# TrevorS/voxtral-mini-realtime-rs

Measured on AMD Instinct MI355X. Metric: decode_tok_per_s, higher is better.
Workload: dtype f32

## Files before the change

include/voxtral_hip.h:

```cpp
#ifndef VOXTRAL_HIP_H
#define VOXTRAL_HIP_H

#include <stddef.h>
#include <stdint.h>

#ifdef __cplusplus
extern "C" {
#endif

#define VOX_OK 0
#define VOX_ERR_INVALID 1
#define VOX_ERR_IO 2
#define VOX_ERR_HIP 3
#define VOX_ERR_NOTFOUND 4
#define VOX_ERR_UNSUPPORTED 5

#define VOX_MEM_HOST 0
#define VOX_MEM_DEVICE 1

typedef struct vox_ctx vox_ctx;
typedef struct vox_gguf vox_gguf;
typedef struct vox_q4 vox_q4;
typedef struct vox_model vox_model;
typedef struct vox_cache vox_cache;
// ... 17 lines not shown
int32_t vox_resample_len(size_t n_in, uint32_t sr_in, uint32_t sr_out, size_t* n_out);
int32_t vox_resample(vox_ctx* ctx, const float* in, size_t n_in, uint32_t sr_in, uint32_t sr_out, float* out, size_t cap, size_t* n_out,
                     int32_t mem_kind);
int32_t vox_resample_plan(uint32_t sr_in, uint32_t sr_out, int32_t* fft_in, int32_t* fft_out, int32_t* delay, float* cutoff, float* taps_or_null, size_t cap);
int32_t vox_peak_normalize(float* samples, size_t n, float target_peak);

typedef struct {
    uint32_t sample_rate;
    uint32_t n_left_pad_tokens;
    float    frame_rate;
    uint32_t extra_right_pad_tokens;
} vox_pad_cfg;
int32_t vox_pad_cfg_voxtral(vox_pad_cfg* cfg);
int32_t vox_pad_len(size_t n, const vox_pad_cfg* cfg, size_t* out);
int32_t vox_pad_audio(const float* in, size_t n, const vox_pad_cfg* cfg, float* out);
int32_t vox_num_audio_tokens(size_t n, const vox_pad_cfg* cfg, size_t* out);

typedef struct {
    uint32_t max_mel_frames;
    uint32_t hop_length;
    uint32_t sample_rate;
    uint32_t overlap_frames;
} vox_chunk_cfg;
typedef struct { size_t start_sample, end_sample, index; int32_t is_last; } vox_chunk;
int32_t vox_needs_chunking(size_t n, const vox_chunk_cfg* cfg, int32_t* out);
int32_t vox_chunk_plan(size_t n, const vox_chunk_cfg* cfg, vox_chunk* out, size_t cap, size_t* n_chunks);

int32_t vox_mel_num_frames(size_t n_samples, size_t* out);
int32_t vox_mel_filterbank(float* out_128x201);
int32_t vox_hann_window(int32_t length, float* out);
int32_t vox_mel_compute_log(vox_ctx* ctx, const float* samples, size_t n, float* out_Tx128, int32_t mem_kind);

int32_t vox_time_embedding(float t, int32_t dim, float* out);

int32_t vox_gguf_open(const char* path, vox_gguf** out);
int32_t vox_gguf_open_memory(const void* data, size_t size, vox_gguf** out);
int32_t vox_gguf_open_shards(const void* const* shards, const size_t* sizes, int32_t n, vox_gguf** out);
int32_t vox_gguf_close(vox_gguf* g);
int32_t vox_gguf_version(const vox_gguf* g, uint32_t* out);
int32_t vox_gguf_tensor_count(const vox_gguf* g, uint64_t* out);
int32_t vox_gguf_tensor_name(const vox_gguf* g, uint64_t index, const char** out);
int32_t vox_gguf_tensor_info(const vox_gguf* g, const char* name, uint64_t dims[4], uint32_t* ndims,
                             uint32_t* dtype, uint64_t* nbytes);
int32_t vox_gguf_tensor_data(const vox_gguf* g, const char* name, void* dst, size_t cap);

int32_t vox_q4_tensor_from_bytes(vox_ctx* ctx, const uint8_t* raw, size_t nbytes, int64_t N, int64_t K, vox_q4** out);
int32_t vox_q4_tensor_shape(const vox_q4* q, int64_t* N, int64_t* K);
int32_t vox_q4_tensor_num_blocks(const vox_q4* q, int64_t* out);
int32_t vox_q4_tensor_dequantize(vox_ctx* ctx, const vox_q4* q, float* out_NxK);
int32_t vox_q4_tensor_free(vox_q4* q);
int32_t vox_q4_matmul(vox_ctx* ctx, const vox_q4* w, const float* x, int32_t B, int32_t M, float* out, int32_t mem_kind);
int32_t vox_q4_linear_forward(vox_ctx* ctx, const vox_q4* w, const float* bias_or_null, const float* x,
                              int32_t B, int32_t M, float* out, int32_t mem_kind);

int32_t vox_dense_tensor_from_f32(vox_ctx* ctx, const float* w_NxK, const float* w_other_or_null, int64_t N, int64_t K, vox_q4** out);
int32_t vox_linear_forward_ex(vox_ctx* ctx, const vox_q4* w, const float* bias_or_null, const float* x, int32_t B, int32_t M, float* out, int32_t epilogue, int32_t mem_kind);
int32_t vox_conv_downsample(vox_ctx* ctx, const float* x_CxL, int32_t C, int32_t L, const float* w1, const float* b1, const float* w2, const float* b2, int32_t O, float* out_OxL2);

typedef struct {
    int32_t enc_layers, enc_dim, enc_heads, enc_head_dim, enc_ffn, enc_window;
    int32_t dec_layers, dec_dim, dec_heads, dec_kv_heads, dec_head_dim, dec_ffn, dec_window, vocab;
    int32_t n_mels, reshape_factor, t_cond_dim;
    float rope_theta, norm_eps;
} vox_model_cfg;

int32_t vox_attention(vox_ctx* ctx, const float* q, const float* k, const float* v, int32_t M, int32_t kv_len, int32_t n_heads,
                      int32_t n_kv_heads, int32_t head_dim, int32_t offset, int32_t window, float* out, int32_t mem_kind);

int32_t vox_q4_model_load(vox_ctx* ctx, const char* gguf_path, vox_model** out);
#define VOX_LOAD_LAYOUT_ONLY 1u
int32_t vox_q4_model_load_ex(vox_ctx* ctx, const char* gguf_path, uint32_t flags, vox_model** out);
int32_t vox_q4_model_load_gguf(vox_ctx* ctx, vox_gguf* g, uint32_t flags, vox_model** out);
int32_t vox_f32_model_load(vox_ctx* ctx, const char* safetensors_path, vox_model** out);
int32_t vox_model_free(vox_model* m);
int32_t vox_model_config(const vox_model* m, vox_model_cfg* out);
int32_t vox_model_weight_bytes(const vox_model* m, uint64_t* out);
int32_t vox_model_arena(const vox_model* m, void** dev_ptr, uint64_t* nbytes);
int32_t vox_model_arena_finalize(vox_model* m);
int32_t vox_model_replicate(const vox_model* src, vox_ctx* dst_ctx, vox_model** out);
int32_t vox_model_memory(const vox_model* m, uint64_t out[4]);

int32_t vox_model_set_t_embed(vox_model* m, const float* t_embed_host);
int32_t vox_model_set_decode_engine(vox_model* m, int32_t on, int32_t* active_or_null);
int32_t vox_model_set_batch_engine(vox_model* m, int32_t on, int32_t* active_or_null, uint64_t* launches_or_null);

int32_t vox_encode_audio(vox_model* m, const float* mel_128xT, int32_t T, float* out, int32_t cap_rows,
                         int32_t* S, int32_t mem_kind);
int32_t vox_transcribe_streaming(vox_model* m, const float* mel_128xT, int32_t T, const float* t_embed,
                                 int32_t* out_ids, int32_t cap, int32_t* n_ids, float* logits_or_null,
                                 int32_t mem_kind);
int32_t vox_transcribe_audio(vox_model* m, const float* samples, size_t n, const float* t_embed,
                             int32_t* out_ids, int32_t cap, int32_t* n_ids, int32_t mem_kind);

int32_t vox_transcribe_batch(vox_model* m, int32_t n, const float* const* samples, const size_t* n_samples, const float* t_embed,
                             int32_t* const* out_ids, const int32_t* caps, int32_t* n_ids, int32_t mem_kind);
int32_t vox_transcribe_batch_ex(vox_model* m, int32_t n, const float* const* samples, const size_t* n_samples, const int32_t* norm_group_or_null, const float* t_embed,
                                int32_t* const* out_ids, const int32_t* caps, int32_t* n_ids, int32_t mem_kind);
int32_t vox_model_set_sessions(vox_model* m, int32_t sessions);

int32_t vox_decoder_cache_create(vox_model* m, int32_t max_seq, vox_cache** out);
int32_t vox_cache_free(vox_cache* c);
int32_t vox_cache_seq_len(const vox_cache* c, int32_t* out);
int32_t vox_cache_reset(vox_cache* c);
int32_t vox_cache_update(vox_cache* c, int32_t layer, int32_t pos, const float* k_HxNxhd, const float* v_HxNxhd, int32_t n_rows, int32_t mem_kind);
int32_t vox_cache_truncate(vox_cache* c, int32_t len);
int32_t vox_encoder_cache_create(vox_model* m, int32_t capacity_rows, vox_cache** out);
int32_t vox_encoder_cache_apply_sliding_window(vox_cache* enc_cache, int32_t window);
int32_t vox_cache_abs_pos(const vox_cache* c, int32_t* out);
int32_t vox_encode_audio_with_cache(vox_model* m, const float* mel_128xT, int32_t T, vox_cache* enc_cache, float* out, int32_t cap_rows,
                                    int32_t* S, int32_t mem_kind);
int32_t vox_embed_tokens_from_ids(vox_model* m, const int32_t* ids, int32_t n, float* out_nxD);
int32_t vox_forward_hidden_with_cache(vox_model* m, const float* x_MxD, int32_t M, const float* t_embed,
                                      vox_cache* cache, float* out_MxD);
int32_t vox_lm_head(vox_model* m, const float* hidden_MxD, int32_t M, float* logits_MxV);
int32_t vox_embed_tokens_from_ids_ex(vox_model* m, const int32_t* ids_host, int32_t n, float* out_nxD, int32_t mem_kind);
int32_t vox_tensor_add(vox_ctx* ctx, const float* a, const float* b, size_t n, float* out, int32_t mem_kind);
int32_t vox_forward_hidden_with_cache_ex(vox_model* m, const float* x_MxD, int32_t M, const float* t_embed, vox_cache* cache, float* out_MxD_or_null,
                                         const float** hidden_ws_or_null, int32_t mem_kind);
int32_t vox_lm_head_ex(vox_model* m, const float* hidden_MxD, int32_t M, float* logits_MxV, int32_t mem_kind);
int32_t vox_argmax_rows(vox_ctx* ctx, const float* logits_MxV, int32_t M, int32_t V, int32_t* ids_host, int32_t mem_kind);
int32_t vox_lm_head_argmax(vox_model* m, const float* hidden_MxD, int32_t M, int32_t* ids_host, int32_t mem_kind);
int32_t vox_generate_step_with_cache(vox_model* m, const int32_t* token_ids, int32_t n, const float* t_embed, vox_cache* cache, float* logits_nxV);

int32_t vox_forward(vox_model* m, const float* mel_128xT, int32_t T, const float* t_embed, float* logits_SxV, int32_t cap_rows, int32_t* S, int32_t mem_kind);
int32_t vox_forward_streaming(vox_model* m, const float* mel_128xT, int32_t T, const int32_t* token_ids, int32_t n_ids, const float* t_embed, float* logits_SxV,
                              int32_t cap_rows, int32_t* S, int32_t mem_kind);
int32_t vox_forward_with_cache(vox_model* m, const float* mel_128xT, int32_t T, const float* t_embed, vox_cache* enc_cache, vox_cache* dec_cache, float* logits_SxV,
                               int32_t cap_rows, int32_t* S, int32_t mem_kind);

typedef struct { double preprocess_ms, encode_ms, decode_ms, total_ms; int32_t decode_tokens; int32_t graph_replays; } vox_timings;
int32_t vox_get_stage_timings(const vox_model* m, vox_timings* out);

int32_t vox_debug_reload_knobs(void);
int32_t vox_debug_attn_launches(uint64_t* out, int32_t cap);
int32_t vox_debug_gemm_launches(uint64_t* out, int32_t cap);
int32_t vox_debug_occupy(vox_ctx* ctx, int32_t workgroups, int32_t micros);

int32_t vox_bench_decode_gemv(vox_model* m, int32_t which, int32_t iters, double* avg_us, double* bytes_per_launch,
                              const char** kernel_name);

int32_t vox_bench_wide(vox_model* m, int32_t which, int32_t mt, int32_t iters, double out_us[4]);

int32_t vox_debug_timeline_start(vox_ctx* ctx, int32_t n_slots, int32_t n_waves);
int32_t vox_debug_timeline_fetch(vox_ctx* ctx, uint64_t* out, size_t cap_words, int32_t* slots_used, int32_t* meta );
int32_t vox_debug_batch_tap_arm(vox_model* m, const int32_t* units, int32_t n_units, int32_t max_rows);
int32_t vox_debug_batch_tap_fetch(vox_model* m, float* out, int32_t* rows_per_unit);
int32_t vox_debug_encode_batch(vox_model* m, int32_t n, const float* const* mels, const int32_t* T, int32_t layout, float* out, int64_t cap_rows,
                               int32_t* rows_per_clip, int64_t* report);

#ifdef __cplusplus
}
#endif
#endif
```

voxtral-mini-realtime-rs_amd/_lib.py:

```python
from __future__ import annotations

import ctypes as C
import os

from .build import LIB_PATH


class VoxError(RuntimeError):
    def __init__(self, code, msg):
        super().__init__(f"[vox error {code}] {msg}")
        self.code = code


class PadCfg(C.Structure):
    _fields_ = [("sample_rate", C.c_uint32), ("n_left_pad_tokens", C.c_uint32), ("frame_rate", C.c_float),
                ("extra_right_pad_tokens", C.c_uint32)]


class ChunkCfg(C.Structure):
    _fields_ = [("max_mel_frames", C.c_uint32), ("hop_length", C.c_uint32), ("sample_rate", C.c_uint32),
                ("overlap_frames", C.c_uint32)]


class Chunk(C.Structure):
    _fields_ = [("start_sample", C.c_size_t), ("end_sample", C.c_size_t), ("index", C.c_size_t), ("is_last", C.c_int32)]


class ModelCfg(C.Structure):
    _fields_ = [(n, C.c_int32) for n in ("enc_layers", "enc_dim", "enc_heads", "enc_head_dim", "enc_ffn", "enc_window",
                                         "dec_layers", "dec_dim", "dec_heads", "dec_kv_heads", "dec_head_dim", "dec_ffn",
                                         "dec_window", "vocab", "n_mels", "reshape_factor", "t_cond_dim")] + \
               [("rope_theta", C.c_float), ("norm_eps", C.c_float)]


class Timings(C.Structure):
    _fields_ = [("preprocess_ms", C.c_double), ("encode_ms", C.c_double), ("decode_ms", C.c_double), ("total_ms", C.c_double),
                ("decode_tokens", C.c_int32), ("graph_replays", C.c_int32)]


vp, i32, i64, u32, u64, sz, f32 = C.c_void_p, C.c_int32, C.c_int64, C.c_uint32, C.c_uint64, C.c_size_t, C.c_float
P = C.POINTER

SIGNATURES = {
    "vox_last_error": (C.c_char_p, []),
    "vox_abi_version": (i32, []),
    "vox_device_count": (i32, [P(i32)]),
    "vox_ctx_create": (i32, [i32, P(vp)]),
    "vox_ctx_destroy": (i32, [vp]),
    "vox_debug_reload_knobs": (i32, []),
    "vox_ctx_synchronize": (i32, [vp]),
    "vox_ctx_set_shared": (i32, [vp, i32]),
    "vox_ctx_stream": (i32, [vp, P(vp)]),
    "vox_dev_alloc": (i32, [vp, sz, P(vp)]),
    "vox_dev_free": (i32, [vp, vp]),
    "vox_dev_upload": (i32, [vp, vp, vp, sz]),
    "vox_dev_download": (i32, [vp, vp, vp, sz]),
    "vox_dev_copy": (i32, [vp, vp, vp, sz]),
    "vox_peak_normalize": (i32, [vp, sz, f32]),
    "vox_pad_cfg_voxtral": (i32, [P(PadCfg)]),
    "vox_pad_len": (i32, [sz, P(PadCfg), P(sz)]),
    "vox_pad_audio": (i32, [vp, sz, P(PadCfg), vp]),
    "vox_num_audio_tokens": (i32, [sz, P(PadCfg), P(sz)]),
    "vox_needs_chunking": (i32, [sz, P(ChunkCfg), P(i32)]),
    "vox_chunk_plan": (i32, [sz, P(ChunkCfg), P(Chunk), sz, P(sz)]),
    "vox_mel_num_frames": (i32, [sz, P(sz)]),
    "vox_mel_filterbank": (i32, [vp]),
    "vox_hann_window": (i32, [i32, vp]),
    "vox_mel_compute_log": (i32, [vp, vp, sz, vp, i32]),
    "vox_time_embedding": (i32, [f32, i32, vp]),
    "vox_gguf_open": (i32, [C.c_char_p, P(vp)]),
    "vox_gguf_open_memory": (i32, [vp, C.c_size_t, P(vp)]),
    "vox_gguf_open_shards": (i32, [vp, vp, i32, P(vp)]),
    "vox_q4_model_load_gguf": (i32, [vp, vp, C.c_uint32, P(vp)]),
    "vox_gguf_close": (i32, [vp]),
    "vox_gguf_version": (i32, [vp, P(u32)]),
    "vox_gguf_tensor_count": (i32, [vp, P(u64)]),
    "vox_gguf_tensor_name": (i32, [vp, u64, P(C.c_char_p)]),
    "vox_gguf_tensor_info": (i32, [vp, C.c_char_p, P(u64 * 4), P(u32), P(u32), P(u64)]),
    "vox_gguf_tensor_data": (i32, [vp, C.c_char_p, vp, sz]),
    "vox_q4_tensor_from_bytes": (i32, [vp, vp, sz, i64, i64, P(vp)]),
    "vox_q4_tensor_shape": (i32, [vp, P(i64), P(i64)]),
    "vox_q4_tensor_num_blocks": (i32, [vp, P(i64)]),
    "vox_q4_tensor_dequantize": (i32, [vp, vp, vp]),
    "vox_q4_tensor_free": (i32, [vp]),
    "vox_q4_matmul": (i32, [vp, vp, vp, i32, i32, vp, i32]),
    "vox_q4_linear_forward": (i32, [vp, vp, vp, vp, i32, i32, vp, i32]),
    "vox_dense_tensor_from_f32": (i32, [vp, vp, vp, i64, i64, P(vp)]),
    "vox_linear_forward_ex": (i32, [vp, vp, vp, vp, i32, i32, vp, i32, i32]),
    "vox_conv_downsample": (i32, [vp, vp, i32, i32, vp, vp, vp, vp, i32, vp]),
    "vox_attention": (i32, [vp, vp, vp, vp, i32, i32, i32, i32, i32, i32, i32, vp, i32]),
    "vox_q4_model_load": (i32, [vp, C.c_char_p, P(vp)]),
    "vox_q4_model_load_ex": (i32, [vp, C.c_char_p, u32, P(vp)]),
    "vox_f32_model_load": (i32, [vp, C.c_char_p, P(vp)]),
    "vox_model_free": (i32, [vp]),
    "vox_model_config": (i32, [vp, P(ModelCfg)]),
    "vox_model_weight_bytes": (i32, [vp, P(u64)]),
    "vox_model_arena": (i32, [vp, P(vp), P(u64)]),
    "vox_model_set_t_embed": (i32, [vp, vp]),
    "vox_model_set_decode_engine": (i32, [vp, i32, P(i32)]),
    "vox_debug_occupy": (i32, [vp, i32, i32]),
    "vox_model_memory": (i32, [vp, P(C.c_uint64)]),
    "vox_model_set_batch_engine": (i32, [vp, i32, P(i32), P(C.c_uint64)]),
    "vox_model_arena_finalize": (i32, [vp]),
    "vox_model_replicate": (i32, [vp, vp, P(vp)]),
    "vox_model_set_sessions": (i32, [vp, i32]),
    "vox_generate_step_with_cache": (i32, [vp, vp, i32, vp, vp, vp]),
    "vox_encode_audio": (i32, [vp, vp, i32, vp, i32, P(i32), i32]),
    "vox_transcribe_streaming": (i32, [vp, vp, i32, vp, vp, i32, P(i32), vp, i32]),
    "vox_transcribe_audio": (i32, [vp, vp, sz, vp, vp, i32, P(i32), i32]),
    "vox_transcribe_batch": (i32, [vp, i32, P(vp), P(sz), vp, P(vp), P(i32), P(i32), i32]),
    "vox_transcribe_batch_ex": (i32, [vp, i32, P(vp), P(sz), vp, vp, P(vp), P(i32), P(i32), i32]),
    "vox_decoder_cache_create": (i32, [vp, i32, P(vp)]),
    "vox_cache_free": (i32, [vp]),
    "vox_cache_seq_len": (i32, [vp, P(i32)]),
    "vox_cache_reset": (i32, [vp]),
    "vox_cache_update": (i32, [vp, i32, i32, vp, vp, i32, i32]),
    "vox_cache_truncate": (i32, [vp, i32]),
    "vox_resample_len": (i32, [sz, C.c_uint32, C.c_uint32, P(sz)]),
    "vox_resample": (i32, [vp, vp, sz, C.c_uint32, C.c_uint32, vp, sz, P(sz), i32]),
    "vox_resample_plan": (i32, [C.c_uint32, C.c_uint32, P(i32), P(i32), P(i32), P(C.c_float), vp, sz]),
    "vox_encoder_cache_create": (i32, [vp, i32, P(vp)]),
    "vox_encoder_cache_apply_sliding_window": (i32, [vp, i32]),
    "vox_cache_abs_pos": (i32, [vp, P(i32)]),
    "vox_encode_audio_with_cache": (i32, [vp, vp, i32, vp, vp, i32, P(i32), i32]),
    "vox_embed_tokens_from_ids": (i32, [vp, vp, i32, vp]),
    "vox_forward_hidden_with_cache": (i32, [vp, vp, i32, vp, vp, vp]),
    "vox_lm_head": (i32, [vp, vp, i32, vp]),
    "vox_embed_tokens_from_ids_ex": (i32, [vp, vp, i32, vp, i32]),
    "vox_tensor_add": (i32, [vp, vp, vp, sz, vp, i32]),
    "vox_forward_hidden_with_cache_ex": (i32, [vp, vp, i32, vp, vp, vp, P(vp), i32]),
    "vox_lm_head_ex": (i32, [vp, vp, i32, vp, i32]),
    "vox_argmax_rows": (i32, [vp, vp, i32, i32, vp, i32]),
    "vox_lm_head_argmax": (i32, [vp, vp, i32, vp, i32]),
    "vox_forward": (i32, [vp, vp, i32, vp, vp, i32, P(i32), i32]),
    "vox_forward_streaming": (i32, [vp, vp, i32, vp, i32, vp, vp, i32, P(i32), i32]),
    "vox_forward_with_cache": (i32, [vp, vp, i32, vp, vp, vp, vp, i32, P(i32), i32]),
    "vox_get_stage_timings": (i32, [vp, P(Timings)]),
    "vox_bench_decode_gemv": (i32, [vp, i32, i32, P(C.c_double), P(C.c_double), P(C.c_char_p)]),
    "vox_bench_wide": (i32, [vp, i32, i32, i32, P(C.c_double)]),
    "vox_debug_attn_launches": (i32, [P(C.c_uint64), i32]),
    "vox_debug_gemm_launches": (i32, [P(C.c_uint64), i32]),
    "vox_debug_timeline_start": (i32, [vp, i32, i32]),
    "vox_debug_timeline_fetch": (i32, [vp, vp, sz, P(i32), vp]),
    "vox_debug_batch_tap_arm": (i32, [vp, P(i32), i32, i32]),
    "vox_debug_batch_tap_fetch": (i32, [vp, vp, P(i32)]),
    "vox_debug_encode_batch": (i32, [vp, i32, P(vp), P(i32), i32, vp, C.c_int64, P(i32), P(C.c_int64)]),
}

_LIB = None
_KNOBS = None


def _knob_env():
    return tuple(sorted((k, v) for k, v in os.environ.items() if k.startswith("VOX_")))


def lib():
    global _LIB, _KNOBS
    if _LIB is not None:
        k = _knob_env()
        if k != _KNOBS:
            _KNOBS = k; _LIB.vox_debug_reload_knobs()
        return _LIB
    if not os.path.exists(LIB_PATH):
        raise VoxError(-1, f"{LIB_PATH} not built: run `python __graft_entry__.py build` (hipcc, gfx950). "
                           "There is no CPU fallback for the HIP path.")
    L = C.CDLL(LIB_PATH)
    for name, (res, args) in SIGNATURES.items():
        fn = getattr(L, name)
        fn.restype = res
        fn.argtypes = args
    _LIB = L; _KNOBS = _knob_env()
    return L


def check(code: int):
    if code != 0:
        raise VoxError(code, (lib().vox_last_error() or b"").decode(errors="replace"))
```

voxtral-mini-realtime-rs_amd/csrc/vox_api.cpp:

```cpp
#include "../../include/voxtral_hip.h"
#include "vox_kernels.h"

#include <dlfcn.h>
#include <fcntl.h>
#include <sys/mman.h>
#include <sys/stat.h>
#include <unistd.h>

#include <algorithm>
#include <chrono>
#include <cmath>
#include <cstdarg>
#include <cstdio>
#include <cstdlib>
#include <cstring>
#include <map>
#include <mutex>
#include <string>
#include <unordered_map>
#include <thread>
#include <vector>

using namespace vox;

// ... 595 lines not shown
    if (e == hipSuccess) e = hipMemcpy(q->sc_mem, l2.data(), ne * 2, hipMemcpyHostToDevice);
    if (e == hipSuccess) e = hipMemcpy(q->qt_mem, host.data(), ne * 4, hipMemcpyHostToDevice);
    if (e != hipSuccess) return bail(e);
    q->w = Q4W{(const uint4*)q->qs_mem, (const uint16_t*)q->sc_mem, (int)Ntot, (int)K, (int)(K / 32), WFMT_F32}; q->w.qt = (const uint4*)q->qt_mem;
    *out = q; return VOX_OK;
}
extern "C" int32_t vox_linear_forward_ex(vox_ctx* c, const vox_q4* w, const float* bias, const float* x, int32_t B, int32_t M, float* out, int32_t epilogue, int32_t mem_kind) {
    ARGCHK(c && w && x && out, "null argument"); ARGCHK(B > 0 && M > 0, "bad batch/rows"); VOXCHK(ctx_bind(c));
    ARGCHK(epilogue == 0 || epilogue == 1 || epilogue == 2, "epilogue %d: 0 none, 1 GELU, 2 SwiGLU over interleaved gate / up rows", epilogue);
    const int epi = epilogue == 1 ? EPI_GELU : epilogue == 2 ? EPI_SWIGLU : EPI_STORE;
    const int rows = B * M, K = w->w.K, N = w->w.N, No = epilogue == 2 ? N / 2 : N;
    ARGCHK(epilogue != 2 || (N % 2 == 0 && !bias), "SwiGLU epilogue needs an even number of interleaved rows and no bias");
    if (mem_kind == VOX_MEM_DEVICE) return q4_linear_dev(c, w->w, bias, x, K, rows, out, No, epi);
    DevBuf dx, dy, db; HIPCHK(dx.alloc((size_t)rows * K * 4)); HIPCHK(dy.alloc((size_t)rows * No * 4));
    HIPCHK(hipMemcpyAsync(dx.p, x, (size_t)rows * K * 4, hipMemcpyHostToDevice, c->stream));
    if (bias) { HIPCHK(db.alloc((size_t)N * 4)); HIPCHK(hipMemcpyAsync(db.p, bias, (size_t)N * 4, hipMemcpyHostToDevice, c->stream)); }
    VOXCHK(q4_linear_dev(c, w->w, bias ? db.as<float>() : nullptr, dx.as<float>(), K, rows, dy.as<float>(), No, epi));
    HIPCHK(hipMemcpyAsync(out, dy.p, (size_t)rows * No * 4, hipMemcpyDeviceToHost, c->stream)); HIPCHK(hipStreamSynchronize(c->stream));
    return VOX_OK;
}
extern "C" int32_t vox_conv_downsample(vox_ctx* c, const float* x, int32_t C, int32_t L, const float* w1, const float* b1, const float* w2, const float* b2, int32_t O, float* out) {
    ARGCHK(c && x && w1 && b1 && w2 && b2 && out && C > 0 && L > 0 && O > 0, "bad argument"); ARGCHK((3 * C) % 128 == 0 && (3 * O) % 128 == 0, "3 * channels must be a multiple of 128");
    VOXCHK(ctx_bind(c)); hipStream_t s = c->stream;
    const int T1 = (L + 2 - 3) / 2 + 1, S = (T1 + 2 - 3) / 2 + 1;
    auto planes = [&](const float* w, int Co, int Ci, DevBuf& hi, DevBuf& lo, Q4W* q) -> int32_t {
        const size_t K = (size_t)3 * Ci; std::vector<float> r((size_t)Co * K);
        for (int co = 0; co < Co; co++) for (int ci = 0; ci < Ci; ci++) for (int kk = 0; kk < 3; kk++) r[(size_t)co * K + (size_t)kk * Ci + ci] = w[((size_t)co * Ci + ci) * 3 + kk];
        std::vector<uint16_t> h(r.size()), l(r.size()); bf16_split(r.data(), r.size(), h.data(), l.data());
        HIPCHK(hi.alloc(h.size() * 2)); HIPCHK(lo.alloc(l.size() * 2));
        HIPCHK(hipMemcpy(hi.p, h.data(), h.size() * 2, hipMemcpyHostToDevice)); HIPCHK(hipMemcpy(lo.p, l.data(), l.size() * 2, hipMemcpyHostToDevice));
        *q = Q4W{(const uint4*)hi.p, (const uint16_t*)lo.p, Co, (int)K, (int)(K / 32), WFMT_BF16X2}; return VOX_OK;
    };
    DevBuf h1, l1, h2, l2, dx, dm, d1, dy, dyt, db1, db2; Q4W g1{}, g2{};
    VOXCHK(planes(w1, O, C, h1, l1, &g1)); VOXCHK(planes(w2, O, O, h2, l2, &g2));
    HIPCHK(dx.alloc((size_t)C * L * 4)); HIPCHK(dm.alloc((size_t)(L + 2) * C * 4)); HIPCHK(d1.alloc((size_t)(T1 + 2) * O * 4)); HIPCHK(dy.alloc((size_t)S * O * 4)); HIPCHK(dyt.alloc((size_t)S * O * 4));
    HIPCHK(db1.alloc((size_t)O * 4)); HIPCHK(db2.alloc((size_t)O * 4));
    HIPCHK(hipMemcpyAsync(dx.p, x, (size_t)C * L * 4, hipMemcpyHostToDevice, s)); HIPCHK(hipMemcpyAsync(db1.p, b1, (size_t)O * 4, hipMemcpyHostToDevice, s)); HIPCHK(hipMemcpyAsync(db2.p, b2, (size_t)O * 4, hipMemcpyHostToDevice, s));
    HIPCHK(hipMemsetAsync(dm.p, 0, (size_t)(L + 2) * C * 4, s)); HIPCHK(hipMemsetAsync(d1.p, 0, (size_t)(T1 + 2) * O * 4, s));
    HIPCHK(launch_transpose(dx.as<float>(), C, L, dm.as<float>() + C, s));
    { GemmParams g{}; g.w = g1; g.x = dm.as<float>(); g.x_stride = 2 * C; g.M = T1; g.out = d1.as<float>() + O; g.out_stride = O; g.bias = db1.as<float>(); HIPCHK(launch_dense2_gemm(g, EPI_GELU, s)); }
    { GemmParams g{}; g.w = g2; g.x = d1.as<float>(); g.x_stride = 2 * O; g.M = S; g.out = dy.as<float>(); g.out_stride = O; g.bias = db2.as<float>(); HIPCHK(launch_dense2_gemm(g, EPI_GELU, s)); }
    HIPCHK(launch_transpose(dy.as<float>(), S, O, dyt.as<float>(), s));
    HIPCHK(hipMemcpyAsync(out, dyt.p, (size_t)S * O * 4, hipMemcpyDeviceToHost, s)); HIPCHK(hipStreamSynchronize(s));
    return VOX_OK;
}

extern "C" int32_t vox_attention(vox_ctx* c, const float* q, const float* k, const float* v, int32_t M, int32_t kv_len, int32_t n_heads,
                                 int32_t n_kv_heads, int32_t head_dim, int32_t offset, int32_t window, float* out, int32_t mem_kind) {
    ARGCHK(c && q && k && v && out, "null argument");
    ARGCHK(M > 0 && kv_len > 0 && n_heads > 0 && n_kv_heads > 0 && n_heads % n_kv_heads == 0, "bad attention shape");
    ARGCHK(head_dim == 64 || head_dim == 128, "head_dim must be 64 (encoder) or 128 (decoder)");
    ARGCHK(offset >= 0 && offset + M <= kv_len, "queries must lie inside the key range (offset + M <= kv_len)");
    VOXCHK(ctx_bind(c));
    const size_t qn = (size_t)M * n_heads * head_dim, kn = (size_t)kv_len * n_kv_heads * head_dim;
    DevBuf dq, dk, dv, dout;
    const float *pq = q, *pk = k, *pv = v; float* po = out;
    if (mem_kind != VOX_MEM_DEVICE) {
        HIPCHK(dq.alloc(qn * 4)); HIPCHK(dk.alloc(kn * 4)); HIPCHK(dv.alloc(kn * 4)); HIPCHK(dout.alloc(qn * 4));
        HIPCHK(hipMemcpyAsync(dq.p, q, qn * 4, hipMemcpyHostToDevice, c->stream));
        HIPCHK(hipMemcpyAsync(dk.p, k, kn * 4, hipMemcpyHostToDevice, c->stream));
        HIPCHK(hipMemcpyAsync(dv.p, v, kn * 4, hipMemcpyHostToDevice, c->stream));
        pq = dq.as<float>(); pk = dk.as<float>(); pv = dv.as<float>(); po = dout.as<float>();
    }
    AttnParams ap{}; ap.q = pq; ap.q_stride = n_heads * head_dim; ap.k = pk; ap.v = pv; ap.kv_row_stride = n_kv_heads * head_dim; ap.kv_head_stride = head_dim;
    ap.out = po; ap.out_stride = n_heads * head_dim; ap.M = M; ap.kv_len = kv_len; ap.n_heads = n_heads; ap.n_kv_heads = n_kv_heads; ap.offset = offset; ap.window = window;
    HIPCHK(launch_attn_prefill(ap, head_dim, c->stream));
    if (mem_kind != VOX_MEM_DEVICE) { HIPCHK(hipMemcpyAsync(out, po, qn * 4, hipMemcpyDeviceToHost, c->stream)); HIPCHK(hipStreamSynchronize(c->stream)); }
    return VOX_OK;
}

struct Lin { Q4W w{}; const float* bias = nullptr; };
struct EncLayer { const float *attn_norm = nullptr, *ffn_norm = nullptr; Lin wqkv, wo, w13, w2; };
struct DecLayer { const float *attn_norm = nullptr, *ffn_norm = nullptr; Lin wqkv, wo, w13, w2, ada0, ada2; float* ada_mul = nullptr; };

struct vox_cache { vox_model* m; vox_ctx* ctx = nullptr; float *k = nullptr, *v = nullptr; int max_seq = 0, len = 0; size_t layer_stride = 0;
                   int kind = 0, abs_pos = 0; uint64_t gen = 0; };

static std::mutex g_cache_mu; static std::unordered_map<const vox_cache*, uint64_t> g_cache_live; static uint64_t g_cache_gen = 0;
static void cache_register(vox_cache* k) { std::lock_guard<std::mutex> l(g_cache_mu); k->gen = ++g_cache_gen; g_cache_live[k] = k->gen; }
static void cache_unregister(const vox_cache* k) { std::lock_guard<std::mutex> l(g_cache_mu); g_cache_live.erase(k); }
static bool cache_alive(const vox_cache* k, uint64_t gen) { std::lock_guard<std::mutex> l(g_cache_mu); auto it = g_cache_live.find(k); return it != g_cache_live.end() && it->second == gen; }

struct TensorMeta { std::vector<uint64_t> shape; int dtype = 0; uint64_t nbytes = 0; };
struct vox_model {
    vox_ctx* ctx = nullptr; vox_model_cfg cfg{};
    std::vector<vox_model*> twins;
    std::map<std::string, TensorMeta> manifest; bool is_q4 = false;
    uint8_t* arena = nullptr; uint64_t arena_bytes = 0, arena_primary_bytes = 0;
    std::vector<Q4W*> tiled;
    const float *conv1_w = nullptr, *conv1_b = nullptr, *conv2_w = nullptr, *conv2_b = nullptr, *enc_norm = nullptr, *dec_norm = nullptr;
    Q4W conv1_g{}, conv2_g{};
    const float *enc_cos = nullptr, *enc_sin = nullptr, *dec_cos = nullptr, *dec_sin = nullptr;
    int enc_rope_len = 4096, dec_rope_len = 16384;
    std::vector<EncLayer> enc; std::vector<DecLayer> dec; Lin ad0, ad2, tok;
    float* ada_mul = nullptr; bool t_embed_set = false; std::vector<float> t_embed_host;
    float* ws = nullptr; size_t ws_floats = 0;
    float *d_audio = nullptr; int audio_cap = 0;
    float *d_mel = nullptr; size_t mel_cap = 0;
    float *d_samples = nullptr; size_t samples_cap = 0;
    vox_cache* cache = nullptr;
    int *d_tokens = nullptr, *d_pos = nullptr; int tokens_cap = 0;
    float* d_prefix = nullptr;
    float *enc_cos_s = nullptr, *enc_sin_s = nullptr; int enc_rope_s_len = 0;
    int* d_seq_len = nullptr; std::vector<int> h_seq_len;
    int *d_seq_off = nullptr, *d_row_pos = nullptr; size_t row_pos_cap = 0; std::vector<int> h_seq_off, h_row_pos;
    float *d_h = nullptr, *d_q = nullptr, *d_att = nullptr, *d_act = nullptr, *d_logits = nullptr, *d_part_val = nullptr; int* d_part_idx = nullptr;
    float* d_h2 = nullptr; long long* d_wo_acc = nullptr;
    int n_parts = 0, argmax_R = 8;
    bool eng_ok = false, eng_on = true, eng_ready = false; unsigned char* eng_stream = nullptr; unsigned char* eng_state = nullptr; EngLayerTab* eng_tab = nullptr;
    const vox_cache* eng_tab_cache = nullptr; const float* eng_tab_k = nullptr; std::vector<EngLayerTab> eng_tab_host;
    int eng_flags = 128 | 512 | 1, eng_pace = 50;
    unsigned long long eng_launches = 0; unsigned eng_err_host[2] = {0, 0};
    int eng_strikes = 0; bool eng_suspended = false;
    unsigned char* eng_wob = nullptr;
    bool engb_ok = false; unsigned char* engb_state[4] = {nullptr, nullptr, nullptr, nullptr}; EngLayerTab* engb_tab[4] = {nullptr, nullptr, nullptr, nullptr};
    bool engb_on = true; unsigned long long engb_launches = 0; int engb_strikes = 0;
    int batch_sessions = 0;
    int engb_flags = 128 | 1 | 64 | 2048;
    int engb_flags2 = 128 | 1024;
    unsigned engb_err_host[4][2] = {{0, 0}, {0, 0}, {0, 0}, {0, 0}};
    hipGraph_t graph[2] = {nullptr, nullptr}; hipGraphExec_t graph_exec[2] = {nullptr, nullptr}; int graph_unroll = 0, graph_mode = 0;
    const vox_cache* graph_cache = nullptr; const float* graph_audio = nullptr;
    float *pw_x = nullptr, *pw_hidden = nullptr, *pw_logits = nullptr; size_t pw_x_cap = 0, pw_hidden_cap = 0, pw_logits_cap = 0;
    float* pw_part_val = nullptr; int* pw_part_idx = nullptr; int* pw_ids = nullptr; int pw_ids_cap = 0; int* pw_zero = nullptr;
    EngLayerTab* pw_tab = nullptr; const vox_cache* pw_tab_cache = nullptr; uint64_t pw_tab_gen = 0;
    bool pw_memo = false, pw_eng_used = false;
    vox_cache* pw_pend_cache = nullptr; uint64_t pw_pend_gen = 0; int pw_pend_rows = 0; bool pw_verdict_failed = false;
    unsigned* pw_err_pin = nullptr;
    vox_timings timings{};
    struct { std::vector<int> units; int max_rows = 0; bool armed = false, on = false, ready = false; float* out = nullptr; int* rows = nullptr; } tap;
};

struct Arena {
    uint8_t* base = nullptr; uint64_t off = 0;
    template <class T> T* take(size_t count) {
        off = (off + 255) / 256 * 256;
        T* p = base ? reinterpret_cast<T*>(base + off) : nullptr;
        off += count * sizeof(T);
        return p;
    }
};

#define ENC_PFX "mm_streams_embeddings.embedding_module.whisper_encoder"
#define EMB_PFX "mm_streams_embeddings.embedding_module"
#define TOK_NAME EMB_PFX ".tok_embeddings.weight"
#define ADP_PFX EMB_PFX ".audio_language_projection"

enum { DT_F32 = 0, DT_F16 = 1, DT_Q4_0 = 2, DT_BF16 = 3 };
struct TensorView { std::vector<uint64_t> shape; int dtype = 0; const uint8_t* data = nullptr; uint64_t nbytes = 0; };
struct TensorSource {
    virtual ~TensorSource() {}
    virtual bool find(const std::string& name, TensorView* out) const = 0;
    virtual uint64_t max_q4_bytes() const { return 0; }
};
struct GgufSource : TensorSource {
    vox_gguf* g = nullptr;
    ~GgufSource() override { if (g) vox_gguf_close(g); }
    bool find(const std::string& name, TensorView* out) const override {
        const GTensor* t = g->find(name); if (!t) return false;
        out->shape.assign(t->dims, t->dims + t->ndims); std::reverse(out->shape.begin(), out->shape.end());
        out->dtype = (int)t->dtype; out->data = g->data(t); out->nbytes = t->nbytes; return true;
    }
    uint64_t max_q4_bytes() const override { uint64_t m = 0; for (auto& t : g->tensors) if (t.dtype == 2) m = std::max<uint64_t>(m, t.nbytes); return m; }
};
struct RecordingSource : TensorSource {
    const TensorSource* in; mutable std::map<std::string, TensorMeta> seen;
    explicit RecordingSource(const TensorSource* s) : in(s) {}
// ... 251 lines not shown
            if (hipMemcpy(dst, host.data(), (size_t)tot * 4, hipMemcpyHostToDevice) != hipSuccess) setfail("hipMemcpy failed for bias");
        }
        return dst;
    }
    const float* rope(int hd, int len, float theta, bool sine) {
        const int half = hd / 2; float* dst = ar.take<float>((size_t)len * half);
        if (fill) {
            std::vector<float> t((size_t)len * half);
            for (int i = 0; i < len; i++)
                for (int j = 0; j < half; j++) {
                    const float inv = 1.0f / std::pow(theta, (float)(2 * j) / (float)hd), fr = (float)i * inv;
                    t[(size_t)i * half + j] = sine ? std::sin(fr) : std::cos(fr);
                }
            if (hipMemcpy(dst, t.data(), t.size() * 4, hipMemcpyHostToDevice) != hipSuccess) setfail("hipMemcpy failed for rope table");
        }
        return dst;
    }

    bool run(bool q4) {
        vox_model_cfg& c = m->cfg; char a[320]; TensorView tv;
        c.enc_head_dim = 64; c.dec_head_dim = 128; c.enc_window = 750; c.dec_window = 8192; c.rope_theta = 1e6f; c.norm_eps = 1e-5f; c.reshape_factor = 4;
        int ne = 0, nd = 0;
        for (;; ne++) { snprintf(a, sizeof a, ENC_PFX ".transformer.layers.%d.attention.wq.weight", ne); if (!src->find(a, &tv)) break; }
        for (;; nd++) { snprintf(a, sizeof a, "layers.%d.attention.wq.weight", nd); if (!src->find(a, &tv)) break; }
        if (ne == 0 || nd == 0) return setfail("model file has no encoder/decoder layers");
        c.enc_layers = ne; c.dec_layers = nd; m->enc.resize(ne); m->dec.resize(nd);
        TensorView cw; if (!need(ENC_PFX ".conv_layers.0.conv.weight", &cw)) return false;
        if (cw.shape.size() != 3 || cw.shape[2] != 3) return setfail("conv weight must be [out][in][3]");
        c.n_mels = (int)cw.shape[1]; c.enc_dim = (int)cw.shape[0];
        m->conv1_w = f32(ENC_PFX ".conv_layers.0.conv.weight"); m->conv1_b = f32(ENC_PFX ".conv_layers.0.conv.bias");
        m->conv2_w = f32(ENC_PFX ".conv_layers.1.conv.weight"); m->conv2_b = f32(ENC_PFX ".conv_layers.1.conv.bias");
        if ((3 * c.n_mels) % 128 == 0 && (3 * c.enc_dim) % 128 == 0) {
            if (!conv_planes(ENC_PFX ".conv_layers.0.conv.weight", &m->conv1_g) || !conv_planes(ENC_PFX ".conv_layers.1.conv.weight", &m->conv2_g)) return false;
        }
        for (int i = 0; i < ne; i++) {
            EncLayer& L = m->enc[i]; std::string p = std::string(ENC_PFX ".transformer.layers.") + std::to_string(i);
            L.attn_norm = f32(p + ".attention_norm.weight"); L.ffn_norm = f32(p + ".ffn_norm.weight");
            if (!lin({p + ".attention.wq.weight", p + ".attention.wk.weight", p + ".attention.wv.weight"}, false, &L.wqkv, q4)) return false;
            const int64_t hq = L.wqkv.w.N / 3;
            L.wqkv.bias = bias_cat({{p + ".attention.wq.bias", hq}, {"", hq}, {p + ".attention.wv.bias", hq}});
            if (!lin({p + ".attention.wo.weight"}, false, &L.wo, q4)) return false;
            L.wo.bias = bias_cat({{p + ".attention.wo.bias", L.wo.w.N}});
            if (!lin({p + ".feed_forward.w1.weight", p + ".feed_forward.w3.weight"}, true, &L.w13, q4)) return false;
            if (!lin({p + ".feed_forward.w2.weight"}, false, &L.w2, q4)) return false;
            L.w2.bias = bias_cat({{p + ".feed_forward.w2.bias", L.w2.w.N}});
        }
        m->enc_norm = f32(ENC_PFX ".transformer.norm.weight");
        if (!lin({ADP_PFX ".0.weight"}, false, &m->ad0, q4) || !lin({ADP_PFX ".2.weight"}, false, &m->ad2, q4)) return false;
        if (!lin({TOK_NAME}, false, &m->tok, false, true)) return false;
        for (int i = 0; i < nd; i++) {
            DecLayer& L = m->dec[i]; std::string p = "layers." + std::to_string(i);
            if (!lin({p + ".ada_rms_norm_t_cond.0.weight"}, false, &L.ada0, q4) || !lin({p + ".ada_rms_norm_t_cond.2.weight"}, false, &L.ada2, q4)) return false;
            L.attn_norm = f32(p + ".attention_norm.weight"); L.ffn_norm = f32(p + ".ffn_norm.weight");
            if (!lin({p + ".attention.wq.weight", p + ".attention.wk.weight", p + ".attention.wv.weight"}, false, &L.wqkv, q4, true)) return false;
            if (!lin({p + ".attention.wo.weight"}, false, &L.wo, q4, true)) return false;
            if (!lin({p + ".feed_forward.w1.weight", p + ".feed_forward.w3.weight"}, true, &L.w13, q4, true)) return false;
            if (!lin({p + ".feed_forward.w2.weight"}, false, &L.w2, q4, true)) return false;
        }
        m->dec_norm = f32("norm.weight");
        if (!err.empty()) return false;
        TensorView ewq, dwq, dwk;
        need(std::string(ENC_PFX ".transformer.layers.0.attention.wq.weight"), &ewq); need("layers.0.attention.wq.weight", &dwq); need("layers.0.attention.wk.weight", &dwk);
        c.enc_heads = (int)(ewq.shape[0] / c.enc_head_dim); c.enc_ffn = m->enc[0].w13.w.N / 2;
        c.dec_dim = (int)dwq.shape[1]; c.dec_heads = (int)(dwq.shape[0] / c.dec_head_dim); c.dec_kv_heads = (int)(dwk.shape[0] / c.dec_head_dim);
        c.dec_ffn = m->dec[0].w13.w.N / 2; c.vocab = m->tok.w.N; c.t_cond_dim = m->dec[0].ada0.w.N;
        if (ewq.shape[0] % c.enc_head_dim || dwq.shape[0] % c.dec_head_dim || dwk.shape[0] % c.dec_head_dim || c.dec_kv_heads == 0 || c.dec_heads % c.dec_kv_heads)
            return setfail("attention projection shapes are not multiples of head_dim");
        if ((int)ewq.shape[1] != c.enc_dim || m->ad0.w.K != c.enc_dim * c.reshape_factor || m->ad2.w.N != c.dec_dim || m->ad0.w.N != m->ad2.w.K || m->tok.w.K != c.dec_dim)
            return setfail("inconsistent encoder / adapter / embedding shapes");
        if (c.enc_dim % 32 || c.dec_dim % 32) return setfail("model dims must be multiples of 32");
        m->enc_cos = rope(c.enc_head_dim, m->enc_rope_len, c.rope_theta, false); m->enc_sin = rope(c.enc_head_dim, m->enc_rope_len, c.rope_theta, true);
        m->dec_cos = rope(c.dec_head_dim, m->dec_rope_len, c.rope_theta, false); m->dec_sin = rope(c.dec_head_dim, m->dec_rope_len, c.rope_theta, true);
        return err.empty();
    }
};
}

static void graphs_destroy(vox_model* m) {
    for (int i = 0; i < 2; i++) {
        if (m->graph_exec[i]) { (void)hipGraphExecDestroy(m->graph_exec[i]); m->graph_exec[i] = nullptr; }
        if (m->graph[i]) { (void)hipGraphDestroy(m->graph[i]); m->graph[i] = nullptr; }
    }
}
static void model_release(vox_model* m) {
    if (!m) return;
    for (vox_model* t : m->twins) { vox_ctx* tc = t->ctx; model_release(t); (void)vox_ctx_destroy(tc); }
    m->twins.clear();
    (void)hipSetDevice(m->ctx->device); (void)hipStreamSynchronize(m->ctx->stream);
    graphs_destroy(m);
    if (m->cache) { cache_unregister(m->cache); (void)hipFree(m->cache->k); (void)hipFree(m->cache->v); delete m->cache; }
    if (m->ctx->pw_model == m) m->ctx->pw_model = nullptr;
    for (void* p : {(void*)m->arena, (void*)m->ada_mul, (void*)m->ws, (void*)m->d_audio, (void*)m->d_mel, (void*)m->d_samples, (void*)m->d_tokens, (void*)m->d_pos,
                    (void*)m->d_h, (void*)m->d_h2, (void*)m->d_wo_acc, (void*)m->d_q, (void*)m->d_att, (void*)m->d_act, (void*)m->d_logits, (void*)m->d_part_val, (void*)m->d_part_idx, (void*)m->d_seq_len, (void*)m->d_seq_off, (void*)m->d_row_pos, (void*)m->d_prefix, (void*)m->enc_cos_s, (void*)m->enc_sin_s, (void*)m->eng_stream, (void*)m->eng_wob, (void*)m->eng_state, (void*)m->eng_tab, (void*)m->engb_state[0], (void*)m->engb_state[1], (void*)m->engb_state[2], (void*)m->engb_state[3],
                    (void*)m->engb_tab[0], (void*)m->engb_tab[1], (void*)m->engb_tab[2], (void*)m->engb_tab[3], (void*)m->pw_x, (void*)m->pw_hidden, (void*)m->pw_logits, (void*)m->pw_part_val, (void*)m->pw_part_idx, (void*)m->pw_ids, (void*)m->pw_zero, (void*)m->pw_tab})
        if (p) (void)hipFree(p);
    if (m->pw_err_pin) (void)hipHostFree(m->pw_err_pin);
    if (m->tap.out) (void)hipFree(m->tap.out);
    if (m->tap.rows) (void)hipFree(m->tap.rows);
    delete m;
}
extern "C" int32_t vox_model_free(vox_model* m) { model_release(m); return VOX_OK; }

static int32_t model_build(vox_ctx* ctx, const TensorSource* src_in, bool q4, bool layout_only, vox_model** out) {
    vox_model* m = new vox_model(); m->ctx = ctx;
    RecordingSource rec(src_in); const TensorSource* src = &rec;
    std::map<std::string, bool> fmt_cache;
    Loader plan{m, src, Arena{}, false}; plan.fmt_cache = &fmt_cache;
    if (!plan.run(q4)) { std::string e = plan.err; model_release(m); return fail(VOX_ERR_IO, "%s", e.c_str()); }
    m->arena_primary_bytes = (plan.ar.off + 255) / 256 * 256 + 256;
    m->arena_bytes = m->arena_primary_bytes + plan.ar2.off + 256;
    if (hipMalloc((void**)&m->arena, m->arena_bytes) != hipSuccess) { model_release(m); return fail(VOX_ERR_HIP, "hipMalloc of %.1f MB weight arena failed", m->arena_bytes / 1e6); }
    const size_t max_q4 = layout_only ? 16 : std::max<uint64_t>(src->max_q4_bytes(), 16);
    DevBuf staging; if (staging.alloc(max_q4) != hipSuccess) { model_release(m); return fail(VOX_ERR_HIP, "hipMalloc of staging buffer failed"); }
    Loader fillr{m, src, Arena{m->arena, 0}, !layout_only, staging.p, max_q4}; fillr.fmt_cache = &fmt_cache; fillr.ar2 = Arena{m->arena + m->arena_primary_bytes, 0};
    if (!fillr.run(q4)) { std::string e = fillr.err; model_release(m); return fail(VOX_ERR_IO, "%s", e.c_str()); }
    const vox_model_cfg& c = m->cfg;
    const int qdim = c.dec_heads * c.dec_head_dim;
    if (m->tok.w.fmt == WFMT_BF16 || m->tok.w.fmt == WFMT_F32) { m->argmax_R = 2; m->n_parts = dense_gemv_grid(c.vocab); }
    else { m->argmax_R = q4_gemv_default_R(c.vocab, c.dec_dim, EPI_ARGMAX); m->n_parts = m->argmax_R > 0 ? q4_gemv_grid(c.vocab, m->argmax_R) : 1; }
    hipError_t e = hipSuccess;
    auto A = [&](void** p, size_t n) { if (e == hipSuccess) e = hipMalloc(p, n); };
    A((void**)&m->ada_mul, (size_t)c.dec_layers * c.dec_dim * 4); A((void**)&m->d_pos, 64); A((void**)&m->d_h, (size_t)c.dec_dim * 4 * 4);
    A((void**)&m->d_q, (size_t)qdim * 4 * 4); A((void**)&m->d_att, (size_t)qdim * 4 * 4); A((void**)&m->d_act, (size_t)c.dec_ffn * 4 * 4);
    A((void**)&m->d_h2, (size_t)c.dec_dim * 4); A((void**)&m->d_wo_acc, (size_t)c.dec_layers * c.dec_dim * 8);
    A((void**)&m->d_logits, (size_t)c.vocab * 4); A((void**)&m->d_part_val, (size_t)m->n_parts * 4 * 4); A((void**)&m->d_part_idx, (size_t)m->n_parts * 4 * 4);
    if (e != hipSuccess) { model_release(m); return fail(VOX_ERR_HIP, "hipMalloc of decode buffers failed: %s", hipGetErrorString(e)); }
    if (hipMemset(m->d_wo_acc, 0, (size_t)c.dec_layers * c.dec_dim * 8) != hipSuccess) { model_release(m); return fail(VOX_ERR_HIP, "hipMemset failed"); }
    for (int i = 0; i < c.dec_layers; i++) m->dec[i].ada_mul = m->ada_mul + (size_t)i * c.dec_dim;
    {
        const char* ev = knob_str("VOX_ENGINE"); bool ok = !(ev && ev[0] == '0') && c.dec_layers <= 32 && eng_geometry_ok(c.dec_dim, c.dec_heads, c.dec_kv_heads, c.dec_head_dim, c.dec_ffn, c.vocab, 256);
        hipDeviceProp_t prop; if (ok && (hipGetDeviceProperties(&prop, ctx->device) != hipSuccess || prop.multiProcessorCount != 256)) ok = false;
        for (int i = 0; ok && i < c.dec_layers; i++) { const DecLayer& L = m->dec[i]; for (const Lin* w : {&L.wqkv, &L.wo, &L.w13, &L.w2}) if (w->w.fmt != WFMT_Q4_0 || !w->w.qs || !w->w.sc || w->bias) ok = false; }
        if (ok && (m->tok.w.fmt != WFMT_Q4_0 || !m->tok.w.qs)) ok = false;
        if (ok) { int occ = 0; if (eng_occupancy(&occ) != hipSuccess || occ < 1) { ok = false; (void)hipGetLastError(); } }
        m->eng_ok = ok; m->eng_on = ok;
        {
            const char* bv = knob_str("VOX_BATCH_ENGINE"); int occ = 0;
            m->engb_ok = ok && !(bv && bv[0] == '0') && engb_occupancy(&occ) == hipSuccess && occ >= 1;
            (void)hipGetLastError();
            if (const char* f = knob_str("VOX_BATCH_ENGINE_FLAGS")) m->engb_flags = atoi(f);
            if (const char* f = knob_str("VOX_BATCH_ENGINE_FLAGS2")) m->engb_flags2 = atoi(f);
        }
        if (const char* f = knob_str("VOX_ENGINE_FLAGS")) m->eng_flags = atoi(f);
        if (const char* f = knob_str("VOX_ENGINE_PACE")) m->eng_pace = atoi(f);
    }
    m->manifest = std::move(rec.seen); m->is_q4 = q4;
    *out = m; return VOX_OK;
}

extern "C" int32_t vox_q4_model_load(vox_ctx* ctx, const char* path, vox_model** out) { return vox_q4_model_load_ex(ctx, path, 0, out); }

extern "C" int32_t vox_q4_model_load_gguf(vox_ctx* ctx, vox_gguf* g, uint32_t flags, vox_model** out) {
    ARGCHK(ctx && g && out, "null argument"); VOXCHK(ctx_bind(ctx));
    GgufSource src; src.g = g;
    const int32_t r = model_build(ctx, &src, true, (flags & VOX_LOAD_LAYOUT_ONLY) != 0, out);
    src.g = nullptr;
    return r;
}
extern "C" int32_t vox_q4_model_load_ex(vox_ctx* ctx, const char* path, uint32_t flags, vox_model** out) {
    ARGCHK(ctx && path && out, "null argument"); VOXCHK(ctx_bind(ctx));
    GgufSource src; VOXCHK(vox_gguf_open(path, &src.g));
    return model_build(ctx, &src, true, (flags & VOX_LOAD_LAYOUT_ONLY) != 0, out);
}

extern "C" int32_t vox_f32_model_load(vox_ctx* ctx, const char* path, vox_model** out) {
    ARGCHK(ctx && path && out, "null argument"); VOXCHK(ctx_bind(ctx));
    SafeTensorsSource src; VOXCHK(src.open(path));
    return model_build(ctx, &src, false, false, out);
}

extern "C" int32_t vox_model_config(const vox_model* m, vox_model_cfg* out) { ARGCHK(m && out, "null argument"); *out = m->cfg; return VOX_OK; }
extern "C" int32_t vox_model_weight_bytes(const vox_model* m, uint64_t* out) { ARGCHK(m && out, "null argument"); *out = m->arena_bytes; return VOX_OK; }
extern "C" int32_t vox_model_memory(const vox_model* m, uint64_t out[4]) {
    ARGCHK(m && out, "null argument");
    out[0] = m->arena_bytes; out[1] = m->arena_primary_bytes;
    out[2] = (m->eng_stream ? eng_stream_bytes(m->cfg.dec_layers, m->cfg.vocab) : 0) + (m->eng_wob ? engb_wo_stream_bytes(m->cfg.dec_layers) : 0);
    out[3] = m->eng_state ? eng_state_bytes() : 0;
    for (int gi = 0; gi < 4; gi++) if (m->engb_state[gi]) out[3] += engb_state_bytes();
    return VOX_OK;
}
extern "C" int32_t vox_model_arena(const vox_model* m, void** p, uint64_t* n) { ARGCHK(m && p && n, "null argument"); *p = m->arena; *n = m->arena_primary_bytes; return VOX_OK; }
extern "C" int32_t vox_model_arena_finalize(vox_model* m) {
    ARGCHK(m, "null argument"); VOXCHK(ctx_bind(m->ctx));
    for (Q4W* w : m->tiled) HIPCHK(launch_q4_tile_build(*w, const_cast<uint4*>(w->qt), const_cast<uint16_t*>(w->st), m->ctx->stream));
    HIPCHK(hipStreamSynchronize(m->ctx->stream));
    m->eng_ready = false; m->eng_tab_cache = nullptr;
    if (m->eng_wob) { HIPCHK(hipStreamSynchronize(m->ctx->stream)); (void)hipFree(m->eng_wob); m->eng_wob = nullptr; }
    graphs_destroy(m);
    return VOX_OK;
}

extern "C" int32_t vox_model_replicate(const vox_model* src, vox_ctx* dst_ctx, vox_model** out) {
    ARGCHK(src && dst_ctx && out, "null argument");
    if (!src->is_q4 || src->manifest.empty()) return fail(VOX_ERR_UNSUPPORTED, "vox_model_replicate: Q4 (GGUF) models only");
    VOXCHK(ctx_bind(src->ctx)); HIPCHK(hipStreamSynchronize(src->ctx->stream));
    VOXCHK(ctx_bind(dst_ctx));
    ManifestSource ms; ms.m = &src->manifest;
    vox_model* d = nullptr;
    VOXCHK(model_build(dst_ctx, &ms, true, true, &d));
    if (d->arena_primary_bytes != src->arena_primary_bytes || d->arena_bytes != src->arena_bytes) { model_release(d); return fail(VOX_ERR_INVALID, "internal: replica arena layout differs from the source's"); }
    hipError_t e = src->ctx->device == dst_ctx->device ? hipMemcpyAsync(d->arena, src->arena, src->arena_primary_bytes, hipMemcpyDeviceToDevice, dst_ctx->stream)
                                                       : hipMemcpyPeerAsync(d->arena, dst_ctx->device, src->arena, src->ctx->device, src->arena_primary_bytes, dst_ctx->stream);
    if (e == hipSuccess) e = hipStreamSynchronize(dst_ctx->stream);
    if (e != hipSuccess) { model_release(d); return fail(VOX_ERR_HIP, "vox_model_replicate: device copy failed: %s", hipGetErrorString(e)); }
    const int32_t r = vox_model_arena_finalize(d);
    if (r != VOX_OK) { model_release(d); return r; }
    *out = d; return VOX_OK;
}

extern "C" int32_t vox_model_set_t_embed(vox_model* m, const float* t_embed) {
    ARGCHK(m && t_embed, "null argument"); VOXCHK(ctx_bind(m->ctx));
    const vox_model_cfg& c = m->cfg; vox_ctx* cx = m->ctx;
    if (m->t_embed_set && m->t_embed_host.size() == (size_t)c.dec_dim && !std::memcmp(m->t_embed_host.data(), t_embed, (size_t)c.dec_dim * 4)) return VOX_OK;
    DevBuf dt, dh, ones; HIPCHK(dt.alloc((size_t)c.dec_dim * 4)); HIPCHK(dh.alloc((size_t)c.t_cond_dim * 4)); HIPCHK(ones.alloc((size_t)c.dec_dim * 4));
    std::vector<float> one(c.dec_dim, 1.0f);
    HIPCHK(hipMemcpyAsync(dt.p, t_embed, (size_t)c.dec_dim * 4, hipMemcpyHostToDevice, cx->stream));
    HIPCHK(hipMemcpyAsync(ones.p, one.data(), (size_t)c.dec_dim * 4, hipMemcpyHostToDevice, cx->stream));
    for (int i = 0; i < c.dec_layers; i++) {
        VOXCHK(q4_linear_dev(cx, m->dec[i].ada0.w, nullptr, dt.as<float>(), c.dec_dim, 1, dh.as<float>(), c.t_cond_dim, EPI_GELU));
        VOXCHK(q4_linear_dev(cx, m->dec[i].ada2.w, nullptr, dh.as<float>(), c.t_cond_dim, 1, m->dec[i].ada_mul, c.dec_dim, EPI_RESID, ones.as<float>(), c.dec_dim));
    }
    HIPCHK(hipStreamSynchronize(cx->stream));
    m->t_embed_host.assign(t_embed, t_embed + c.dec_dim); m->t_embed_set = true;
    return VOX_OK;
}

static int conv_len(int L) { return (L + 2 - 3) / 2 + 1; }

static int32_t ensure(float** p, size_t* cap, size_t need) {
    if (*cap >= need) return VOX_OK;
    if (*p) HIPCHK(hipFree(*p));
    *p = nullptr; *cap = 0;
    HIPCHK(hipMalloc((void**)p, need * sizeof(float))); *cap = need; return VOX_OK;
}

static int enc_rows(int T) { return conv_len(conv_len(T)); }
static int enc_row_budget(const vox_model* m, const int* T, int n) {
    int mx = 0; for (int i = 0; i < n; i++) mx = std::max(mx, enc_rows(T[i]));
    const int r = m->cfg.reshape_factor; return n == 1 ? mx : (mx + r - 1) / r * r;
}
static size_t conv_scratch_floats(const vox_model* m, int T) {
    const int D = m->cfg.enc_dim, T1 = conv_len(T);
    return std::max((size_t)D * T1, (size_t)(T + 2) * m->cfg.n_mels + (size_t)(T1 + 2) * D) + 64;
}
static int32_t conv_stem_dev(vox_model* m, const float* d_mel, int T, float* c1, float* x) {
    const vox_model_cfg& c = m->cfg; hipStream_t s = m->ctx->stream; const int D = c.enc_dim, T1 = conv_len(T), S = conv_len(T1);
    const bool conv_mfma = m->conv1_g.qs && m->conv2_g.qs && !knob_str("VOX_CONV_VALU");
    if (conv_mfma) {
        const int Cm = c.n_mels;
        float* melT = c1; float* c1T = melT + (size_t)(T + 2) * Cm;
        HIPCHK(hipMemsetAsync(melT, 0, (size_t)Cm * 4, s)); HIPCHK(hipMemsetAsync(melT + (size_t)(T + 1) * Cm, 0, (size_t)Cm * 4, s));
        HIPCHK(hipMemsetAsync(c1T, 0, (size_t)D * 4, s)); HIPCHK(hipMemsetAsync(c1T + (size_t)(T1 + 1) * D, 0, (size_t)D * 4, s));
        HIPCHK(launch_transpose(d_mel, Cm, T, melT + Cm, s));
        { GemmParams g{}; g.w = m->conv1_g; g.x = melT; g.x_stride = 2 * Cm; g.M = T1; g.out = c1T + D; g.out_stride = D; g.bias = m->conv1_b; HIPCHK(launch_dense2_gemm(g, EPI_GELU, s)); }
        { GemmParams g{}; g.w = m->conv2_g; g.x = c1T; g.x_stride = 2 * D; g.M = S; g.out = x; g.out_stride = D; g.bias = m->conv2_b; HIPCHK(launch_dense2_gemm(g, EPI_GELU, s)); }
    } else {
        HIPCHK(launch_conv1d_gelu(d_mel, c.n_mels, T, m->conv1_w, m->conv1_b, D, c1, 0, s));
        HIPCHK(launch_conv1d_gelu(c1, D, T1, m->conv2_w, m->conv2_b, D, x, 1, s));
    }
    return VOX_OK;
}
static int enc_packed_rows_of(const vox_model* m, int T) { const int R = m->cfg.reshape_factor; return std::max((enc_rows(T) + R - 1) / R * R, R * 40); }
static long enc_packed_rows(const vox_model* m, const int* T, int n) { long r = 0; for (int i = 0; i < n; i++) r += enc_packed_rows_of(m, T[i]); return r; }
struct EncForms { long Mtot = 0; int ksp = 0, ksp_wo = 0, fused_rope = 0; };
static int32_t encode_batch_dev(vox_model* m, int n, const float* const* d_mels, const int* T, float* audio_out, int audio_rows, int* S4_out, long* audio_off_out = nullptr,
                                EncForms* forms = nullptr) {
    const vox_model_cfg& c = m->cfg; vox_ctx* cx = m->ctx; hipStream_t s = cx->stream;
    const int D = c.enc_dim, H = c.enc_heads, hd = c.enc_head_dim, QD = H * hd, F = c.enc_ffn, R = c.reshape_factor;
    const bool packed = audio_off_out != nullptr;
    ARGCHK(n <= 128, "internal: encoder stack of %d utterances", n);
    const int S_pad = enc_row_budget(m, T, n);
    int T1max = 0; bool any = false;
    std::vector<int> S(n);
    for (int i = 0; i < n; i++) { S[i] = enc_rows(T[i]); S4_out[i] = S[i] / R; T1max = std::max(T1max, conv_len(T[i])); any = any || S4_out[i] > 0; }
    if (!any || S_pad <= 0) return VOX_OK;
    ARGCHK(S_pad <= m->enc_rope_len, "audio too long for the encoder RoPE table (%d > %d positions); chunk it (--max-mel-frames)", S_pad, m->enc_rope_len);
    std::vector<int> roff(n + 1, 0);
    if (packed) for (int i = 0; i < n; i++) roff[i + 1] = roff[i] + enc_packed_rows_of(m, T[i]);
    const int Mtot = packed ? roff[n] : n * S_pad, M4 = packed ? Mtot / R : n == 1 ? S4_out[0] : Mtot / R;
    ARGCHK(packed || n == 1 || audio_rows >= S_pad / R, "internal: audio row budget %d < %d", audio_rows, S_pad / R);
    int Tmax = 0; for (int i = 0; i < n; i++) Tmax = std::max(Tmax, T[i]);
    (void)T1max;
    const size_t c1_floats = conv_scratch_floats(m, Tmax);
    int ksp = 0;
    {
        const Q4W& w2 = m->enc[0].w2.w;
        const long wgs = (long)((w2.N + 127) / 128) * ((Mtot + 31) / 32);
        const bool geom_ok = w2.fmt == WFMT_Q4_0 && w2.qt && w2.st && w2.nb % 16 == 0 && Mtot > 48 && D % 4 == 0 && D <= 4096;
        if (geom_ok && wgs < 1024) ksp = 4;
        if (const char* e = knob_str("VOX_ENC_SPLITK")) ksp = geom_ok && atoi(e) > 1 ? std::min(atoi(e), w2.nb / 4) : 0;
        for (int l = 0; ksp && l < c.enc_layers; l++) if (m->enc[l].w2.w.fmt != WFMT_Q4_0 || !m->enc[l].w2.w.qt || m->enc[l].w2.w.nb / 4 < ksp) ksp = 0;
    }
    int ksp_wo = ksp ? 2 : 0;
    if (ksp) { if (const char* e = knob_str("VOX_ENC_SPLITK_WO")) ksp_wo = atoi(e) > 1 ? std::min(atoi(e), ksp) : 0; }
    for (int l = 0; ksp_wo && l < c.enc_layers; l++) if (m->enc[l].wo.w.fmt != WFMT_Q4_0 || !m->enc[l].wo.w.qt || m->enc[l].wo.w.nb / 4 < ksp_wo || m->enc[l].wo.w.nb % 4) ksp_wo = 0;
    const size_t need = c1_floats + (size_t)Mtot * D * 2 + (size_t)Mtot * QD * 4 + (size_t)Mtot * F + (size_t)(M4 + 1) * m->ad0.w.N + (size_t)ksp * Mtot * D + 1024;
    VOXCHK(ensure(&m->ws, &m->ws_floats, need));
    if (forms) { forms->Mtot = Mtot; forms->ksp = ksp; forms->ksp_wo = ksp_wo; forms->fused_rope = 0; }
    float* c1 = m->ws; float* x = c1 + c1_floats / 64 * 64; float* xn = x + (size_t)Mtot * D; float* qkv = xn + (size_t)Mtot * D;
    float* att = qkv + (size_t)Mtot * QD * 3; float* ffn = att + (size_t)Mtot * QD; float* ah = ffn + (size_t)Mtot * F; float* w2p = ah + (size_t)(M4 + 1) * m->ad0.w.N;
    const int* d_len = nullptr; const int* d_roff = nullptr; const int* d_rpos = nullptr;
    if (n > 1 || packed) {
        HIPCHK(hipMemsetAsync(x, 0, (size_t)Mtot * D * 4, s));
        HIPCHK(hipMemsetAsync(att, 0, (size_t)Mtot * QD * 4, s));
        if (!m->d_seq_len) HIPCHK(hipMalloc((void**)&m->d_seq_len, 128 * sizeof(int)));
        m->h_seq_len.assign(S.begin(), S.end());
        HIPCHK(hipMemcpyAsync(m->d_seq_len, m->h_seq_len.data(), (size_t)n * 4, hipMemcpyHostToDevice, s));
        d_len = m->d_seq_len;
    }
    if (packed) {
        if (!m->d_seq_off) HIPCHK(hipMalloc((void**)&m->d_seq_off, 128 * sizeof(int)));
        if (m->row_pos_cap < (size_t)Mtot) { if (m->d_row_pos) { HIPCHK(hipStreamSynchronize(s)); HIPCHK(hipFree(m->d_row_pos)); } m->d_row_pos = nullptr; m->row_pos_cap = 0;
                                              HIPCHK(hipMalloc((void**)&m->d_row_pos, (size_t)Mtot * sizeof(int))); m->row_pos_cap = (size_t)Mtot; }
        HIPCHK(hipStreamSynchronize(s));
        m->h_seq_off.assign(roff.begin(), roff.begin() + n); m->h_row_pos.resize((size_t)Mtot);
        for (int i = 0; i < n; i++) for (int r = roff[i]; r < roff[i + 1]; r++) m->h_row_pos[(size_t)r] = std::min(r - roff[i], m->enc_rope_len - 1);
        HIPCHK(hipMemcpyAsync(m->d_seq_off, m->h_seq_off.data(), (size_t)n * 4, hipMemcpyHostToDevice, s)); HIPCHK(hipMemcpyAsync(m->d_row_pos, m->h_row_pos.data(), (size_t)Mtot * 4, hipMemcpyHostToDevice, s));
        d_roff = m->d_seq_off; d_rpos = m->d_row_pos;
    }
    for (int i = 0; i < n; i++) {
        if (S[i] <= 0) continue;
        VOXCHK(conv_stem_dev(m, d_mels[i], T[i], c1, x + (packed ? (size_t)roff[i] : (size_t)i * S_pad) * D));
    }
    const int seq_rows = packed ? 0 : n > 1 ? S_pad : 0;
    for (int l = 0; l < c.enc_layers; l++) {
        const EncLayer& L = m->enc[l];
        if (ksp && l > 0) HIPCHK(launch_rms_norm_sumk(x, D, Mtot, D, w2p, (size_t)Mtot * D, ksp, L.attn_norm, c.norm_eps, xn, D, s));
        else HIPCHK(launch_rms_norm(x, D, Mtot, D, L.attn_norm, nullptr, c.norm_eps, xn, D, s));
        if (Mtot > 48) {
            GemmParams g{}; g.w = L.wqkv.w; g.x = xn; g.x_stride = D; g.M = Mtot; g.out = qkv; g.out_stride = 3 * QD; g.bias = L.wqkv.bias;
            g.rope_cos = m->enc_cos; g.rope_sin = m->enc_sin; g.hd = hd; g.n_q = 2 * QD; g.pos = d_rpos; g.rope_seq_rows = seq_rows;
            bool fused = false; HIPCHK(launch_q4_gemm(g, EPI_ROPE_ROWS, s, &fused));
            if (forms && fused) forms->fused_rope++;
        } else {
            VOXCHK(q4_linear_dev(cx, L.wqkv.w, L.wqkv.bias, xn, D, Mtot, qkv, 3 * QD));
            HIPCHK(launch_rope(qkv, Mtot, 3 * QD, 2 * QD, hd, 0, m->enc_cos, m->enc_sin, s, seq_rows, d_rpos));
        }
        AttnParams ap{}; ap.q = qkv; ap.q_stride = 3 * QD; ap.k = qkv + QD; ap.v = qkv + 2 * QD; ap.kv_row_stride = 3 * QD; ap.kv_head_stride = hd;
        ap.out = att; ap.out_stride = QD; ap.M = S_pad; ap.kv_len = S_pad; ap.n_heads = H; ap.n_kv_heads = H; ap.offset = 0; ap.window = c.enc_window;
        ap.seq_len = d_len; ap.q_seq_stride = S_pad * 3 * QD; ap.out_seq_stride = S_pad * QD; ap.kv_seq_stride = (long)S_pad * 3 * QD; ap.seq_row_off = d_roff;
        HIPCHK(launch_attn_prefill(ap, hd, s, n));
        if (ksp_wo) {
            VOXCHK(q4_linear_dev(cx, L.wo.w, L.wo.bias, att, QD, Mtot, w2p, D, EPI_STORE, nullptr, 0, ksp_wo));
            HIPCHK(launch_rms_norm_sumk(x, D, Mtot, D, w2p, (size_t)Mtot * D, ksp_wo, L.ffn_norm, c.norm_eps, xn, D, s));
        } else {
            VOXCHK(q4_linear_dev(cx, L.wo.w, L.wo.bias, att, QD, Mtot, x, D, EPI_RESID, x, D));
            HIPCHK(launch_rms_norm(x, D, Mtot, D, L.ffn_norm, nullptr, c.norm_eps, xn, D, s));
        }
        VOXCHK(q4_linear_dev(cx, L.w13.w, nullptr, xn, D, Mtot, ffn, F, EPI_SWIGLU));
        if (ksp) VOXCHK(q4_linear_dev(cx, L.w2.w, L.w2.bias, ffn, F, Mtot, w2p, D, EPI_STORE, nullptr, 0, ksp));
        else VOXCHK(q4_linear_dev(cx, L.w2.w, L.w2.bias, ffn, F, Mtot, x, D, EPI_RESID, x, D));
    }
    if (ksp && c.enc_layers > 0) HIPCHK(launch_rms_norm_sumk(x, D, Mtot, D, w2p, (size_t)Mtot * D, ksp, m->enc_norm, c.norm_eps, xn, D, s));
    else HIPCHK(launch_rms_norm(x, D, Mtot, D, m->enc_norm, nullptr, c.norm_eps, xn, D, s));
    VOXCHK(q4_linear_dev(cx, m->ad0.w, nullptr, xn, D * R, M4, ah, m->ad0.w.N, EPI_GELU));
    if (packed) { for (int i = 0; i < n; i++) audio_off_out[i] = (long)(roff[i] / R) * c.dec_dim; }
    if (packed || n == 1 || audio_rows * R == S_pad) VOXCHK(q4_linear_dev(cx, m->ad2.w, nullptr, ah, m->ad0.w.N, M4, audio_out, c.dec_dim));
    else for (int i = 0; i < n; i++)
        VOXCHK(q4_linear_dev(cx, m->ad2.w, nullptr, ah + (size_t)i * (S_pad / R) * m->ad0.w.N, m->ad0.w.N, S_pad / R, audio_out + (size_t)i * audio_rows * c.dec_dim, c.dec_dim));
    return VOX_OK;
}
static int32_t encode_dev(vox_model* m, const float* d_mel, int T, int* S4_out) {
    const int S4 = enc_rows(T) / m->cfg.reshape_factor;
    if (S4 > 0) { size_t cap = (size_t)m->audio_cap * m->cfg.dec_dim; VOXCHK(ensure(&m->d_audio, &cap, (size_t)S4 * m->cfg.dec_dim)); m->audio_cap = (int)(cap / m->cfg.dec_dim); }
    return encode_batch_dev(m, 1, &d_mel, &T, m->d_audio, S4, S4_out);
}

static int32_t cache_alloc(vox_model* m, int max_seq, vox_cache** out) {
    const vox_model_cfg& c = m->cfg;
    ARGCHK(max_seq > 0 && max_seq <= m->dec_rope_len, "max_seq %d out of range (1..%d)", max_seq, m->dec_rope_len);
    vox_cache* k = new vox_cache(); k->m = m; k->ctx = m->ctx; k->max_seq = max_seq;
    const size_t n = (size_t)c.dec_layers * c.dec_kv_heads * max_seq * c.dec_head_dim * 4;
    if (hipMalloc((void**)&k->k, n) != hipSuccess || hipMalloc((void**)&k->v, n) != hipSuccess) { if (k->k) (void)hipFree(k->k); delete k; return fail(VOX_ERR_HIP, "hipMalloc of KV cache failed"); }
    HIPCHK(hipMemsetAsync(k->k, 0, n, m->ctx->stream)); HIPCHK(hipMemsetAsync(k->v, 0, n, m->ctx->stream));
    k->layer_stride = (size_t)c.dec_kv_heads * max_seq * c.dec_head_dim;
    cache_register(k);
    *out = k; return VOX_OK;
}
extern "C" int32_t vox_decoder_cache_create(vox_model* m, int32_t max_seq, vox_cache** out) { ARGCHK(m && out, "null argument"); VOXCHK(ctx_bind(m->ctx)); return cache_alloc(m, max_seq, out); }
extern "C" int32_t vox_cache_free(vox_cache* k) {
    if (!k) return VOX_OK;
    (void)hipSetDevice(k->ctx->device); (void)hipStreamSynchronize(k->ctx->stream);
    cache_unregister(k);
    (void)hipFree(k->k); (void)hipFree(k->v); delete k; return VOX_OK;
}
static int32_t pw_sync(vox_model* m);
static int32_t cache_settle_pending(vox_cache* kc) {
    vox_model* m = kc->m;
    if (m && m->pw_pend_rows > 0 && m->pw_pend_cache == kc) { VOXCHK(ctx_bind(kc->ctx)); VOXCHK(pw_sync(m)); }
    return VOX_OK;
}
extern "C" int32_t vox_cache_update(vox_cache* kc, int32_t layer, int32_t pos, const float* k, const float* v, int32_t n_rows, int32_t mem_kind) {
    ARGCHK(kc && k && v && n_rows > 0 && pos >= 0, "bad argument"); VOXCHK(ctx_bind(kc->ctx)); VOXCHK(cache_settle_pending(kc));
    const vox_model_cfg& c = kc->m->cfg;
    const int L = kc->kind == 1 ? c.enc_layers : c.dec_layers, H = kc->kind == 1 ? c.enc_heads : c.dec_kv_heads, hd = kc->kind == 1 ? c.enc_head_dim : c.dec_head_dim;
    ARGCHK(layer >= 0 && layer < L, "layer %d out of range (0..%d)", layer, L - 1);
    ARGCHK(pos + n_rows <= kc->max_seq, "KV cache overflow: %d + %d > %d", pos, n_rows, kc->max_seq);
    hipStream_t s = kc->ctx->stream; const hipMemcpyKind kind = mem_kind == VOX_MEM_DEVICE ? hipMemcpyDeviceToDevice : hipMemcpyHostToDevice;
    for (int h = 0; h < H; h++) {
        const size_t dst = (size_t)layer * kc->layer_stride + ((size_t)h * kc->max_seq + pos) * hd, src = (size_t)h * n_rows * hd, nb = (size_t)n_rows * hd * 4;
        HIPCHK(hipMemcpyAsync(kc->k + dst, k + src, nb, kind, s)); HIPCHK(hipMemcpyAsync(kc->v + dst, v + src, nb, kind, s));
    }
    if (mem_kind != VOX_MEM_DEVICE) HIPCHK(hipStreamSynchronize(s));
    kc->len = std::max(kc->len, pos + n_rows);
    return VOX_OK;
}
extern "C" int32_t vox_cache_truncate(vox_cache* kc, int32_t len) {
    ARGCHK(kc, "null cache"); VOXCHK(cache_settle_pending(kc)); ARGCHK(len >= 0 && len <= kc->len, "truncate to %d: the cache holds %d rows", len, kc->len);
    if (kc->kind == 1) kc->abs_pos -= kc->len - len;
    kc->len = len; return VOX_OK;
}
extern "C" int32_t vox_cache_seq_len(const vox_cache* k, int32_t* out) { ARGCHK(k && out, "null argument"); *out = k->len; return VOX_OK; }
extern "C" int32_t vox_cache_reset(vox_cache* k) {
    ARGCHK(k, "null cache");
    (void)cache_settle_pending(k);
    k->len = 0; k->abs_pos = 0; return VOX_OK;
}

static size_t cache_layer_floats(const vox_model* m, const vox_cache* k) { (void)m; return k->layer_stride; }

extern "C" int32_t vox_encoder_cache_create(vox_model* m, int32_t capacity_rows, vox_cache** out) {
    ARGCHK(m && out, "null argument"); VOXCHK(ctx_bind(m->ctx));
    const vox_model_cfg& c = m->cfg;
    if (capacity_rows <= 0) capacity_rows = 2 * c.enc_window + 512;
    ARGCHK(capacity_rows > c.enc_window, "encoder cache capacity %d must exceed the sliding window (%d)", capacity_rows, c.enc_window);
    vox_cache* k = new vox_cache(); k->m = m; k->ctx = m->ctx; k->max_seq = capacity_rows; k->kind = 1;
    const size_t n = (size_t)c.enc_layers * c.enc_heads * capacity_rows * c.enc_head_dim * 4;
    if (hipMalloc((void**)&k->k, n) != hipSuccess || hipMalloc((void**)&k->v, n) != hipSuccess) { if (k->k) (void)hipFree(k->k); delete k; return fail(VOX_ERR_HIP, "hipMalloc of encoder KV cache failed"); }
    HIPCHK(hipMemsetAsync(k->k, 0, n, m->ctx->stream)); HIPCHK(hipMemsetAsync(k->v, 0, n, m->ctx->stream));
    k->layer_stride = (size_t)c.enc_heads * capacity_rows * c.enc_head_dim;
    cache_register(k);
    *out = k; return VOX_OK;
}
extern "C" int32_t vox_cache_abs_pos(const vox_cache* k, int32_t* out) { ARGCHK(k && out, "null argument"); *out = k->kind == 1 ? k->abs_pos : k->len; return VOX_OK; }

static int32_t enc_cache_evict(vox_model* m, vox_cache* kc, int keep) {
    const vox_model_cfg& c = m->cfg; hipStream_t s = m->ctx->stream;
    if (keep >= kc->len) return VOX_OK;
    const size_t planes = (size_t)c.enc_layers * c.enc_heads, pitch = (size_t)kc->max_seq * c.enc_head_dim * 4, width = (size_t)keep * c.enc_head_dim * 4;
    VOXCHK(ensure(&m->ws, &m->ws_floats, planes * width / 4 + 64));
    for (float* base : {kc->k, kc->v}) {
        const char* src = reinterpret_cast<const char*>(base) + (size_t)(kc->len - keep) * c.enc_head_dim * 4;
        HIPCHK(hipMemcpy2DAsync(m->ws, width, src, pitch, width, planes, hipMemcpyDeviceToDevice, s));
        HIPCHK(hipMemcpy2DAsync(base, pitch, m->ws, width, width, planes, hipMemcpyDeviceToDevice, s));
    }
    kc->len = keep;
    return VOX_OK;
}
// ... 242 lines not shown
    if (!m->eng_ready) return VOX_OK;
    if (m->eng_tab_cache != m->cache || m->eng_tab_k != m->cache->k) {
        const size_t lf = cache_layer_floats(m, m->cache);
        m->eng_tab_host.resize(c.dec_layers);
        for (int l = 0; l < c.dec_layers; l++) m->eng_tab_host[l] = EngLayerTab{m->dec[l].attn_norm, m->dec[l].ffn_norm, m->dec[l].ada_mul, m->cache->k + (size_t)l * lf, m->cache->v + (size_t)l * lf};
        HIPCHK(hipMemcpyAsync(m->eng_tab, m->eng_tab_host.data(), sizeof(EngLayerTab) * c.dec_layers, hipMemcpyHostToDevice, s));
        HIPCHK(hipStreamSynchronize(s));
        m->eng_tab_cache = m->cache; m->eng_tab_k = m->cache->k;
    }
    return VOX_OK;
}
static bool engb_prepare(vox_model* m, int n_grp) {
    if (!m->engb_ok || !m->engb_on || n_grp > 4) return false;
    if (engine_stream_prepare(m) != VOX_OK || !m->eng_ready) return false;
    if (engb_prepare_kernels() != hipSuccess) { (void)hipGetLastError(); m->engb_ok = false; return false; }
    if (!m->eng_wob) {
        const vox_model_cfg& c = m->cfg; hipStream_t s = m->ctx->stream;
        hipError_t e = hipMalloc((void**)&m->eng_wob, engb_wo_stream_bytes(c.dec_layers));
        if (e == hipSuccess) e = hipMemsetAsync(m->eng_wob, 0, engb_wo_stream_bytes(c.dec_layers), s);
        for (int l = 0; l < c.dec_layers && e == hipSuccess; l++) e = launch_eng_pack(m->dec[l].wo.w, 5, l, c.dec_layers, m->eng_wob, c.vocab, s);
        if (e != hipSuccess) { (void)hipGetLastError(); if (m->eng_wob) { (void)hipFree(m->eng_wob); m->eng_wob = nullptr; } m->engb_ok = false; return false; }
    }
    for (int gi = 0; gi < n_grp; gi++) {
        if (m->engb_state[gi]) continue;
        hipError_t e = hipMalloc((void**)&m->engb_state[gi], engb_state_bytes());
        if (e == hipSuccess) e = hipMalloc((void**)&m->engb_tab[gi], sizeof(EngLayerTab) * 32);
        if (e == hipSuccess) e = engb_state_init(m->engb_state[gi], m->ctx->stream);
        if (e != hipSuccess) { (void)hipGetLastError(); if (m->engb_state[gi]) { (void)hipFree(m->engb_state[gi]); m->engb_state[gi] = nullptr; } return false; }
    }
    return true;
}
static bool engine_active(const vox_model* m) { return m->eng_on && !m->eng_suspended && m->eng_ready && m->cache && m->eng_tab_cache == m->cache && m->eng_tab_k == m->cache->k && m->cache->max_seq <= 1024; }
static EngParams engine_params(vox_model* m, float* logits_out, bool argmax_in = false) {
    const vox_model_cfg& c = m->cfg;
    EngParams ep{}; ep.stream = m->eng_stream; ep.cu_stride = eng_stream_bytes(c.dec_layers, c.vocab) / 256; ep.layers = m->eng_tab; ep.n_layers = c.dec_layers; ep.h_in = m->d_h; ep.final_norm = m->dec_norm;
    ep.pos_ptr = m->d_pos; ep.pos_off = 0; ep.rope_cos = m->dec_cos; ep.rope_sin = m->dec_sin; ep.max_seq = m->cache->max_seq; ep.window = c.dec_window; ep.eps = c.norm_eps;
    eng_state_carve(m->eng_state, &ep); ep.part_val = m->d_part_val; ep.part_idx = m->d_part_idx; ep.logits_out = logits_out; ep.vocab = c.vocab; ep.tl = nullptr; ep.tl_layer = -1;
    ep.flags = m->eng_flags; ep.pace_ticks = (m->eng_flags & 512) ? 0 : m->eng_pace; ep.ag_delay_ticks = (m->eng_flags & 512) ? m->eng_pace : 0;
    if (argmax_in) {
        ep.flags |= 65536; ep.h_in = nullptr; ep.tokens = m->d_tokens; ep.pos_rw = m->d_pos; ep.tok_qs = m->tok.w.qs; ep.tok_sc = m->tok.w.sc; ep.tok_nb = m->tok.w.nb; ep.audio = m->d_audio;
    }
    return ep;
}

extern "C" int32_t vox_model_set_decode_engine(vox_model* m, int32_t on, int32_t* active) {
    ARGCHK(m, "null argument"); VOXCHK(ctx_bind(m->ctx));
    const bool want = on != 0 && m->eng_ok;
    if (want != m->eng_on) { HIPCHK(hipStreamSynchronize(m->ctx->stream)); graphs_destroy(m); m->eng_on = want; }
    if (active) *active = m->eng_on ? 1 : 0;
    return VOX_OK;
}

extern "C" int32_t vox_model_set_batch_engine(vox_model* m, int32_t on, int32_t* active, uint64_t* launches) {
    ARGCHK(m, "null argument");
    if (on >= 0) m->engb_on = on != 0;
    if (active) *active = m->engb_ok && m->engb_on ? 1 : 0;
    if (launches) *launches = m->engb_launches;
    return VOX_OK;
}

static int32_t lm_head_argmax_dev(vox_model* m, const float* h, float* logits_out) {
    const vox_model_cfg& c = m->cfg;
    ARGCHK(c.dec_dim <= 4096, "lm_head GEMV is instantiated for dec_dim <= 4096 (got %d)", c.dec_dim);
    GemvParams p{}; p.w = m->tok.w; p.x = h; p.x_stride = c.dec_dim; p.out = logits_out; p.out_stride = c.vocab; p.gamma = m->dec_norm; p.eps = c.norm_eps;
    p.part_val = m->d_part_val; p.part_idx = m->d_part_idx;
    if (m->tok.w.fmt == WFMT_Q4_0) m->n_parts = q4_gemv_grid_k(c.vocab, c.dec_dim, m->argmax_R, EPI_ARGMAX);
    HIPCHK(launch_q4_gemv(p, 1, PRO_RMS, EPI_ARGMAX, m->argmax_R, m->ctx->stream));
    return VOX_OK;
}

static int32_t ensure_decode_state(vox_model* m, int S) {
    if (!m->cache || m->cache->max_seq < S) {
        int cap = std::max(S, 256); cap = std::min((cap + 255) / 256 * 256, m->dec_rope_len);
        ARGCHK(S <= cap, "sequence of %d decoder positions exceeds the RoPE table (%d)", S, m->dec_rope_len);
        if (m->cache) { HIPCHK(hipStreamSynchronize(m->ctx->stream)); cache_unregister(m->cache); (void)hipFree(m->cache->k); (void)hipFree(m->cache->v); delete m->cache; m->cache = nullptr; m->eng_tab_cache = nullptr; m->eng_tab_k = nullptr; }
        graphs_destroy(m);
        VOXCHK(cache_alloc(m, cap, &m->cache));
    }
    if (!m->d_tokens) { m->tokens_cap = m->dec_rope_len + 2; HIPCHK(hipMalloc((void**)&m->d_tokens, (size_t)m->tokens_cap * 4)); }
    ARGCHK(S + 2 <= m->tokens_cap, "sequence of %d decoder positions exceeds the token buffer", S);
    return VOX_OK;
}

static int32_t decode_step_enqueue(vox_model* m, float* logits_out, int mode = 0) {
    const vox_model_cfg& c = m->cfg; hipStream_t s = m->ctx->stream;
    if (mode != 0) { HIPCHK(launch_decode_engine(engine_params(m, logits_out, mode == 2), s)); return VOX_OK; }
    if (engine_active(m)) {
        HIPCHK(launch_decode_engine(engine_params(m, logits_out), s));
        HIPCHK(launch_argmax_embed(m->d_part_val, m->d_part_idx, 256, m->d_tokens, m->d_pos, m->tok.w, m->d_audio, c.dec_dim, m->d_h, s));
        return VOX_OK;
    }
    VOXCHK(decoder_step_dev(m, m->d_h, m->cache, m->d_pos, 0));
    VOXCHK(lm_head_argmax_dev(m, m->d_h, logits_out));
    HIPCHK(launch_argmax_embed(m->d_part_val, m->d_part_idx, m->n_parts, m->d_tokens, m->d_pos, m->tok.w, m->d_audio, c.dec_dim, m->d_h, s));
    return VOX_OK;
}

static int32_t transcribe_dev(vox_model* m, const float* d_mel, int T, const float* t_embed, int32_t* out_ids, int32_t cap, int32_t* n_ids,
                              float* logits_host) {
    const vox_model_cfg& c = m->cfg; vox_ctx* cx = m->ctx; hipStream_t s = cx->stream;
    const int PREFIX_LEN = 38, BOS = 1, STREAMING_PAD = 32;
    VOXCHK(vox_model_set_t_embed(m, t_embed));
    double t0 = now_ms();
    RoctxScope whole("transcribe_streaming"); RoctxStage stage;
    stage.begin("encode_audio");
    int S = 0; VOXCHK(encode_dev(m, d_mel, T, &S));
    HIPCHK(hipStreamSynchronize(s));
    stage.end();
    m->timings.encode_ms = now_ms() - t0; t0 = now_ms();
    *n_ids = 0; m->timings.decode_tokens = 0; m->timings.graph_replays = 0;
    if (S < PREFIX_LEN) { m->timings.decode_ms = 0; return VOX_OK; }
    const int n = std::max(S - PREFIX_LEN, 1);
    ARGCHK(cap >= n, "out_ids capacity %d < %d", cap, n);
    bool eng_failed = false; int steps = 0;
    auto decode_once = [&]() -> int32_t {
    VOXCHK(ensure_decode_state(m, S));
    VOXCHK(engine_prepare(m));
    if (engine_active(m)) {
        if (m->eng_launches + (unsigned long long)S + 8 > (1ull << 25)) { HIPCHK(hipMemsetAsync(m->eng_state, 0, eng_state_bytes(), s)); m->eng_launches = 0; }
        m->eng_launches += (unsigned long long)S + 8;
    }
    std::vector<int32_t> prefix(PREFIX_LEN, STREAMING_PAD); prefix[0] = BOS;
    HIPCHK(hipMemcpyAsync(m->d_tokens, prefix.data(), PREFIX_LEN * 4, hipMemcpyHostToDevice, s));
    m->cache->len = 0;
    if (!m->d_prefix) HIPCHK(hipMalloc((void**)&m->d_prefix, (size_t)PREFIX_LEN * c.dec_dim * 4));
    float* px = m->d_prefix;
    stage.begin("prefill");
    HIPCHK(launch_embed(m->tok.w, m->d_tokens, PREFIX_LEN, m->d_audio, c.dec_dim, nullptr, 0, 0, px, s));
    VOXCHK(decoder_prefill_dev(m, px, PREFIX_LEN, m->cache, 0));
    m->cache->len = PREFIX_LEN;
    DevBuf dlog; float* d_logits_all = nullptr;
    if (logits_host) { HIPCHK(dlog.alloc((size_t)n * c.vocab * 4)); d_logits_all = dlog.as<float>(); }
    VOXCHK(lm_head_argmax_dev(m, px + (size_t)(PREFIX_LEN - 1) * c.dec_dim, d_logits_all));
    const int pos_init = PREFIX_LEN;
    HIPCHK(hipMemcpyAsync(m->d_pos, &pos_init, 4, hipMemcpyHostToDevice, s));
    HIPCHK(launch_argmax_final(m->d_part_val, m->d_part_idx, m->n_parts, m->d_tokens, m->d_pos, 0, 0, s));
    steps = std::max(S - PREFIX_LEN - 1, 0);
    stage.begin("decode");
    if (steps > 0 && m->d_wo_acc) HIPCHK(hipMemsetAsync(m->d_wo_acc, 0, (size_t)c.dec_layers * c.dec_dim * 8, s));
    if (steps > 0) HIPCHK(launch_embed(m->tok.w, m->d_tokens, 1, m->d_audio, c.dec_dim, m->d_pos, 0, 0, m->d_h, s));
    if (logits_host) {
        for (int i = 0; i < steps; i++) VOXCHK(decode_step_enqueue(m, d_logits_all + (size_t)(i + 1) * c.vocab));
    } else if (steps > 0) {
        const bool chain = engine_active(m) && !(knob_str("VOX_ENGINE_ARGMAX_IN") && knob_str("VOX_ENGINE_ARGMAX_IN")[0] == '0');
        const int step_mode = chain ? 2 : 0;
        int U = engine_active(m) ? 8 : 1; { const char* e = knob_str("VOX_DECODE_UNROLL"); if (e && atoi(e) >= 1 && atoi(e) <= 32) U = atoi(e); }
        if (m->graph_cache != m->cache || m->graph_audio != m->d_audio || m->graph_unroll != U || m->graph_mode != step_mode) {
            graphs_destroy(m); m->graph_cache = m->cache; m->graph_audio = m->d_audio; m->graph_unroll = U; m->graph_mode = step_mode;
        }
        auto capture = [&](int which, int n_steps) -> int32_t {
            HIPCHK(hipStreamBeginCapture(s, hipStreamCaptureModeThreadLocal));
            int32_t r = VOX_OK;
            for (int i = 0; i < n_steps && r == VOX_OK; i++) r = decode_step_enqueue(m, nullptr, step_mode);
            hipError_t ce = hipStreamEndCapture(s, &m->graph[which]);
            if (r != VOX_OK) return r;
            HIPCHK(ce);
            HIPCHK(hipGraphInstantiate(&m->graph_exec[which], m->graph[which], nullptr, nullptr, 0));
            return VOX_OK;
        };
        int done = 0;
        if (chain) { VOXCHK(decode_step_enqueue(m, nullptr, 1)); done = 1; }
        if (!m->graph_exec[0]) {
            if (!chain) { VOXCHK(decode_step_enqueue(m, nullptr)); done = 1; }
            HIPCHK(hipStreamSynchronize(s));
            VOXCHK(capture(0, 1));
        }
        if (U > 1 && !m->graph_exec[1] && steps - done >= 2 * U) VOXCHK(capture(1, U));
        while (U > 1 && m->graph_exec[1] && steps - done >= U) { HIPCHK(hipGraphLaunch(m->graph_exec[1], s)); done += U; m->timings.graph_replays += U; }
        while (done < steps) { HIPCHK(hipGraphLaunch(m->graph_exec[0], s)); done++; m->timings.graph_replays++; }
        if (chain) HIPCHK(launch_argmax_final(m->d_part_val, m->d_part_idx, 256, m->d_tokens, m->d_pos, 1, 1, s));
    }
    HIPCHK(hipMemcpyAsync(out_ids, m->d_tokens + PREFIX_LEN, (size_t)n * 4, hipMemcpyDeviceToHost, s));
    if (logits_host) HIPCHK(hipMemcpyAsync(logits_host, d_logits_all, (size_t)n * c.vocab * 4, hipMemcpyDeviceToHost, s));
    const bool eng_used = engine_active(m) && steps > 0;
    if (eng_used) { EngParams ep = engine_params(m, nullptr); HIPCHK(hipMemcpyAsync(m->eng_err_host, ep.err, 8, hipMemcpyDeviceToHost, s)); }
    HIPCHK(hipStreamSynchronize(s));
    stage.end();
    if (eng_used && m->eng_err_host[0]) { eng_failed = true; return VOX_OK; }
    return VOX_OK;
    };
    VOXCHK(decode_once());
    if (eng_failed) {
        const unsigned e = m->eng_err_host[0];
        m->eng_strikes++;
        fprintf(stderr, "[voxtral_hip] decode engine: hand-off timeout (code %u, workgroup %u), strike %d of 3; this utterance is decoded again on the per-operator path%s\n",
                e & 0xff, (e >> 8) & 0xff, m->eng_strikes, m->eng_strikes >= 3 ? ", the engine is switched off" : "");
        HIPCHK(hipMemsetAsync(m->eng_state, 0, eng_state_bytes(), s)); m->eng_launches = 0; graphs_destroy(m);
        if (m->eng_strikes >= 3) { m->eng_ok = false; m->eng_on = false; }
        m->eng_suspended = true; eng_failed = false;
        const int32_t r = decode_once();
        m->eng_suspended = false; graphs_destroy(m);
        if (r != VOX_OK) return r;
    }
    m->cache->len = PREFIX_LEN + steps;
    *n_ids = n; m->timings.decode_tokens = n;
    m->timings.decode_ms = now_ms() - t0;
    return VOX_OK;
}

extern "C" int32_t vox_encode_audio(vox_model* m, const float* mel, int32_t T, float* out, int32_t cap_rows, int32_t* S, int32_t mem_kind) {
    ARGCHK(m && mel && out && S, "null argument"); ARGCHK(T > 0, "empty mel"); VOXCHK(ctx_bind(m->ctx));
    const vox_model_cfg& c = m->cfg; hipStream_t s = m->ctx->stream;
    const float* d_mel = mel;
    if (mem_kind == VOX_MEM_HOST) {
        VOXCHK(ensure(&m->d_mel, &m->mel_cap, (size_t)c.n_mels * T));
        HIPCHK(hipMemcpyAsync(m->d_mel, mel, (size_t)c.n_mels * T * 4, hipMemcpyHostToDevice, s)); d_mel = m->d_mel;
    }
    int S4 = 0; VOXCHK(encode_dev(m, d_mel, T, &S4));
    ARGCHK(cap_rows >= S4, "output capacity %d rows < %d", cap_rows, S4);
    if (S4 > 0) HIPCHK(hipMemcpyAsync(out, m->d_audio, (size_t)S4 * c.dec_dim * 4, mem_kind == VOX_MEM_HOST ? hipMemcpyDeviceToHost : hipMemcpyDeviceToDevice, s));
    HIPCHK(hipStreamSynchronize(s));
    *S = S4; return VOX_OK;
}

extern "C" int32_t vox_transcribe_streaming(vox_model* m, const float* mel, int32_t T, const float* t_embed, int32_t* out_ids, int32_t cap,
                                            int32_t* n_ids, float* logits, int32_t mem_kind) {
    ARGCHK(m && mel && t_embed && out_ids && n_ids, "null argument"); ARGCHK(T > 0, "empty mel"); VOXCHK(ctx_bind(m->ctx));
    const vox_model_cfg& c = m->cfg; hipStream_t s = m->ctx->stream;
    const float* d_mel = mel;
    m->timings = vox_timings{};
    if (mem_kind == VOX_MEM_HOST) {
        VOXCHK(ensure(&m->d_mel, &m->mel_cap, (size_t)c.n_mels * T));
        HIPCHK(hipMemcpyAsync(m->d_mel, mel, (size_t)c.n_mels * T * 4, hipMemcpyHostToDevice, s)); d_mel = m->d_mel;
    }
    VOXCHK(transcribe_dev(m, d_mel, T, t_embed, out_ids, cap, n_ids, logits));
    m->timings.total_ms = m->timings.preprocess_ms + m->timings.encode_ms + m->timings.decode_ms;
    return VOX_OK;
}

extern "C" int32_t vox_transcribe_audio(vox_model* m, const float* samples, size_t n, const float* t_embed, int32_t* out_ids, int32_t cap,
                                        int32_t* n_ids, int32_t mem_kind) {
    ARGCHK(m && samples && t_embed && out_ids && n_ids, "null argument"); ARGCHK(n > 0, "empty audio"); VOXCHK(ctx_bind(m->ctx));
    const vox_model_cfg& c = m->cfg; vox_ctx* cx = m->ctx; hipStream_t s = cx->stream;
    ARGCHK(c.n_mels == 128, "the log-mel front-end produces 128 bins; model expects %d", c.n_mels);
    m->timings = vox_timings{};
    const double t0 = now_ms();
    const float* d_s = samples;
    if (mem_kind == VOX_MEM_HOST) {
        VOXCHK(ensure(&m->d_samples, &m->samples_cap, n));
        HIPCHK(hipMemcpyAsync(m->d_samples, samples, n * 4, hipMemcpyHostToDevice, s)); d_s = m->d_samples;
    }
    vox_pad_cfg pc; vox_pad_cfg_voxtral(&pc);
    const size_t left = pad_left(&pc), right = pad_right(&pc, n + left), total = left + n + right, T = total / 160;
    MelTables t; VOXCHK(ctx_mel_tables(cx, &t));
    VOXCHK(ensure(&m->d_mel, &m->mel_cap, (size_t)128 * T));
    HIPCHK(launch_absmax(d_s, (long)n, 0.95f, cx->d_scale, s));
    HIPCHK(launch_mel(d_s, (long)n, (long)left, (long)right, cx->d_scale, t, m->d_mel, (int)T, 1, s));
    HIPCHK(hipStreamSynchronize(s));
    m->timings.preprocess_ms = now_ms() - t0;
    VOXCHK(transcribe_dev(m, m->d_mel, (int)T, t_embed, out_ids, cap, n_ids, nullptr));
    m->timings.total_ms = m->timings.preprocess_ms + m->timings.encode_ms + m->timings.decode_ms;
    return VOX_OK;
}

static const int32_t VOX_RETRY_ON_LAUNCHES = -1000;
struct BatchDrain { vox_ctx* c; ~BatchDrain() { (void)hipStreamSynchronize(c->stream); if (c->fe_stream) (void)hipStreamSynchronize(c->fe_stream); } };
static int32_t batch_lengths(const vox_model* m, int n, const float* const* samples, const size_t* n_samples, const int32_t* caps, const int* slot_of,
                             std::vector<int>& T, std::vector<int>& S, std::vector<int>& len, int* Smax) {
    const int PREFIX_LEN = 38;
    vox_pad_cfg pc; vox_pad_cfg_voxtral(&pc);
    T.assign(n, 0); S.assign(n, 0); len.assign(n, 0); *Smax = 0;
    for (int i = 0; i < n; i++) {
        ARGCHK(samples[i] && n_samples[i] > 0, "empty audio in batch slot %d", slot_of[i]);
        const size_t left = pad_left(&pc), total = left + n_samples[i] + pad_right(&pc, n_samples[i] + left);
        T[i] = (int)(total / 160); S[i] = conv_len(conv_len(T[i])) / m->cfg.reshape_factor; *Smax = std::max(*Smax, S[i]);
        const int cnt_i = S[i] >= PREFIX_LEN ? std::max(S[i] - PREFIX_LEN, 1) : 0;
        ARGCHK(caps[i] >= cnt_i, "out_ids[%d] capacity %d < %d", slot_of[i], caps[i], cnt_i);
        len[i] = S[i] >= PREFIX_LEN ? std::max(S[i], PREFIX_LEN + 1) : 0;
    }
    ARGCHK(*Smax <= m->dec_rope_len, "sequence too long for the decoder RoPE table");
    return VOX_OK;
}
static int32_t front_end_units(const MelTables& mt, int i0, int nu, const float* const* samples, const size_t* n_samples, const int* T, const float* const* unit_scale,
                               float* smp, float* mel, float* scale, const float** d_mels, hipStream_t sf) {
    vox_pad_cfg pc; vox_pad_cfg_voxtral(&pc);
    size_t mo = 0, so = 0;
    for (int k = 0; k < nu; k++) {
        const int i = i0 + k; const float* d_s = samples[i];
        if (smp) { float* dst = smp + so; so += n_samples[i]; HIPCHK(hipMemcpyAsync(dst, samples[i], n_samples[i] * 4, hipMemcpyHostToDevice, sf)); d_s = dst; }
        const size_t left = pad_left(&pc), right = pad_right(&pc, n_samples[i] + left);
        float* mel_i = mel + mo; mo += (size_t)128 * T[i]; d_mels[k] = mel_i;
        if (!unit_scale) HIPCHK(launch_absmax(d_s, (long)n_samples[i], 0.95f, scale + k, sf));
        HIPCHK(launch_mel(d_s, (long)n_samples[i], (long)left, (long)right, unit_scale ? unit_scale[i] : scale + k, mt, mel_i, T[i], 1, sf));
    }
    return VOX_OK;
}
static int32_t upload_prefix(int n, int tstride, const std::vector<int>& len, int* d_tok, int* d_pos, int* d_len, hipStream_t s) {
    const int PREFIX_LEN = 38, BOS = 1, STREAMING_PAD = 32;
    std::vector<int32_t> prefix((size_t)n * tstride, 0); std::vector<int> pos0(n, PREFIX_LEN - 1);
    for (int i = 0; i < n; i++) { prefix[(size_t)i * tstride] = BOS; for (int r = 1; r < PREFIX_LEN; r++) prefix[(size_t)i * tstride + r] = STREAMING_PAD; }
    HIPCHK(hipMemcpyAsync(d_tok, prefix.data(), prefix.size() * 4, hipMemcpyHostToDevice, s)); HIPCHK(hipMemcpyAsync(d_pos, pos0.data(), (size_t)n * 4, hipMemcpyHostToDevice, s)); HIPCHK(hipMemcpyAsync(d_len, len.data(), (size_t)n * 4, hipMemcpyHostToDevice, s));
    HIPCHK(hipStreamSynchronize(s));
    return VOX_OK;
}
static int32_t copy_out_ids(int n, const std::vector<int>& S, int tstride, const int* d_tok, int32_t* const* out_ids, int32_t* n_ids, int* total, hipStream_t s) {
    const int PREFIX_LEN = 38;
    std::vector<int32_t> host_tok((size_t)n * tstride);
    HIPCHK(hipMemcpyAsync(host_tok.data(), d_tok, host_tok.size() * 4, hipMemcpyDeviceToHost, s));
    HIPCHK(hipStreamSynchronize(s)); *total = 0;
    for (int i = 0; i < n; i++) {
        const int cnt = S[i] >= PREFIX_LEN ? std::max(S[i] - PREFIX_LEN, 1) : 0;
        if (cnt > 0) std::memcpy(out_ids[i], host_tok.data() + (size_t)i * tstride + PREFIX_LEN, (size_t)cnt * 4);
        n_ids[i] = cnt; *total += cnt;
    }
    return VOX_OK;
}
static int32_t engb_timeout_check(vox_model* m, int n_blk, bool continuous, hipStream_t s) {
    for (int b = 0; b < n_blk; b++) { EngBParams ep{}; engb_state_carve(m->engb_state[b], &ep); HIPCHK(hipMemcpyAsync(m->engb_err_host[b], ep.err, 8, hipMemcpyDeviceToHost, s)); }
    HIPCHK(hipStreamSynchronize(s));
    for (int b = 0; b < n_blk; b++) if (m->engb_err_host[b][0]) {
        const unsigned e = m->engb_err_host[b][0];
        m->engb_strikes++;
        char grp[32] = ""; if (!continuous) snprintf(grp, sizeof grp, ", group %d", b);
        fprintf(stderr, "[voxtral_hip] batched decode engine%s: hand-off timeout (code %u, workgroup %u%s), strike %d of 3; re-running the %s on the launch-based step%s\n",
                continuous ? " (continuous batch)" : "", e & 0xff, (e >> 8) & 0xff, grp, m->engb_strikes, continuous ? "session" : "batch", m->engb_strikes >= 3 ? ", the engine is switched off" : "");
        for (int gj = 0; gj < 4; gj++) if (m->engb_state[gj]) (void)engb_state_init(m->engb_state[gj], s);
        if (m->engb_strikes >= 3) m->engb_ok = false;
        return VOX_RETRY_ON_LAUNCHES;
    }
    return VOX_OK;
}
struct StepGraphs {
    hipStream_t s; std::vector<std::pair<uint32_t, hipGraphExec_t>> ex; std::vector<hipGraph_t> gr;
    explicit StepGraphs(hipStream_t st) : s(st) {} StepGraphs(const StepGraphs&) = delete; StepGraphs& operator=(const StepGraphs&) = delete;
    ~StepGraphs() { (void)hipStreamSynchronize(s); for (auto& e : ex) if (e.second) (void)hipGraphExecDestroy(e.second); for (auto g : gr) if (g) (void)hipGraphDestroy(g); }
    hipGraphExec_t find(uint32_t a) const { for (auto& e : ex) if (e.first == a) return e.second; return nullptr; }
    template <class Step> int32_t capture(uint32_t act, Step& step, hipGraphExec_t* out) {
        HIPCHK(hipStreamBeginCapture(s, hipStreamCaptureModeThreadLocal));
        const int32_t r = step(act);
        hipGraph_t graph = nullptr;
        const hipError_t ce = hipStreamEndCapture(s, &graph);
        if (graph) gr.push_back(graph);
        if (r != VOX_OK) return r;
// ... 1235 lines not shown
```

voxtral-mini-realtime-rs_amd/csrc/vox_kernels.h:

```cpp
#pragma once
#include <hip/hip_runtime.h>
#include <atomic>
struct DevOnce {
    std::atomic<uint64_t> mask{0};
    bool done(int dev) const { return (mask.load(std::memory_order_acquire) >> (dev & 63)) & 1ull; }
    void set(int dev) { mask.fetch_or(1ull << (dev & 63), std::memory_order_release); }
};
static inline int vox_current_device() { int d = 0; if (hipGetDevice(&d) != hipSuccess) { (void)hipGetLastError(); d = 0; } return d; }
#include <stdint.h>

namespace vox {

struct Q4W {
    const uint4* qs;
    const uint16_t* sc;
    int N, K, nb;
    int fmt;
    const uint4* qt = nullptr; const uint16_t* st = nullptr;
};
enum WFmt { WFMT_Q4_0 = 0, WFMT_BF16 = 1, WFMT_BF16X2 = 2, WFMT_F32 = 3 };

enum Epi { EPI_STORE = 0, EPI_RESID = 1, EPI_SWIGLU = 2, EPI_ROPE_KV = 3, EPI_ARGMAX = 4, EPI_GELU = 5, EPI_SWIGLU_XF = 6, EPI_RESID_XF = 7,
           EPI_ROPE_ROWS = 8 };
enum Pro { PRO_NONE = 0, PRO_RMS = 1, PRO_RMS_MUL = 2,
// ... 11 lines not shown
    const int* pos_ptr; int pos_off;
    const float* rope_cos; const float* rope_sin; int hd;
    int n_q, n_k;
    float* kcache; float* vcache; int cache_head_stride;
    float* part_val; int* part_idx;
    int tl_slot;
};
hipError_t launch_q4_gemv(const GemvParams& p, int n_rows_x, int pro, int epi, int R, hipStream_t s);
const char* q4_gemv_kernel_name(int K, int pro, int epi, int R);
int q4_gemv_default_R(int N, int K, int epi);
int q4_gemv_grid(int N, int R);
int q4_gemv_nwv(int K, int epi);
int q4_gemv_grid_k(int N, int K, int R, int epi);
int dense_gemv_grid(int N);

struct GemmParams {
    Q4W w;
    const float* x; int x_stride; int M;
    float* out; int out_stride;
    const float* bias;
    const float* resid; int resid_stride;
    const uint4* xf;
    uint16_t* xf_scratch; size_t xf_scratch_bytes;
    const float* ssq_part; int n_part; float norm_eps;
    uint16_t* xf_out; const float* xf_w; const float* xf_w2; float* ssq_out;
    const int* pos; const float* rope_cos; const float* rope_sin; int hd, n_q, n_kv; float* kc; float* vc; long kv_seq_stride; int kv_head_stride;
    const int* kv_row;
    int tl_slot;
    int ksplit;
    float* kz_scratch; size_t kz_scratch_bytes;
    int rope_seq_rows;
    int wide_mt; long xf_gstride , xf_out_gstride , ssq_part_gstride, ssq_out_gstride ;
    int wide_rows;
};
struct WidePlan { int kz, sps, ntw; };
bool q4_wide_plan(const Q4W& w, int mt, int epi, WidePlan* pl);
size_t q4_wide_planes_bytes(const Q4W& w, int mt, const WidePlan& pl);
hipError_t launch_q4_wide(const GemmParams& p, int epi, hipStream_t s);
hipError_t launch_q4_tile_build(Q4W w, uint4* qt, uint16_t* st, hipStream_t s);
hipError_t launch_q4_gemm(const GemmParams& p, int epi, hipStream_t s, bool* fused_rope = nullptr);
hipError_t launch_dense2_gemm(const GemmParams& p, int epi, hipStream_t s);
hipError_t launch_transpose(const float* in, int R, int C, float* out, hipStream_t s);
int q4_skinny_resid_xf_parts(int N);

hipError_t launch_q4_repack(const uint8_t* raw, uint4* qs, uint16_t* sc, int64_t n_blocks, int nb, int row_mul, int row_add, hipStream_t s);
hipError_t launch_q4_dequant(Q4W w, float* out, hipStream_t s);
hipError_t launch_rms_norm(const float* x, int x_stride, int rows, int dim, const float* gamma, const float* mul,
                           float eps, float* out, int out_stride, hipStream_t s);
hipError_t launch_rms_norm_sumk(float* x, int x_stride, int rows, int dim, const float* part, size_t part_stride, int ksplit, const float* gamma, float eps, float* out, int out_stride, hipStream_t s);
int q4_skinny_mt2_plan(const Q4W& w, int M);
hipError_t launch_xf_rows(const float* x, int x_stride, int M, int K, uint16_t* xf, hipStream_t s);
hipError_t launch_q4_skinny_mt2_planes(const GemmParams& p, int KZ, hipStream_t s);
hipError_t launch_splitk_finish_resid(const float* planes, int KZ, int M, int N, float* x, int x_stride, hipStream_t s);
hipError_t launch_splitk_finish_swiglu_xf(const float* planes, int KZ, int M, int N, const float* bias, uint16_t* xf, hipStream_t s);
hipError_t launch_splitk_finish_rope_kv(const float* planes, int KZ, int M, int N, float* q_out, int q_stride, int n_q, int n_kv, int hd, int pos_off,
                                        const float* cos_t, const float* sin_t, float* kc, float* vc, int head_stride, hipStream_t s);
hipError_t launch_rms_norm_xf_sumk(float* x, int x_stride, int rows, int dim, const float* planes, int kz, const float* gamma, const float* mul, float eps, uint16_t* xf, hipStream_t s);
hipError_t launch_rms_norm_xf(const float* x, int x_stride, int rows, int dim, const float* gamma, const float* mul,
                              float eps, uint16_t* xf, hipStream_t s);
hipError_t launch_rope(float* buf, int M, int stride, int n_rot, int hd, int pos_off, const float* cos_t,
                       const float* sin_t, hipStream_t s, int seq_rows = 0, const int* row_pos = nullptr);
hipError_t launch_kv_store(const float* buf, int M, int stride, int k_col, int n_kv, int hd, int pos_off,
                           float* kcache, float* vcache, int cache_head_stride, hipStream_t s, int seq_rows = 0, long kv_seq_stride = 0);

struct AttnParams {
    const float* q; int q_stride;
    const float* k; const float* v;
    int kv_row_stride, kv_head_stride;
    float* out; int out_stride;
    int M, kv_len, n_heads, n_kv_heads, offset, window;
    const int* pos_ptr;
    int pos_per_seq; int q_seq_stride, out_seq_stride; long kv_seq_stride;
    const int* kv_row;
    const int* seq_len;
    const int* seq_row_off;
    uint16_t* out_xf_tiles; long out_xf_tile_stride;
    uint16_t* out_xf;
    long out_xf_gstride;
    int prefer_gqa;
    int no_xcd_remap;
    int tl_slot;
    int spec_zero;
    int spec_rows;
};
hipError_t launch_attn_prefill(const AttnParams& p, int hd, hipStream_t s, int n_seq = 1);
bool attn_prefill_small_ok(const AttnParams& p, int hd, int n_seq);
hipError_t launch_attn_decode(const AttnParams& p, int hd, int max_seq, hipStream_t s, int n_seq = 1);
bool attn_wo_supported(const AttnParams& p, const Q4W& wo, int hd, int max_seq);
hipError_t launch_attn_wo(const AttnParams& p, const Q4W& wo, long long* acc, int max_seq, hipStream_t s);
enum AttnForm { ATTN_FORM_PREFILL_SMALL, ATTN_FORM_PREFILL_MFMA, ATTN_FORM_PREFILL_F32, ATTN_FORM_DECODE, ATTN_FORM_DECODE_SPEC, ATTN_FORM_DECODE_GQA, ATTN_FORM_WO,
                ATTN_FORM_ENGINE, ATTN_FORM_COUNT };
void attn_form_note(AttnForm f);
void attn_form_counts(unsigned long long out[ATTN_FORM_COUNT]);
enum GemmForm { GEMM_FORM_GEMV_R1, GEMM_FORM_GEMV_R2, GEMM_FORM_GEMV_R4, GEMM_FORM_DENSE_GEMV, GEMM_FORM_SKINNY, GEMM_FORM_SKINNY_MT, GEMM_FORM_SKINNY_MT2, GEMM_FORM_XF_ROWS,
                GEMM_FORM_SPLITK_FINISH, GEMM_FORM_TILE_11, GEMM_FORM_TILE_12, GEMM_FORM_TILE_21, GEMM_FORM_TILE_22, GEMM_FORM_TILE_21_TB, GEMM_FORM_TILE_22_TB, GEMM_FORM_K32,
                GEMM_FORM_BIG, GEMM_FORM_BIG_ROPE, GEMM_FORM_DENSE2, GEMM_FORM_WIDE, GEMM_FORM_COUNT };
void gemm_form_counts(unsigned long long out[GEMM_FORM_COUNT]);

hipError_t launch_conv1d_gelu(const float* in, int Cin, int L, const float* w, const float* b, int Cout, float* out,
                              int out_token_major, hipStream_t s);

struct MelTables { const float* window; const float* cos_t; const float* sin_t; const float* fb; const int* fb_lo; const int* fb_hi; };
hipError_t launch_mel(const float* audio, long n, long left, long right, const float* scale_ptr, MelTables t,
                      float* out, int T, int transposed, hipStream_t s);
hipError_t launch_resample_matrix(const double* H, int new_len, int fft_in, int fft_out, float* At, hipStream_t s);
hipError_t launch_resample(const float* x, long n_in, const float* At, int fft_in, int fft_out, int delay, float* out, long n_out, hipStream_t s);
hipError_t launch_absmax(const float* x, long n, float target_peak, float* scale_out, hipStream_t s);
hipError_t launch_absmax_group(const float* x, long n, unsigned* group_max_cell, hipStream_t s);
hipError_t launch_group_scale(const unsigned* group_max, const int* unit_group, int n, float target, float* unit_scale, hipStream_t s);

hipError_t launch_embed(Q4W tok, const int* ids, int n, const float* audio, int D, const int* pos_ptr, int id_off,
                        int a_off, float* out, hipStream_t s);
hipError_t launch_argmax_final(const float* part_val, const int* part_idx, int n_parts, int* tokens, int* pos_ptr,
                               int tok_off, int inc, hipStream_t s);
hipError_t launch_argmax_embed(const float* part_val, const int* part_idx, int n_parts, int* tokens, int* pos_ptr, Q4W tok,
                               const float* audio, int D, float* h, hipStream_t s);
hipError_t launch_rope_kv_batch(float* qkv, int n, int stride, int n_q, int n_kv, int hd, const int* pos, const float* cos_t, const float* sin_t,
                                float* kcache, float* vcache, long seq_stride, int head_stride, hipStream_t s);
hipError_t launch_argmax_embed_batch(const float* logits, int n, int vocab, int* tokens, int tok_stride, int* pos, const int* seq_len, Q4W tok,
                                     const float* audio, long audio_seq_stride, int D, float* h, hipStream_t s,
                                     uint16_t* xf = nullptr, const float* xf_w = nullptr, float* ssq_out = nullptr,
                                     long xf_group_stride = 0, int ssq_group_stride = 0,
                                     const long* audio_off = nullptr);
struct SlotStepParams {
    const float* logits; int vocab;
    int* tokens; int tok_stride; const int* clip_len;
    int* slot_clip; int* slot_qpos; const int* queue; int q_stride;
    int* pos; int* kv_row; int n_clips; int first_pos;
    Q4W tok; const float* audio; const long* audio_off; int D;
    const float* h0;
    float* h;
    uint16_t* xf; const float* xf_w; float* ssq_out; long xf_group_stride; int ssq_group_stride;
    int init;
};
hipError_t launch_argmax_embed_slots(const SlotStepParams& p, int n_slots, hipStream_t s);
struct BatchTapParams {
    const float* logits; int vocab;
    const int* slot_clip; int clip0; const int* pos; const int* seq_len;
    const int* clip_unit; int n_clips;
    float* out; int* rows; int n_units, max_rows, first_pos;
};
hipError_t launch_batch_tap(const BatchTapParams& p, int n_rows, hipStream_t s);
hipError_t launch_occupy(int workgroups, int micros, hipStream_t s);
hipError_t launch_add_rows(const float* a, const float* b, float* out, long n, hipStream_t s);
hipError_t launch_gelu(float* x, long n, hipStream_t s);
hipError_t launch_argmax_rows(const float* x, int rows, int V, int* out, hipStream_t s);

struct EngLayerTab { const float* attn_norm; const float* ffn_norm; const float* ada_mul; float* kc; float* vc; };
struct EngParams {
    const unsigned char* stream; size_t cu_stride;
    const EngLayerTab* layers; int n_layers;
    const float* h_in;
    const float* final_norm;
    const int* pos_ptr; int pos_off;
    const float* rope_cos; const float* rope_sin;
    int max_seq, window; float eps;
    unsigned long long *H0, *H1, *G, *PW, *A, *P2;
    unsigned long long *SS0, *SS1;
    unsigned long long* XC;
    unsigned* serial; unsigned* err;
    float* part_val; int* part_idx;
    int* tokens; int* pos_rw; const uint4* tok_qs; const uint16_t* tok_sc; int tok_nb; const float* audio;
    float* logits_out;
    int vocab;
    unsigned long long* tl; int tl_layer;
    int flags;
    int ag_delay_ticks;
    int pace_ticks;
// ... 58 lines not shown
```

voxtral-mini-realtime-rs_amd/csrc/vox_kernels.hip:

```cpp
#include "vox_kernels.h"

#include <hip/hip_fp16.h>

#include <unistd.h>

#include <algorithm>
#include <atomic>
#include <cstdio>
#include <cstdlib>
#include <cstring>
#include <string>
#include <mutex>
#include <unordered_map>

namespace vox {

static int g_tl_next = -1, g_tl_slots = 0;
#ifdef VOX_TIMELINE
__device__ unsigned long long* g_tl_buf = nullptr;
__device__ int g_tl_waves = 0;
__device__ __forceinline__ void tl_stamp(int slot, int wave_global, int k) {
    if (slot >= 0 && (wave_global & 3) == 0 && (threadIdx.x & 63) == 0 && g_tl_buf && wave_global < g_tl_waves)
        g_tl_buf[((size_t)slot * g_tl_waves + wave_global) * 4 + k] = wall_clock64();
}
// ... 2397 lines not shown
    const bool q_ok = m < p.M;
    const int pos = p.offset + (q_ok ? m : (p.M - 1));
    const float scale = 1.0f / sqrtf((float)HD);

    float qv[DP], o[DP];
    {
        const float* qp = p.q + (size_t)(q_ok ? m : 0) * p.q_stride + h * HD + part * DP;
#pragma unroll
        for (int e = 0; e < DP; e += 4) {
            const float4 v = *reinterpret_cast<const float4*>(qp + e);
            qv[e] = v.x; qv[e + 1] = v.y; qv[e + 2] = v.z; qv[e + 3] = v.w;
        }
#pragma unroll
        for (int e = 0; e < DP; e++) o[e] = 0.f;
    }
    float mx = -INFINITY, l = 0.f;

    const int last_m = min(m0 + 63, p.M - 1);
    int j_lo = 0;
    if (p.window >= 0) j_lo = max(0, p.offset + m0 - p.window);
    const int j_hi = min(p.kv_len - 1, p.offset + last_m);
    const float* kbase = p.k + (size_t)kvh * p.kv_head_stride;
    const float* vbase = p.v + (size_t)kvh * p.kv_head_stride;

    for (int j0 = (j_lo / 64) * 64; j0 <= j_hi; j0 += 64) {
        __syncthreads();
        for (int i = tid; i < 64 * (HD / 4); i += 256) {
            const int jj = i / (HD / 4), d4 = i % (HD / 4), j = j0 + jj;
            const int jc = min(j, p.kv_len - 1);
            float4 kk = *reinterpret_cast<const float4*>(kbase + (size_t)jc * p.kv_row_stride + d4 * 4);
            float4 vv = *reinterpret_cast<const float4*>(vbase + (size_t)jc * p.kv_row_stride + d4 * 4);
            reinterpret_cast<float4*>(Ks)[i] = kk;
            reinterpret_cast<float4*>(Vs)[i] = vv;
        }
        __syncthreads();
        for (int jj = 0; jj < 64; jj += 4) {
            float sc[4];
#pragma unroll
            for (int kk = 0; kk < 4; kk++) {
                const float* kr = Ks + (jj + kk) * HD + part * DP;
                float s = 0.f;
#pragma unroll
                for (int e = 0; e < DP; e += 4) {
                    const float4 kv = *reinterpret_cast<const float4*>(kr + e);
                    s = fmaf(qv[e], kv.x, s); s = fmaf(qv[e + 1], kv.y, s); s = fmaf(qv[e + 2], kv.z, s); s = fmaf(qv[e + 3], kv.w, s);
                }
                s += __shfl_xor(s, 16, 64); s += __shfl_xor(s, 32, 64);
                const int j = j0 + jj + kk;
                bool vis = (j < p.kv_len) && (j <= pos);
                if (p.window >= 0) vis = vis && (pos - j <= p.window);
                sc[kk] = vis ? s * scale : -INFINITY;
            }
            const float mnew = fmaxf(fmaxf(fmaxf(sc[0], sc[1]), fmaxf(sc[2], sc[3])), mx);
            if (mnew > -INFINITY) {
                const float alpha = expf(mx - mnew);
                float pr[4];
#pragma unroll
                for (int kk = 0; kk < 4; kk++) pr[kk] = expf(sc[kk] - mnew);
                l = l * alpha + ((pr[0] + pr[1]) + (pr[2] + pr[3]));
#pragma unroll
                for (int e = 0; e < DP; e++) o[e] *= alpha;
#pragma unroll
                for (int kk = 0; kk < 4; kk++) {
                    const float* vr = Vs + (jj + kk) * HD + part * DP;
#pragma unroll
                    for (int e = 0; e < DP; e += 4) {
                        const float4 vv = *reinterpret_cast<const float4*>(vr + e);
                        o[e] = fmaf(pr[kk], vv.x, o[e]); o[e + 1] = fmaf(pr[kk], vv.y, o[e + 1]);
                        o[e + 2] = fmaf(pr[kk], vv.z, o[e + 2]); o[e + 3] = fmaf(pr[kk], vv.w, o[e + 3]);
                    }
                }
                mx = mnew;
            }
        }
    }
    if (q_ok) {
        float* op = p.out + (size_t)m * p.out_stride + h * HD + part * DP;
        const float inv = 1.0f / l;
#pragma unroll
        for (int e = 0; e < DP; e += 4)
            *reinterpret_cast<float4*>(op + e) = make_float4(o[e] * inv, o[e + 1] * inv, o[e + 2] * inv, o[e + 3] * inv);
    }
}
template <int HD>
__global__ __launch_bounds__(256) __attribute__((amdgpu_waves_per_eu(2))) void attn_prefill_mfma_kernel(const AttnParams p) {
    constexpr int KS = HD / 32, DT = HD / 16, KROW = HD + 8, VROW = 72;
    extern __shared__ __attribute__((aligned(16))) uint16_t smh[];
    uint16_t* Kh = smh;
    uint16_t* Kl = Kh + 64 * KROW;
    uint16_t* Vh = Kl + 64 * KROW;
    uint16_t* Vl = Vh + HD * VROW;
    const int tid = threadIdx.x, lane = tid & 63, wave = tid >> 6, c = lane & 15, g = lane >> 4;
    int bx = blockIdx.x, h = blockIdx.y, sq = blockIdx.z;
    {
        const int nblk = gridDim.x, pairs = gridDim.y * gridDim.z;
        if (nblk > 1 && pairs % 8 == 0) {
            const int lin = (blockIdx.z * gridDim.y + blockIdx.y) * nblk + blockIdx.x, xcd = lin & 7, slot = lin >> 3;
            const int pair = xcd * (pairs >> 3) + slot / nblk;
            bx = slot % nblk; h = pair % (int)gridDim.y; sq = pair / (int)gridDim.y;
        }
    }
    const int kvh = h / (p.n_heads / p.n_kv_heads);
    const int M = p.seq_len ? p.seq_len[sq] : p.M, kv_len = p.seq_len ? p.offset + M : p.kv_len;
    const int m0 = ((int)gridDim.x - 1 - bx) * 64;
    if (m0 >= M) return;
    const int m = m0 + wave * 16 + c;
    const int mq = min(m, M - 1);
    const int pos = p.offset + mq;
    const int wave_pos_hi = p.offset + min(m0 + wave * 16 + 15, M - 1);
    const float scale = 1.0f / sqrtf((float)HD);

    bf16x8 qh[KS], ql[KS];
    {
        const float* qp = p.q + (p.seq_row_off ? (size_t)p.seq_row_off[sq] * p.q_stride : (size_t)sq * p.q_seq_stride) + (size_t)mq * p.q_stride + h * HD + 8 * g;
#pragma unroll
        for (int ks = 0; ks < KS; ks++) {
            const float4 a = *reinterpret_cast<const float4*>(qp + ks * 32), b = *reinterpret_cast<const float4*>(qp + ks * 32 + 4);
            uint4 hi, lo; split_bf16x8(a, b, hi, lo); qh[ks] = as_bf16x8(hi); ql[ks] = as_bf16x8(lo);
        }
    }
    f32x4 o[DT];
#pragma unroll
    for (int dt = 0; dt < DT; dt++) o[dt] = (f32x4){0.f, 0.f, 0.f, 0.f};
    float mx = -INFINITY, lsum = 0.f;

    const int last_m = min(m0 + 63, M - 1);
    int j_lo = 0;
    if (p.window >= 0) j_lo = max(0, p.offset + m0 - p.window);
    const int j_hi = min(kv_len - 1, p.offset + last_m);
    const size_t kvso = p.seq_row_off ? (size_t)p.seq_row_off[sq] * p.kv_row_stride : (size_t)sq * p.kv_seq_stride;
    const float* kbase = p.k + kvso + (size_t)kvh * p.kv_head_stride;
    const float* vbase = p.v + kvso + (size_t)kvh * p.kv_head_stride;

    constexpr int NK = (64 * (HD / 4)) / 256, NV = (32 * (HD / 4)) / 256;
    float4 kreg[NK], vra[NV], vrb[NV];
#define VOX_ATT_LOAD(J0_)                                                                                           \
    _Pragma("unroll") for (int u = 0; u < NK; u++) {                                                                \
        const int i = tid + 256 * u, key = i / (HD / 4), d4 = i % (HD / 4);                                         \
        const int jc = min((J0_) + key, kv_len - 1);      \
        kreg[u] = *reinterpret_cast<const float4*>(kbase + (size_t)jc * p.kv_row_stride + d4 * 4);                  \
    }                                                                                                               \
    _Pragma("unroll") for (int u = 0; u < NV; u++) {                                                                \
        const int i = tid + 256 * u, kp = i / (HD / 4), d4 = i % (HD / 4);                                          \
        const int ja = min((J0_) + 2 * kp, kv_len - 1), jb = min((J0_) + 2 * kp + 1, kv_len - 1);               \
        vra[u] = *reinterpret_cast<const float4*>(vbase + (size_t)ja * p.kv_row_stride + d4 * 4);                   \
        vrb[u] = *reinterpret_cast<const float4*>(vbase + (size_t)jb * p.kv_row_stride + d4 * 4);                   \
    }
    const int j_first = (j_lo / 64) * 64, j_last = (j_hi / 64) * 64;
    VOX_ATT_LOAD(j_first)
    for (int j0 = j_first; j0 <= j_hi; j0 += 64) {
        __syncthreads();
#pragma unroll
        for (int u = 0; u < NK; u++) {
            const int i = tid + 256 * u, key = i / (HD / 4), d4 = i % (HD / 4);
            uint2 hi, lo; split_pair(kreg[u].x, kreg[u].y, hi.x, lo.x); split_pair(kreg[u].z, kreg[u].w, hi.y, lo.y);
            *reinterpret_cast<uint2*>(Kh + key * KROW + d4 * 4) = hi;
            *reinterpret_cast<uint2*>(Kl + key * KROW + d4 * 4) = lo;
        }
#pragma unroll
        for (int u = 0; u < NV; u++) {
            const int i = tid + 256 * u, kp = i / (HD / 4), d4 = i % (HD / 4);
            const float4 va = vra[u], vb = vrb[u];
            uint32_t hi, lo;
            split_pair(va.x, vb.x, hi, lo); *reinterpret_cast<uint32_t*>(Vh + (d4 * 4 + 0) * VROW + 2 * kp) = hi; *reinterpret_cast<uint32_t*>(Vl + (d4 * 4 + 0) * VROW + 2 * kp) = lo;
            split_pair(va.y, vb.y, hi, lo); *reinterpret_cast<uint32_t*>(Vh + (d4 * 4 + 1) * VROW + 2 * kp) = hi; *reinterpret_cast<uint32_t*>(Vl + (d4 * 4 + 1) * VROW + 2 * kp) = lo;
            split_pair(va.z, vb.z, hi, lo); *reinterpret_cast<uint32_t*>(Vh + (d4 * 4 + 2) * VROW + 2 * kp) = hi; *reinterpret_cast<uint32_t*>(Vl + (d4 * 4 + 2) * VROW + 2 * kp) = lo;
            split_pair(va.w, vb.w, hi, lo); *reinterpret_cast<uint32_t*>(Vh + (d4 * 4 + 3) * VROW + 2 * kp) = hi; *reinterpret_cast<uint32_t*>(Vl + (d4 * 4 + 3) * VROW + 2 * kp) = lo;
        }
        __syncthreads();
        { const int jn = min(j0 + 64, j_last); VOX_ATT_LOAD(jn) }
        __builtin_amdgcn_sched_barrier(0);
        if (j0 > wave_pos_hi) continue;

        f32x4 sc[4];
#pragma unroll
        for (int kt = 0; kt < 4; kt++) {
            sc[kt] = (f32x4){0.f, 0.f, 0.f, 0.f};
            if (j0 + kt * 16 <= wave_pos_hi) {
#pragma unroll
                for (int ks = 0; ks < KS; ks++) {
                    const bf16x8 ah = as_bf16x8(*reinterpret_cast<const uint4*>(Kh + (kt * 16 + c) * KROW + ks * 32 + 8 * g));
                    const bf16x8 al = as_bf16x8(*reinterpret_cast<const uint4*>(Kl + (kt * 16 + c) * KROW + ks * 32 + 8 * g));
                    sc[kt] = __builtin_amdgcn_mfma_f32_16x16x32_bf16(ah, qh[ks], sc[kt], 0, 0, 0);
                    sc[kt] = __builtin_amdgcn_mfma_f32_16x16x32_bf16(ah, ql[ks], sc[kt], 0, 0, 0);
                    sc[kt] = __builtin_amdgcn_mfma_f32_16x16x32_bf16(al, qh[ks], sc[kt], 0, 0, 0);
                }
            }
        }
        float mt = -INFINITY;
#pragma unroll
        for (int kt = 0; kt < 4; kt++)
#pragma unroll
            for (int r = 0; r < 4; r++) {
                const int j = j0 + kt * 16 + 4 * g + r;
                bool vis = (j < kv_len) && (j <= pos);
                if (p.window >= 0) vis = vis && (pos - j <= p.window);
                const float v = vis ? sc[kt][r] * scale : -INFINITY;
                sc[kt][r] = v; mt = fmaxf(mt, v);
            }
        mt = fmaxf(mt, __shfl_xor(mt, 16, 64)); mt = fmaxf(mt, __shfl_xor(mt, 32, 64));
        const float mnew = fmaxf(mx, mt);
        const float msafe = (mnew == -INFINITY) ? 0.f : mnew;
        const float alpha = __expf(mx - msafe);
        float ps = 0.f;
#pragma unroll
        for (int kt = 0; kt < 4; kt++)
#pragma unroll
            for (int r = 0; r < 4; r++) { const float e = __expf(sc[kt][r] - msafe); sc[kt][r] = e; ps += e; }
        lsum = lsum * alpha + ps; mx = mnew;
#pragma unroll
        for (int dt = 0; dt < DT; dt++) { o[dt][0] *= alpha; o[dt][1] *= alpha; o[dt][2] *= alpha; o[dt][3] *= alpha; }
#pragma unroll
        for (int kk = 0; kk < 2; kk++) {
            if (j0 + kk * 32 <= wave_pos_hi) {
                uint4 ph, pl;
                split_pair(sc[2 * kk][0], sc[2 * kk][1], ph.x, pl.x); split_pair(sc[2 * kk][2], sc[2 * kk][3], ph.y, pl.y);
                split_pair(sc[2 * kk + 1][0], sc[2 * kk + 1][1], ph.z, pl.z); split_pair(sc[2 * kk + 1][2], sc[2 * kk + 1][3], ph.w, pl.w);
                const bf16x8 bh = as_bf16x8(ph), bl = as_bf16x8(pl);
#pragma unroll
                for (int dt = 0; dt < DT; dt++) {
                    const uint16_t* vh = Vh + (dt * 16 + c) * VROW + kk * 32 + 4 * g;
                    const uint16_t* vl = Vl + (dt * 16 + c) * VROW + kk * 32 + 4 * g;
                    const uint2 h0 = *reinterpret_cast<const uint2*>(vh), h1 = *reinterpret_cast<const uint2*>(vh + 16);
                    const uint2 l0 = *reinterpret_cast<const uint2*>(vl), l1 = *reinterpret_cast<const uint2*>(vl + 16);
                    const bf16x8 ah = as_bf16x8(make_uint4(h0.x, h0.y, h1.x, h1.y)), al = as_bf16x8(make_uint4(l0.x, l0.y, l1.x, l1.y));
                    o[dt] = __builtin_amdgcn_mfma_f32_16x16x32_bf16(ah, bh, o[dt], 0, 0, 0);
                    o[dt] = __builtin_amdgcn_mfma_f32_16x16x32_bf16(ah, bl, o[dt], 0, 0, 0);
                    o[dt] = __builtin_amdgcn_mfma_f32_16x16x32_bf16(al, bh, o[dt], 0, 0, 0);
                }
            }
        }
    }
#undef VOX_ATT_LOAD
    lsum += __shfl_xor(lsum, 16, 64); lsum += __shfl_xor(lsum, 32, 64);
    if (m < M) {
        const float inv = 1.0f / lsum;
        float* op = p.out + (p.seq_row_off ? (size_t)p.seq_row_off[sq] * p.out_stride : (size_t)sq * p.out_seq_stride) + (size_t)m * p.out_stride + h * HD + 4 * g;
#pragma unroll
        for (int dt = 0; dt < DT; dt++)
            *reinterpret_cast<float4*>(op + dt * 16) = make_float4(o[dt][0] * inv, o[dt][1] * inv, o[dt][2] * inv, o[dt][3] * inv);
    }
}
template <int HD>
static hipError_t attn_prefill_mfma_launch(const AttnParams& p, hipStream_t s, int n_seq) {
    constexpr size_t lds = ((size_t)2 * 64 * (HD + 8) + (size_t)2 * HD * 72) * sizeof(uint16_t);
    auto kern = attn_prefill_mfma_kernel<HD>;
    static DevOnce attr_done;
    hipError_t e = ensure_dyn_lds(kern, lds, &attr_done);
    if (e != hipSuccess) return e;
    kern<<<dim3((p.M + 63) / 64, p.n_heads, n_seq), dim3(256), lds, s>>>(p);
    attn_form_note(ATTN_FORM_PREFILL_MFMA);
    return hipGetLastError();
}
template <int HD>
__global__ __launch_bounds__(256) void attn_prefill_small_kernel(const AttnParams p) {
    constexpr int KROW = HD + 4, MAXR = 48;
    extern __shared__ __attribute__((aligned(16))) float sms[];
    float* Ks = sms; float* Vs = Ks + MAXR * KROW; float* Qs = Vs + MAXR * HD; float* Ps = Qs + 4 * HD;
    const int tid = threadIdx.x, lane = tid & 63, wave = tid >> 6;
    const int h = blockIdx.x, sq = blockIdx.y, kvh = h / (p.n_heads / p.n_kv_heads);
    const int M = p.seq_len ? p.seq_len[sq] : p.M;
    const int r = 4 * (int)blockIdx.z + wave;
    const int n_keys = min(M, 4 * (int)blockIdx.z + 4);
    if (4 * (int)blockIdx.z >= M) {
        if (p.out_xf_tiles && lane < 32) xf_store4(p.out_xf_tiles + (size_t)(r >> 4) * p.out_xf_tile_stride, p.n_heads * HD, r & 15, h * HD + 4 * lane, make_float4(0.f, 0.f, 0.f, 0.f));
        return;
    }
    const size_t kvso = (size_t)sq * p.kv_seq_stride;
    const float* kbase = p.k + kvso + (size_t)kvh * p.kv_head_stride; const float* vbase = p.v + kvso + (size_t)kvh * p.kv_head_stride;
    for (int i = tid; i < n_keys * (HD / 4); i += 256) {
        const int j = i / (HD / 4), d4 = i % (HD / 4);
        *reinterpret_cast<float4*>(Ks + j * KROW + 4 * d4) = *reinterpret_cast<const float4*>(kbase + (size_t)j * p.kv_row_stride + 4 * d4);
        *reinterpret_cast<float4*>(Vs + j * HD + 4 * d4) = *reinterpret_cast<const float4*>(vbase + (size_t)j * p.kv_row_stride + 4 * d4);
    }
    float* qs = Qs + wave * HD; float* ps = Ps + wave * 64;
    if (r < M) { const float* qp = p.q + (size_t)sq * p.q_seq_stride + (size_t)r * p.q_stride + h * HD; for (int d = lane; d < HD; d += 64) qs[d] = qp[d]; }
    __syncthreads();
    const float scale = 1.0f / sqrtf((float)HD);
    float4 o = make_float4(0.f, 0.f, 0.f, 0.f);
    if (r < M) {
        const float* kr = Ks + min(lane, n_keys - 1) * KROW;
        float s0 = 0.f, s1 = 0.f, s2 = 0.f, s3 = 0.f;
#pragma unroll 8
        for (int d = 0; d < HD; d += 4) {
            const float4 kv = *reinterpret_cast<const float4*>(kr + d), qv = *reinterpret_cast<const float4*>(qs + d);
            s0 = fmaf(qv.x, kv.x, s0); s1 = fmaf(qv.y, kv.y, s1); s2 = fmaf(qv.z, kv.z, s2); s3 = fmaf(qv.w, kv.w, s3);
        }
        const bool vis = lane <= r && (p.window < 0 || r - lane <= p.window);
        const float sc = vis ? ((s0 + s1) + (s2 + s3)) * scale : -INFINITY;
        const float mx = wave_max(sc);
        const float e = vis ? expf(sc - mx) : 0.f;
        const float sum = wave_sum(e);
        ps[lane] = e / sum;
        __builtin_amdgcn_wave_barrier();
        const int c = lane & 31, half = lane >> 5;
        for (int j = half; j <= r; j += 2) {
            const float pj = ps[j]; const float4 vv = *reinterpret_cast<const float4*>(Vs + j * HD + 4 * c);
            o.x = fmaf(pj, vv.x, o.x); o.y = fmaf(pj, vv.y, o.y); o.z = fmaf(pj, vv.z, o.z); o.w = fmaf(pj, vv.w, o.w);
        }
        o.x += __shfl_xor(o.x, 32, 64); o.y += __shfl_xor(o.y, 32, 64); o.z += __shfl_xor(o.z, 32, 64); o.w += __shfl_xor(o.w, 32, 64);
    }
    if (lane < 32) {
        const int col = h * HD + 4 * lane;
        if (p.out_xf_tiles) xf_store4(p.out_xf_tiles + (size_t)(r >> 4) * p.out_xf_tile_stride, p.n_heads * HD, r & 15, col, o);
        else if (r < M) *reinterpret_cast<float4*>(p.out + (size_t)sq * p.out_seq_stride + (size_t)r * p.out_stride + col) = o;
    }
}
bool attn_prefill_small_ok(const AttnParams& p, int hd, int n_seq) {
    return hd == 128 && p.M >= 1 && p.M <= 48 && p.offset == 0 && p.kv_len == p.M && !p.seq_row_off && (p.window < 0 || p.window >= p.M) && (p.q_stride % 4) == 0 && (p.kv_row_stride % 4) == 0 &&
           n_seq == 1  &&
           !env_int("VOX_ATTN_F32");
}
static hipError_t attn_prefill_small_launch(const AttnParams& p, hipStream_t s, int n_seq) {
    constexpr int HD = 128;
    const size_t lds = (size_t)(48 * (HD + 4) + 48 * HD + 4 * HD + 4 * 64) * sizeof(float);
    auto kern = attn_prefill_small_kernel<HD>; static DevOnce done;
    hipError_t e = ensure_dyn_lds(kern, lds, &done); if (e != hipSuccess) return e;
    const int rows = p.out_xf_tiles ? ((p.M + 15) / 16) * 16 : p.M;
    kern<<<dim3(p.n_heads, n_seq, (rows + 3) / 4), dim3(256), lds, s>>>(p);
    attn_form_note(ATTN_FORM_PREFILL_SMALL);
    return hipGetLastError();
}
hipError_t launch_attn_prefill(const AttnParams& p, int hd, hipStream_t s, int n_seq) {
    if (attn_prefill_small_ok(p, hd, n_seq)) return attn_prefill_small_launch(p, s, n_seq);
    if (p.out_xf_tiles) return hipErrorInvalidValue;
    const int f32_only = env_int("VOX_ATTN_F32");
    if (!f32_only && (p.q_stride % 4) == 0 && (p.kv_row_stride % 4) == 0) {
        if (hd == 64) return attn_prefill_mfma_launch<64>(p, s, n_seq);
        if (hd == 128) return attn_prefill_mfma_launch<128>(p, s, n_seq);
    }
    if (n_seq != 1 || p.seq_len) return hipErrorInvalidValue;
    dim3 grid((p.M + 63) / 64, p.n_heads);
    const size_t lds = (size_t)2 * 64 * hd * sizeof(float);
    if (hd == 64) {
        attn_prefill_kernel<64><<<grid, dim3(256), lds, s>>>(p);
    } else if (hd == 128) {
        auto kern = attn_prefill_kernel<128>;
        static DevOnce attr_done;
        hipError_t e = ensure_dyn_lds(kern, lds, &attr_done);
        if (e != hipSuccess) return e;
        kern<<<grid, dim3(256), lds, s>>>(p);
    } else return hipErrorInvalidValue;
    attn_form_note(ATTN_FORM_PREFILL_F32);
    return hipGetLastError();
}

template <bool NT>
__device__ __forceinline__ float4 ldf4(const float* p) {
    if (NT) { const u32x4_t v = __builtin_nontemporal_load(reinterpret_cast<const u32x4_t*>(p)); return make_float4(__uint_as_float(v.x), __uint_as_float(v.y), __uint_as_float(v.z), __uint_as_float(v.w)); }
    return *reinterpret_cast<const float4*>(p);
}
template <int HD, bool NT, bool LATE_V, bool SPEC, class Hook>
__device__ __forceinline__ float4 attn_decode_core(const float* __restrict__ qh, const float* __restrict__ kb, const float* __restrict__ vb, int kv_row_stride,
                                                   int pos_in, int window, float* __restrict__ sc, float* __restrict__ red, float4* __restrict__ osum, int tl_slot, int tlw,
                                                   int spec_rows, Hook after_issue) {
    static_assert(HD == 128 || HD == 64, "head_dim");
    constexpr int PER = HD / 8;
    const int tid = threadIdx.x, lane = tid & 63, wave = tid >> 6;
    const float scale = 1.0f / sqrtf((float)HD);
    const int ks = tid >> 3, part = tid & 7;
    (void)tl_slot; (void)tlw;
    float qv[PER];
#pragma unroll
    for (int e = 0; e < PER; e += 4) {
        const float4 v = ldf4<NT>(qh + part * PER + e);
        qv[e] = v.x; qv[e + 1] = v.y; qv[e + 2] = v.z; qv[e + 3] = v.w;
    }
    constexpr int NPRE = LATE_V ? 4 : 5, COLS = HD / 4, GROUPS = 256 / COLS;
    static_assert(4 * GROUPS == 32 || HD != 128, "prefetch tiling assumes 32 keys per P.V iteration for HD = 128");
    const int grp = tid / COLS, col = tid % COLS;
    float4 kpre[NPRE][PER / 4], vpre[NPRE][4];
#define VOX_KPRE(ROW_)                                                                                        \
    _Pragma("unroll") for (int u = 0; u < NPRE; u++) {                                                        \
        const int jc = (ROW_);                                                                                \
        const float* kr = kb + (size_t)jc * kv_row_stride + part * PER;                                       \
        _Pragma("unroll") for (int e = 0; e < PER / 4; e++) kpre[u][e] = ldf4<NT>(kr + 4 * e);                \
    }
#define VOX_VPRE_AT(ROW_)                                                                                     \
    _Pragma("unroll") for (int u = 0; u < NPRE; u++)                                                          \
        _Pragma("unroll") for (int w = 0; w < 4; w++) {                                                       \
            const int iv = u * 4 * GROUPS + grp + w * GROUPS;                                                 \
            vpre[u][w] = ldf4<NT>(vb + (size_t)(ROW_) * kv_row_stride + col * 4);                             \
        }
#define VOX_VPRE VOX_VPRE_AT(j_lo + min(iv, n - 1))
    static_assert(!SPEC || !LATE_V, "speculative rows: K and V are both requested up front");
    if (SPEC) {
        VOX_KPRE(min(32 * u + ks, spec_rows - 1))
        VOX_VPRE_AT(min(iv, spec_rows - 1))
        __builtin_amdgcn_sched_barrier(0);
    }
    const int pos = SPEC ? __builtin_amdgcn_readfirstlane(pos_in) : pos_in;
    const int len = pos + 1;
    const int j_lo = window >= 0 ? max(0, pos - window) : 0;
    const int n = len - j_lo;
    if (SPEC) {
        if (j_lo != 0) {
            VOX_KPRE(j_lo + min(32 * u + ks, n - 1))
            VOX_VPRE
        }
    } else {
        VOX_KPRE(j_lo + min(32 * u + ks, n - 1))
        if (!LATE_V) { VOX_VPRE }
    }
    __builtin_amdgcn_sched_barrier(0);
    after_issue();
    __builtin_amdgcn_sched_barrier(0);
#undef VOX_KPRE
#pragma unroll
    for (int u = 0; u < NPRE; u++) {
        float s = 0.f;
#pragma unroll
        for (int e = 0; e < PER / 4; e++) {
// ... 929 lines not shown
```

voxtral-mini-realtime-rs_amd/gguf.py:

```python
from __future__ import annotations

import ctypes as C
import weakref

import numpy as np

from . import _lib
from ._lib import check, lib, VoxError

F32, F16, Q4_0 = 0, 1, 2


def _f32(a):
    return np.ascontiguousarray(a, dtype=np.float32)


def _ptr(a):
    return a.ctypes.data_as(C.c_void_p)


class Context:

    def __init__(self, device: int = 0):
        self.h = C.c_void_p()
# ... 306 lines not shown
        out = np.empty_like(x2)
        check(lib().vox_forward_hidden_with_cache(self._m.h, _ptr(x2), x2.shape[0], _ptr(_f32(t_embed).reshape(-1)), caches.h, _ptr(out)))
        return out.reshape(shp)

    def lm_head(self, hidden):
        h = _f32(hidden); shp = h.shape; h2 = h.reshape(-1, self.d_model())
        out = np.empty((h2.shape[0], self._m.config.vocab), dtype=np.float32)
        check(lib().vox_lm_head(self._m.h, _ptr(h2), h2.shape[0], _ptr(out)))
        return out.reshape(shp[:-1] + (self._m.config.vocab,))


    def embed_tokens_from_ids_dev(self, ids, out_ptr):
        ids = np.ascontiguousarray(ids, dtype=np.int32).reshape(-1)
        check(lib().vox_embed_tokens_from_ids_ex(self._m.h, _ptr(ids), ids.size, C.c_void_p(out_ptr), 1))

    def forward_hidden_with_cache_dev(self, x_ptr, rows, t_embed, caches: LayerCaches, out_ptr=None):
        ws = C.c_void_p()
        check(lib().vox_forward_hidden_with_cache_ex(self._m.h, C.c_void_p(x_ptr), rows, _ptr(_f32(t_embed).reshape(-1)), caches.h,
                                                     None if out_ptr is None else C.c_void_p(out_ptr), C.byref(ws), 1))
        return ws.value

    def lm_head_dev(self, hidden_ptr, rows, logits_ptr):
        check(lib().vox_lm_head_ex(self._m.h, C.c_void_p(hidden_ptr), rows, C.c_void_p(logits_ptr), 1))

    def lm_head_argmax(self, hidden_ptr, rows):
        ids = np.zeros(rows, dtype=np.int32)
        check(lib().vox_lm_head_argmax(self._m.h, C.c_void_p(hidden_ptr), rows, _ptr(ids), 1))
        return ids


def tensor_add_dev(ctx, a_ptr, b_ptr, n, out_ptr):
    check(lib().vox_tensor_add(ctx.h, C.c_void_p(a_ptr), C.c_void_p(b_ptr), n, C.c_void_p(out_ptr), 1))


def argmax_rows_dev(ctx, logits_ptr, rows, vocab):
    ids = np.zeros(rows, dtype=np.int32)
    check(lib().vox_argmax_rows(ctx.h, C.c_void_p(logits_ptr), rows, vocab, _ptr(ids), 1))
    return ids


class Q4VoxtralModel:

    def __init__(self, ctx, h):
        self.ctx, self.h = ctx, h
        self._caches = weakref.WeakSet()
        self.config = _lib.ModelCfg(); check(lib().vox_model_config(h, C.byref(self.config)))

    def decoder(self):
        return Q4LanguageModel(self)

    def create_decoder_cache_preallocated(self, max_seq):
        return LayerCaches(self, max_seq)

    def generate_step_with_cache(self, token_ids, t_embed, caches):
        ids = np.ascontiguousarray(token_ids, dtype=np.int32).reshape(-1)
        out = np.empty((ids.size, self.config.vocab), dtype=np.float32)
        check(lib().vox_generate_step_with_cache(self.h, _ptr(ids), ids.size, _ptr(_f32(t_embed).reshape(-1)), caches.h, _ptr(out)))
        return out

    def _mel2(self, mel):
        mel = _f32(mel); return mel.reshape(mel.shape[-2], mel.shape[-1])

    def forward(self, mel, t_embed):
        mel = self._mel2(mel); T = mel.shape[1]; cap = T // 16 + 2
        out = np.empty((cap, self.config.vocab), dtype=np.float32); S = C.c_int32()
        check(lib().vox_forward(self.h, _ptr(mel), T, _ptr(_f32(t_embed).reshape(-1)), _ptr(out), cap, C.byref(S), 0))
        return out[:S.value][None].copy()

    def forward_streaming(self, mel, token_ids, t_embed):
        mel = self._mel2(mel); T = mel.shape[1]; cap = T // 16 + 2
        ids = np.ascontiguousarray(token_ids, dtype=np.int32).reshape(-1)
        out = np.empty((cap, self.config.vocab), dtype=np.float32); S = C.c_int32()
        check(lib().vox_forward_streaming(self.h, _ptr(mel), T, _ptr(ids), ids.size, _ptr(_f32(t_embed).reshape(-1)), _ptr(out), cap, C.byref(S), 0))
        return out[:S.value][None].copy()

    def forward_with_cache(self, mel, t_embed, encoder_cache, decoder_cache):
        mel = self._mel2(mel); T = mel.shape[1]; cap = T // 16 + 2
        out = np.empty((cap, self.config.vocab), dtype=np.float32); S = C.c_int32()
        check(lib().vox_forward_with_cache(self.h, _ptr(mel), T, _ptr(_f32(t_embed).reshape(-1)), encoder_cache.h, decoder_cache.h, _ptr(out), cap, C.byref(S), 0))
        return out[:S.value][None].copy()

    def set_decode_engine(self, on: bool) -> bool:
        a = C.c_int32(); check(lib().vox_model_set_decode_engine(self.h, 1 if on else 0, C.byref(a))); return bool(a.value)

    def memory(self):
        v = (C.c_uint64 * 4)(); check(lib().vox_model_memory(self.h, v)); return {"arena": v[0], "arena_primary": v[1], "engine_stream": v[2], "engine_state": v[3]}

    def set_batch_engine(self, on=None):
        a = C.c_int32(); n = C.c_uint64()
        check(lib().vox_model_set_batch_engine(self.h, -1 if on is None else (1 if on else 0), C.byref(a), C.byref(n))); return bool(a.value), int(n.value)

    def weight_bytes(self):
        v = C.c_uint64(); check(lib().vox_model_weight_bytes(self.h, C.byref(v))); return v.value

    def arena(self):
        p = C.c_void_p(); n = C.c_uint64(); check(lib().vox_model_arena(self.h, C.byref(p), C.byref(n)))
        return p.value, n.value

    def replicate(self, dst_ctx):
        h = C.c_void_p(); check(lib().vox_model_replicate(self.h, dst_ctx.h, C.byref(h)))
        return type(self)(dst_ctx, h)

    def set_sessions(self, sessions: int):
        check(lib().vox_model_set_sessions(self.h, int(sessions)))

    def arena_finalize(self):
        check(lib().vox_model_arena_finalize(self.h))

    def encode_audio(self, mel):
        mel = _f32(mel); mel = mel.reshape(mel.shape[-2], mel.shape[-1]); T = mel.shape[1]
        cap = T // 16 + 2
        out = np.empty((cap, self.config.dec_dim), dtype=np.float32); S = C.c_int32()
        check(lib().vox_encode_audio(self.h, _ptr(mel), T, _ptr(out), cap, C.byref(S), 0))
        return out[:S.value].reshape(1, S.value, self.config.dec_dim).copy()

    def debug_encode_batch(self, mels, layout):
        arrs = [_f32(x) for x in mels]; arrs = [np.ascontiguousarray(a.reshape(a.shape[-2], a.shape[-1])) for a in arrs]; n = len(arrs)
        Ts = [a.shape[1] for a in arrs]
        cap = sum(T // 16 + 2 for T in Ts)
        D = self.config.dec_dim
        out = np.zeros((cap, D), dtype=np.float32); rows = (C.c_int32 * max(n, 1))(); rep = (C.c_int64 * 4)()
        ptrs = (C.c_void_p * max(n, 1))(*[a.ctypes.data for a in arrs])
        check(lib().vox_debug_encode_batch(self.h, n, ptrs, (C.c_int32 * max(n, 1))(*Ts), layout, _ptr(out), cap, rows, rep))
        res, o = [], 0
        for i in range(n):
            res.append(out[o:o + rows[i]].copy()); o += rows[i]
        return res, {"Mtot": rep[0], "ksp": rep[1], "ksp_wo": rep[2], "fused_rope": rep[3]}

    def create_encoder_cache(self, capacity_rows=0):
        return EncoderCaches(self, capacity_rows)

    def encode_audio_with_cache(self, mel, encoder_cache):
        mel = _f32(mel); mel = mel.reshape(mel.shape[-2], mel.shape[-1]); T = mel.shape[1]
        cap = T // 16 + 2
        out = np.empty((cap, self.config.dec_dim), dtype=np.float32); S = C.c_int32()
        check(lib().vox_encode_audio_with_cache(self.h, _ptr(mel), T, encoder_cache.h, _ptr(out), cap, C.byref(S), 0))
        return out[:S.value].reshape(1, S.value, self.config.dec_dim).copy()

    def transcribe_streaming(self, mel, t_embed, return_logits=False):
        mel = _f32(mel); mel = mel.reshape(mel.shape[-2], mel.shape[-1]); T = mel.shape[1]
        cap = T // 16 + 2
        ids = np.zeros(cap, dtype=np.int32); n = C.c_int32()
        t = _f32(t_embed).reshape(-1)
        lg = np.empty((cap, self.config.vocab), dtype=np.float32) if return_logits else None
        check(lib().vox_transcribe_streaming(self.h, _ptr(mel), T, _ptr(t), _ptr(ids), cap, C.byref(n),
                                             None if lg is None else _ptr(lg), 0))
        if return_logits:
            return ids[:n.value].copy(), lg[:n.value].copy()
        return ids[:n.value].copy()

    def transcribe_audio(self, samples, t_embed, device_ptr=None, n_samples=None):
        t = _f32(t_embed).reshape(-1)
        if device_ptr is None:
            x = _f32(samples); n_samples = x.size; ptr = _ptr(x); kind = 0
        else:
            ptr = C.c_void_p(device_ptr); kind = 1
        cap = n_samples // 1280 + 128
        ids = np.zeros(cap, dtype=np.int32); n = C.c_int32()
        check(lib().vox_transcribe_audio(self.h, ptr, n_samples, _ptr(t), _ptr(ids), cap, C.byref(n), kind))
        return ids[:n.value].copy()

    def transcribe_batch(self, samples_list, t_embed, device_ptrs=None, n_samples=None, norm_group=None, tap_units=None):
        t = _f32(t_embed).reshape(-1)
        if device_ptrs is None:
            arrs = [_f32(x) for x in samples_list]; n = len(arrs)
            ptrs = (C.c_void_p * n)(*[a.ctypes.data for a in arrs]); lens = (C.c_size_t * n)(*[a.size for a in arrs]); kind = 0
# ... 80 lines not shown
```

Measured before the change: 1447.

## Cache encoder and decoder state for the constant left-padding prefix

Adds a per-model prefix cache. It precomputes the encoder K/V and adapter audio rows for the silent left-pad region, plus the decoder KV cache for the BOS/streaming-pad prefix tokens. Later transcriptions skip those rows: the encoder runs only on the remaining rows, and a new templated MFMA attention path reads the cached prefix K/V. Decoding then starts from the copied prefix KV instead of re-prefilling it. This removes repeated, input-independent prefix work. The cost is extra device memory, and correctness depends on the prefix being truly independent of the audio, which the code invalidates when t_embed changes.

```diff
diff --git a/include/voxtral_hip.h b/include/voxtral_hip.h
--- a/include/voxtral_hip.h
+++ b/include/voxtral_hip.h
@@ -123,6 +123,8 @@
 
 int32_t vox_model_set_t_embed(vox_model* m, const float* t_embed_host);
 int32_t vox_model_set_decode_engine(vox_model* m, int32_t on, int32_t* active_or_null);
+int32_t vox_model_set_prefix_cache(vox_model* m, int32_t on, int32_t* active_or_null);
+int32_t vox_model_prefix_info(const vox_model* m, int32_t out[4]);
 int32_t vox_model_set_batch_engine(vox_model* m, int32_t on, int32_t* active_or_null, uint64_t* launches_or_null);
 
 int32_t vox_encode_audio(vox_model* m, const float* mel_128xT, int32_t T, float* out, int32_t cap_rows,
diff --git a/voxtral-mini-realtime-rs_amd/_lib.py b/voxtral-mini-realtime-rs_amd/_lib.py
--- a/voxtral-mini-realtime-rs_amd/_lib.py
+++ b/voxtral-mini-realtime-rs_amd/_lib.py
@@ -98,6 +98,8 @@
     "vox_model_arena": (i32, [vp, P(vp), P(u64)]),
     "vox_model_set_t_embed": (i32, [vp, vp]),
     "vox_model_set_decode_engine": (i32, [vp, i32, P(i32)]),
+    "vox_model_set_prefix_cache": (i32, [vp, i32, P(i32)]),
+    "vox_model_prefix_info": (i32, [vp, P(i32 * 4)]),
     "vox_debug_occupy": (i32, [vp, i32, i32]),
     "vox_model_memory": (i32, [vp, P(C.c_uint64)]),
     "vox_model_set_batch_engine": (i32, [vp, i32, P(i32), P(C.c_uint64)]),
diff --git a/voxtral-mini-realtime-rs_amd/csrc/vox_api.cpp b/voxtral-mini-realtime-rs_amd/csrc/vox_api.cpp
--- a/voxtral-mini-realtime-rs_amd/csrc/vox_api.cpp
+++ b/voxtral-mini-realtime-rs_amd/csrc/vox_api.cpp
@@ -701,7 +701,20 @@
 static bool cache_alive(const vox_cache* k, uint64_t gen) { std::lock_guard<std::mutex> l(g_cache_mu); auto it = g_cache_live.find(k); return it != g_cache_live.end() && it->second == gen; }
 
 struct TensorMeta { std::vector<uint64_t> shape; int dtype = 0; uint64_t nbytes = 0; };
+struct PrefixState {
+    bool on = true;
+    int RC = 0, PC = 0;
+    float* enc_kv = nullptr;
+    float* audio = nullptr;
+    float *dec_k = nullptr, *dec_v = nullptr;
+    bool enc_built = false, dec_built = false;
+    std::vector<float> t_embed;
+    float* capture = nullptr; int capture_rows = 0;
+    uint64_t enc_bytes = 0, dec_bytes = 0;
+};
+static const int VOX_PREFIX_TOKENS = 38, VOX_TOK_BOS = 1, VOX_TOK_STREAMING_PAD = 32;
 struct vox_model {
+    PrefixState pfx;
     vox_ctx* ctx = nullptr; vox_model_cfg cfg{};
     std::vector<vox_model*> twins;
     std::map<std::string, TensorMeta> manifest; bool is_q4 = false;
@@ -1119,6 +1132,11 @@
         if (m->graph[i]) { (void)hipGraphDestroy(m->graph[i]); m->graph[i] = nullptr; }
     }
 }
+static void prefix_release(vox_model* m) {
+    PrefixState& p = m->pfx;
+    for (float** q : {&p.enc_kv, &p.audio, &p.dec_k, &p.dec_v}) { if (*q) (void)hipFree(*q); *q = nullptr; }
+    p.enc_built = p.dec_built = false; p.enc_bytes = p.dec_bytes = 0; p.t_embed.clear();
+}
 static void model_release(vox_model* m) {
     if (!m) return;
     for (vox_model* t : m->twins) { vox_ctx* tc = t->ctx; model_release(t); (void)vox_ctx_destroy(tc); }
@@ -1131,6 +1149,7 @@
                     (void*)m->d_h, (void*)m->d_h2, (void*)m->d_wo_acc, (void*)m->d_q, (void*)m->d_att, (void*)m->d_act, (void*)m->d_logits, (void*)m->d_part_val, (void*)m->d_part_idx, (void*)m->d_seq_len, (void*)m->d_seq_off, (void*)m->d_row_pos, (void*)m->d_prefix, (void*)m->enc_cos_s, (void*)m->enc_sin_s, (void*)m->eng_stream, (void*)m->eng_wob, (void*)m->eng_state, (void*)m->eng_tab, (void*)m->engb_state[0], (void*)m->engb_state[1], (void*)m->engb_state[2], (void*)m->engb_state[3],
                     (void*)m->engb_tab[0], (void*)m->engb_tab[1], (void*)m->engb_tab[2], (void*)m->engb_tab[3], (void*)m->pw_x, (void*)m->pw_hidden, (void*)m->pw_logits, (void*)m->pw_part_val, (void*)m->pw_part_idx, (void*)m->pw_ids, (void*)m->pw_zero, (void*)m->pw_tab})
         if (p) (void)hipFree(p);
+    prefix_release(m);
     if (m->pw_err_pin) (void)hipHostFree(m->pw_err_pin);
     if (m->tap.out) (void)hipFree(m->tap.out);
     if (m->tap.rows) (void)hipFree(m->tap.rows);
@@ -1222,6 +1241,7 @@
     for (Q4W* w : m->tiled) HIPCHK(launch_q4_tile_build(*w, const_cast<uint4*>(w->qt), const_cast<uint16_t*>(w->st), m->ctx->stream));
     HIPCHK(hipStreamSynchronize(m->ctx->stream));
     m->eng_ready = false; m->eng_tab_cache = nullptr;
+    prefix_release(m);
     if (m->eng_wob) { HIPCHK(hipStreamSynchronize(m->ctx->stream)); (void)hipFree(m->eng_wob); m->eng_wob = nullptr; }
     graphs_destroy(m);
     return VOX_OK;
@@ -1259,6 +1279,7 @@
     }
     HIPCHK(hipStreamSynchronize(cx->stream));
     m->t_embed_host.assign(t_embed, t_embed + c.dec_dim); m->t_embed_set = true;
+    m->pfx.dec_built = false;
     return VOX_OK;
 }
 
@@ -1301,7 +1322,7 @@
 static long enc_packed_rows(const vox_model* m, const int* T, int n) { long r = 0; for (int i = 0; i < n; i++) r += enc_packed_rows_of(m, T[i]); return r; }
 struct EncForms { long Mtot = 0; int ksp = 0, ksp_wo = 0, fused_rope = 0; };
 static int32_t encode_batch_dev(vox_model* m, int n, const float* const* d_mels, const int* T, float* audio_out, int audio_rows, int* S4_out, long* audio_off_out = nullptr,
-                                EncForms* forms = nullptr) {
+                                EncForms* forms = nullptr, int prefix_rows = 0) {
     const vox_model_cfg& c = m->cfg; vox_ctx* cx = m->ctx; hipStream_t s = cx->stream;
     const int D = c.enc_dim, H = c.enc_heads, hd = c.enc_head_dim, QD = H * hd, F = c.enc_ffn, R = c.reshape_factor;
     const bool packed = audio_off_out != nullptr;
@@ -1314,7 +1335,11 @@
     ARGCHK(S_pad <= m->enc_rope_len, "audio too long for the encoder RoPE table (%d > %d positions); chunk it (--max-mel-frames)", S_pad, m->enc_rope_len);
     std::vector<int> roff(n + 1, 0);
     if (packed) for (int i = 0; i < n; i++) roff[i + 1] = roff[i] + enc_packed_rows_of(m, T[i]);
-    const int Mtot = packed ? roff[n] : n * S_pad, M4 = packed ? Mtot / R : n == 1 ? S4_out[0] : Mtot / R;
+    const int r0 = prefix_rows;
+    ARGCHK(r0 == 0 || (n == 1 && !packed && r0 % R == 0 && r0 < S_pad && m->pfx.enc_built && r0 == m->pfx.RC), "internal: encoder prefix of %d rows", r0);
+    const int Mfull = packed ? roff[n] : n * S_pad;
+    const int Mtot = Mfull - r0, M4 = packed ? Mtot / R : n == 1 ? S4_out[0] - r0 / R : Mtot / R;
+    ARGCHK(!m->pfx.capture || (n == 1 && !packed && r0 == 0 && m->pfx.capture_rows <= S_pad), "internal: prefix capture");
     ARGCHK(packed || n == 1 || audio_rows >= S_pad / R, "internal: audio row budget %d < %d", audio_rows, S_pad / R);
     int Tmax = 0; for (int i = 0; i < n; i++) Tmax = std::max(Tmax, T[i]);
     (void)T1max;
@@ -1331,10 +1356,10 @@
     int ksp_wo = ksp ? 2 : 0;
     if (ksp) { if (const char* e = knob_str("VOX_ENC_SPLITK_WO")) ksp_wo = atoi(e) > 1 ? std::min(atoi(e), ksp) : 0; }
     for (int l = 0; ksp_wo && l < c.enc_layers; l++) if (m->enc[l].wo.w.fmt != WFMT_Q4_0 || !m->enc[l].wo.w.qt || m->enc[l].wo.w.nb / 4 < ksp_wo || m->enc[l].wo.w.nb % 4) ksp_wo = 0;
-    const size_t need = c1_floats + (size_t)Mtot * D * 2 + (size_t)Mtot * QD * 4 + (size_t)Mtot * F + (size_t)(M4 + 1) * m->ad0.w.N + (size_t)ksp * Mtot * D + 1024;
+    const size_t need = c1_floats + (size_t)Mfull * D + (size_t)Mtot * D + (size_t)Mtot * QD * 4 + (size_t)Mtot * F + (size_t)(M4 + 1) * m->ad0.w.N + (size_t)ksp * Mtot * D + 1024;
     VOXCHK(ensure(&m->ws, &m->ws_floats, need));
     if (forms) { forms->Mtot = Mtot; forms->ksp = ksp; forms->ksp_wo = ksp_wo; forms->fused_rope = 0; }
-    float* c1 = m->ws; float* x = c1 + c1_floats / 64 * 64; float* xn = x + (size_t)Mtot * D; float* qkv = xn + (size_t)Mtot * D;
+    float* c1 = m->ws; float* x0 = c1 + c1_floats / 64 * 64; float* x = x0 + (size_t)r0 * D; float* xn = x0 + (size_t)Mfull * D; float* qkv = xn + (size_t)Mtot * D;
     float* att = qkv + (size_t)Mtot * QD * 3; float* ffn = att + (size_t)Mtot * QD; float* ah = ffn + (size_t)Mtot * F; float* w2p = ah + (size_t)(M4 + 1) * m->ad0.w.N;
     const int* d_len = nullptr; const int* d_roff = nullptr; const int* d_rpos = nullptr;
     if (n > 1 || packed) {
@@ -1357,7 +1382,7 @@
     }
     for (int i = 0; i < n; i++) {
         if (S[i] <= 0) continue;
-        VOXCHK(conv_stem_dev(m, d_mels[i], T[i], c1, x + (packed ? (size_t)roff[i] : (size_t)i * S_pad) * D));
+        VOXCHK(conv_stem_dev(m, d_mels[i], T[i], c1, x0 + (packed ? (size_t)roff[i] : (size_t)i * S_pad) * D));
     }
     const int seq_rows = packed ? 0 : n > 1 ? S_pad : 0;
     for (int l = 0; l < c.enc_layers; l++) {
@@ -1366,15 +1391,20 @@
         else HIPCHK(launch_rms_norm(x, D, Mtot, D, L.attn_norm, nullptr, c.norm_eps, xn, D, s));
         if (Mtot > 48) {
             GemmParams g{}; g.w = L.wqkv.w; g.x = xn; g.x_stride = D; g.M = Mtot; g.out = qkv; g.out_stride = 3 * QD; g.bias = L.wqkv.bias;
-            g.rope_cos = m->enc_cos; g.rope_sin = m->enc_sin; g.hd = hd; g.n_q = 2 * QD; g.pos = d_rpos; g.rope_seq_rows = seq_rows;
+            g.rope_cos = m->enc_cos + (size_t)r0 * (hd / 2); g.rope_sin = m->enc_sin + (size_t)r0 * (hd / 2);
+            g.hd = hd; g.n_q = 2 * QD; g.pos = d_rpos; g.rope_seq_rows = seq_rows;
             bool fused = false; HIPCHK(launch_q4_gemm(g, EPI_ROPE_ROWS, s, &fused));
             if (forms && fused) forms->fused_rope++;
         } else {
             VOXCHK(q4_linear_dev(cx, L.wqkv.w, L.wqkv.bias, xn, D, Mtot, qkv, 3 * QD));
-            HIPCHK(launch_rope(qkv, Mtot, 3 * QD, 2 * QD, hd, 0, m->enc_cos, m->enc_sin, s, seq_rows, d_rpos));
-        }
+            HIPCHK(launch_rope(qkv, Mtot, 3 * QD, 2 * QD, hd, r0, m->enc_cos, m->enc_sin, s, seq_rows, d_rpos));
+        }
+        if (m->pfx.capture)
+            HIPCHK(hipMemcpy2DAsync(m->pfx.capture + (size_t)l * m->pfx.capture_rows * 2 * QD, (size_t)2 * QD * 4, qkv + QD, (size_t)3 * QD * 4, (size_t)2 * QD * 4, (size_t)m->pfx.capture_rows,
+                                    hipMemcpyDeviceToDevice, s));
         AttnParams ap{}; ap.q = qkv; ap.q_stride = 3 * QD; ap.k = qkv + QD; ap.v = qkv + 2 * QD; ap.kv_row_stride = 3 * QD; ap.kv_head_stride = hd;
-        ap.out = att; ap.out_stride = QD; ap.M = S_pad; ap.kv_len = S_pad; ap.n_heads = H; ap.n_kv_heads = H; ap.offset = 0; ap.window = c.enc_window;
+        ap.out = att; ap.out_stride = QD; ap.M = S_pad - r0; ap.kv_len = S_pad; ap.n_heads = H; ap.n_kv_heads = H; ap.offset = r0; ap.window = c.enc_window;
+        if (r0) { ap.prefix_k = m->pfx.enc_kv + (size_t)l * r0 * 2 * QD; ap.prefix_v = ap.prefix_k + QD; ap.prefix_len = r0; ap.prefix_row_stride = 2 * QD; ap.prefix_head_stride = hd; }
         ap.seq_len = d_len; ap.q_seq_stride = S_pad * 3 * QD; ap.out_seq_stride = S_pad * QD; ap.kv_seq_stride = (long)S_pad * 3 * QD; ap.seq_row_off = d_roff;
         HIPCHK(launch_attn_prefill(ap, hd, s, n));
         if (ksp_wo) {
@@ -1392,15 +1422,15 @@
     else HIPCHK(launch_rms_norm(x, D, Mtot, D, m->enc_norm, nullptr, c.norm_eps, xn, D, s));
     VOXCHK(q4_linear_dev(cx, m->ad0.w, nullptr, xn, D * R, M4, ah, m->ad0.w.N, EPI_GELU));
     if (packed) { for (int i = 0; i < n; i++) audio_off_out[i] = (long)(roff[i] / R) * c.dec_dim; }
-    if (packed || n == 1 || audio_rows * R == S_pad) VOXCHK(q4_linear_dev(cx, m->ad2.w, nullptr, ah, m->ad0.w.N, M4, audio_out, c.dec_dim));
+    if (packed || n == 1 || audio_rows * R == S_pad) VOXCHK(q4_linear_dev(cx, m->ad2.w, nullptr, ah, m->ad0.w.N, M4, audio_out + (size_t)(r0 / R) * c.dec_dim, c.dec_dim));
     else for (int i = 0; i < n; i++)
         VOXCHK(q4_linear_dev(cx, m->ad2.w, nullptr, ah + (size_t)i * (S_pad / R) * m->ad0.w.N, m->ad0.w.N, S_pad / R, audio_out + (size_t)i * audio_rows * c.dec_dim, c.dec_dim));
     return VOX_OK;
 }
-static int32_t encode_dev(vox_model* m, const float* d_mel, int T, int* S4_out) {
+static int32_t encode_dev(vox_model* m, const float* d_mel, int T, int* S4_out, int prefix_rows = 0) {
     const int S4 = enc_rows(T) / m->cfg.reshape_factor;
     if (S4 > 0) { size_t cap = (size_t)m->audio_cap * m->cfg.dec_dim; VOXCHK(ensure(&m->d_audio, &cap, (size_t)S4 * m->cfg.dec_dim)); m->audio_cap = (int)(cap / m->cfg.dec_dim); }
-    return encode_batch_dev(m, 1, &d_mel, &T, m->d_audio, S4, S4_out);
+    return encode_batch_dev(m, 1, &d_mel, &T, m->d_audio, S4, S4_out, nullptr, nullptr, prefix_rows);
 }
 
 static int32_t cache_alloc(vox_model* m, int max_seq, vox_cache** out) {
@@ -1809,6 +1839,91 @@
     return VOX_OK;
 }
 
+static void prefix_bounds(const vox_model* m, int* RC, int* PC) {
+    const vox_model_cfg& c = m->cfg; *RC = 0; *PC = 0;
+    vox_pad_cfg pc; vox_pad_cfg_voxtral(&pc);
+    const long left = (long)pad_left(&pc), R = c.reshape_factor;
+    if (left < 200 || R < 1 || c.n_mels != 128 || (c.enc_head_dim != 64 && c.enc_head_dim != 128) || m->enc.empty() || m->dec.empty()) return;
+    const long Fc = (left - 200) / 160, rows = Fc >= 3 ? (Fc - 3) / 4 + 1 : 0;
+    const long pcn = VOX_PREFIX_TOKENS - 1;
+    if (rows / R < pcn || pcn * R + 4 > m->enc_rope_len) return;
+    *PC = (int)pcn; *RC = (int)(pcn * R);
+}
+static bool prefix_active(const vox_model* m) { int rc, pc; prefix_bounds(m, &rc, &pc); return m->pfx.on && rc > 0; }
+static int32_t prefix_build(vox_model* m, const float* t_embed) {
+    PrefixState& p = m->pfx; const vox_model_cfg& c = m->cfg; vox_ctx* cx = m->ctx; hipStream_t s = cx->stream;
+    int RC, PC; prefix_bounds(m, &RC, &PC);
+    if (!p.on || RC <= 0) return VOX_OK;
+    if (p.enc_built && p.dec_built && p.t_embed.size() == (size_t)c.dec_dim && !std::memcmp(p.t_embed.data(), t_embed, (size_t)c.dec_dim * 4)) return VOX_OK;
+    const int QD = c.enc_heads * c.enc_head_dim, hd = c.dec_head_dim, KV = c.dec_kv_heads;
+    p.RC = RC; p.PC = PC;
+    const size_t rows_bytes = (size_t)PC * hd * 4, n_rows = (size_t)c.dec_layers * KV;
+    {
+        hipError_t e = hipSuccess;
+        auto A = [&](float** q, size_t n) { if (e == hipSuccess && !*q) e = hipMalloc((void**)q, n); };
+        A(&p.enc_kv, (size_t)c.enc_layers * RC * 2 * QD * 4); A(&p.audio, (size_t)PC * c.dec_dim * 4); A(&p.dec_k, rows_bytes * n_rows); A(&p.dec_v, rows_bytes * n_rows);
+        if (e != hipSuccess) {
+            (void)hipGetLastError(); prefix_release(m); p.on = false;
+            fprintf(stderr, "[voxtral_hip] prefix state: allocating %.1f MB failed (%s); every call runs the full computation\n",
+                    ((double)c.enc_layers * RC * 2 * QD * 4 + 2.0 * rows_bytes * n_rows) / 1e6, hipGetErrorString(e));
+            return VOX_OK;
+        }
+    }
+    if (!p.enc_built) {
+        const int Tb = 4 * (RC + 4);
+        p.enc_bytes = (uint64_t)c.enc_layers * RC * 2 * QD * 4 + (uint64_t)PC * c.dec_dim * 4;
+        MelTables t; VOXCHK(ctx_mel_tables(cx, &t));
+        DevBuf mel; HIPCHK(mel.alloc((size_t)c.n_mels * Tb * 4));
+        HIPCHK(launch_mel(nullptr, 0, (long)Tb * 160, 0, nullptr, t, mel.as<float>(), Tb, 1, s));
+        int S4 = 0; p.capture = p.enc_kv; p.capture_rows = RC;
+        const int32_t r = encode_dev(m, mel.as<float>(), Tb, &S4);
+        p.capture = nullptr; p.capture_rows = 0;
+        VOXCHK(r); ARGCHK(S4 >= PC, "internal: prefix build gave %d audio rows", S4);
+        HIPCHK(hipMemcpyAsync(p.audio, m->d_audio, (size_t)PC * c.dec_dim * 4, hipMemcpyDeviceToDevice, s));
+        HIPCHK(hipStreamSynchronize(s));
+        p.enc_built = true;
+    }
+    VOXCHK(vox_model_set_t_embed(m, t_embed));
+    VOXCHK(ensure_decode_state(m, VOX_PREFIX_TOKENS));
+    p.dec_bytes = 2 * (uint64_t)rows_bytes * n_rows;
+    std::vector<int32_t> prefix(VOX_PREFIX_TOKENS, VOX_TOK_STREAMING_PAD); prefix[0] = VOX_TOK_BOS;
+    HIPCHK(hipMemcpyAsync(m->d_tokens, prefix.data(), prefix.size() * 4, hipMemcpyHostToDevice, s));
+    if (!m->d_prefix) HIPCHK(hipMalloc((void**)&m->d_prefix, (size_t)VOX_PREFIX_TOKENS * c.dec_dim * 4));
+    HIPCHK(launch_embed(m->tok.w, m->d_tokens, PC, p.audio, c.dec_dim, nullptr, 0, 0, m->d_prefix, s));
+    m->cache->len = 0;
+    VOXCHK(decoder_prefill_dev(m, m->d_prefix, PC, m->cache, 0));
+    const size_t pitch = (size_t)m->cache->max_seq * hd * 4;
+    ARGCHK(cache_layer_floats(m, m->cache) == (size_t)KV * m->cache->max_seq * hd, "internal: cache layout");
+    HIPCHK(hipMemcpy2DAsync(p.dec_k, rows_bytes, m->cache->k, pitch, rows_bytes, n_rows, hipMemcpyDeviceToDevice, s));
+    HIPCHK(hipMemcpy2DAsync(p.dec_v, rows_bytes, m->cache->v, pitch, rows_bytes, n_rows, hipMemcpyDeviceToDevice, s));
+    HIPCHK(hipStreamSynchronize(s));
+    p.t_embed.assign(t_embed, t_embed + c.dec_dim); p.dec_built = true;
+    return VOX_OK;
+}
+static bool prefix_usable(const vox_model* m, int T) {
+    const PrefixState& p = m->pfx; const vox_model_cfg& c = m->cfg;
+    if (!p.on || !p.enc_built || !p.dec_built || p.RC <= 0 || knob_str("VOX_ATTN_F32")) return false;
+    const int S = enc_rows(T);
+    return S / c.reshape_factor > VOX_PREFIX_TOKENS && S <= m->enc_rope_len;
+}
+extern "C" int32_t vox_model_set_prefix_cache(vox_model* m, int32_t on, int32_t* active) {
+    ARGCHK(m, "null argument"); VOXCHK(ctx_bind(m->ctx));
+    if (on >= 0) {
+        m->pfx.on = on != 0;
+        if (!m->pfx.on) { HIPCHK(hipStreamSynchronize(m->ctx->stream)); prefix_release(m); }
+        else if (m->t_embed_set) { std::vector<float> te = m->t_embed_host; VOXCHK(prefix_build(m, te.data())); }
+    }
+    if (active) *active = prefix_active(m) ? 1 : 0;
+    return VOX_OK;
+}
+extern "C" int32_t vox_model_prefix_info(const vox_model* m, int32_t out[4]) {
+    ARGCHK(m && out, "null argument");
+    int rc, pc; prefix_bounds(m, &rc, &pc);
+    const uint64_t b = (m->pfx.enc_kv ? m->pfx.enc_bytes : 0) + (m->pfx.dec_k ? m->pfx.dec_bytes : 0);
+    out[0] = m->pfx.enc_built && m->pfx.dec_built ? 1 : 0; out[1] = rc; out[2] = pc; out[3] = (int32_t)std::min<uint64_t>(b, 0x7fffffff);
+    return VOX_OK;
+}
+
 static int32_t decode_step_enqueue(vox_model* m, float* logits_out, int mode = 0) {
     const vox_model_cfg& c = m->cfg; hipStream_t s = m->ctx->stream;
     if (mode != 0) { HIPCHK(launch_decode_engine(engine_params(m, logits_out, mode == 2), s)); return VOX_OK; }
@@ -1824,14 +1939,16 @@
 }
 
 static int32_t transcribe_dev(vox_model* m, const float* d_mel, int T, const float* t_embed, int32_t* out_ids, int32_t cap, int32_t* n_ids,
-                              float* logits_host) {
+                              float* logits_host, bool from_padded_samples = false) {
     const vox_model_cfg& c = m->cfg; vox_ctx* cx = m->ctx; hipStream_t s = cx->stream;
-    const int PREFIX_LEN = 38, BOS = 1, STREAMING_PAD = 32;
+    const int PREFIX_LEN = VOX_PREFIX_TOKENS, BOS = VOX_TOK_BOS, STREAMING_PAD = VOX_TOK_STREAMING_PAD;
     VOXCHK(vox_model_set_t_embed(m, t_embed));
+    const bool pfx = from_padded_samples && !logits_host && prefix_usable(m, T);
+    const int PC = pfx ? m->pfx.PC : 0;
     double t0 = now_ms();
     RoctxScope whole("transcribe_streaming"); RoctxStage stage;
     stage.begin("encode_audio");
-    int S = 0; VOXCHK(encode_dev(m, d_mel, T, &S));
+    int S = 0; VOXCHK(encode_dev(m, d_mel, T, &S, pfx ? m->pfx.RC : 0));
     HIPCHK(hipStreamSynchronize(s));
     stage.end();
     m->timings.encode_ms = now_ms() - t0; t0 = now_ms();
@@ -1850,19 +1967,28 @@
     std::vector<int32_t> prefix(PREFIX_LEN, STREAMING_PAD); prefix[0] = BOS;
     HIPCHK(hipMemcpyAsync(m->d_tokens, prefix.data(), PREFIX_LEN * 4, hipMemcpyHostToDevice, s));
     m->cache->len = 0;
+    DevBuf dlog; float* d_logits_all = nullptr;
+    stage.begin("prefill");
+    if (pfx) {
+        const PrefixState& P = m->pfx; const size_t rows_bytes = (size_t)PC * c.dec_head_dim * 4, n_rows = (size_t)c.dec_layers * c.dec_kv_heads, pitch = (size_t)m->cache->max_seq * c.dec_head_dim * 4;
+        HIPCHK(hipMemcpy2DAsync(m->cache->k, pitch, P.dec_k, rows_bytes, rows_bytes, n_rows, hipMemcpyDeviceToDevice, s));
+        HIPCHK(hipMemcpy2DAsync(m->cache->v, pitch, P.dec_v, rows_bytes, rows_bytes, n_rows, hipMemcpyDeviceToDevice, s));
+        m->cache->len = PC;
+        HIPCHK(hipMemcpyAsync(m->d_pos, &PC, 4, hipMemcpyHostToDevice, s));
+        steps = S - PC - 1;
+    } else {
     if (!m->d_prefix) HIPCHK(hipMalloc((void**)&m->d_prefix, (size_t)PREFIX_LEN * c.dec_dim * 4));
     float* px = m->d_prefix;
-    stage.begin("prefill");
     HIPCHK(launch_embed(m->tok.w, m->d_tokens, PREFIX_LEN, m->d_audio, c.dec_dim, nullptr, 0, 0, px, s));
     VOXCHK(decoder_prefill_dev(m, px, PREFIX_LEN, m->cache, 0));
     m->cache->len = PREFIX_LEN;
-    DevBuf dlog; float* d_logits_all = nullptr;
     if (logits_host) { HIPCHK(dlog.alloc((size_t)n * c.vocab * 4)); d_logits_all = dlog.as<float>(); }
     VOXCHK(lm_head_argmax_dev(m, px + (size_t)(PREFIX_LEN - 1) * c.dec_dim, d_logits_all));
     const int pos_init = PREFIX_LEN;
     HIPCHK(hipMemcpyAsync(m->d_pos, &pos_init, 4, hipMemcpyHostToDevice, s));
     HIPCHK(launch_argmax_final(m->d_part_val, m->d_part_idx, m->n_parts, m->d_tokens, m->d_pos, 0, 0, s));
     steps = std::max(S - PREFIX_LEN - 1, 0);
+    }
     stage.begin("decode");
     if (steps > 0 && m->d_wo_acc) HIPCHK(hipMemsetAsync(m->d_wo_acc, 0, (size_t)c.dec_layers * c.dec_dim * 8, s));
     if (steps > 0) HIPCHK(launch_embed(m->tok.w, m->d_tokens, 1, m->d_audio, c.dec_dim, m->d_pos, 0, 0, m->d_h, s));
@@ -1919,7 +2045,7 @@
         m->eng_suspended = false; graphs_destroy(m);
         if (r != VOX_OK) return r;
     }
-    m->cache->len = PREFIX_LEN + steps;
+    m->cache->len = (pfx ? PC : PREFIX_LEN) + steps;
     *n_ids = n; m->timings.decode_tokens = n;
     m->timings.decode_ms = now_ms() - t0;
     return VOX_OK;
@@ -1961,6 +2087,7 @@
     const vox_model_cfg& c = m->cfg; vox_ctx* cx = m->ctx; hipStream_t s = cx->stream;
     ARGCHK(c.n_mels == 128, "the log-mel front-end produces 128 bins; model expects %d", c.n_mels);
     m->timings = vox_timings{};
+    VOXCHK(prefix_build(m, t_embed));
     const double t0 = now_ms();
     const float* d_s = samples;
     if (mem_kind == VOX_MEM_HOST) {
@@ -1975,7 +2102,7 @@
     HIPCHK(launch_mel(d_s, (long)n, (long)left, (long)right, cx->d_scale, t, m->d_mel, (int)T, 1, s));
     HIPCHK(hipStreamSynchronize(s));
     m->timings.preprocess_ms = now_ms() - t0;
-    VOXCHK(transcribe_dev(m, m->d_mel, (int)T, t_embed, out_ids, cap, n_ids, nullptr));
+    VOXCHK(transcribe_dev(m, m->d_mel, (int)T, t_embed, out_ids, cap, n_ids, nullptr, true));
     m->timings.total_ms = m->timings.preprocess_ms + m->timings.encode_ms + m->timings.decode_ms;
     return VOX_OK;
 }
diff --git a/voxtral-mini-realtime-rs_amd/csrc/vox_kernels.h b/voxtral-mini-realtime-rs_amd/csrc/vox_kernels.h
--- a/voxtral-mini-realtime-rs_amd/csrc/vox_kernels.h
+++ b/voxtral-mini-realtime-rs_amd/csrc/vox_kernels.h
@@ -117,8 +117,10 @@
     int tl_slot;
     int spec_zero;
     int spec_rows;
+    const float* prefix_k; const float* prefix_v; int prefix_len, prefix_row_stride, prefix_head_stride;
 };
 hipError_t launch_attn_prefill(const AttnParams& p, int hd, hipStream_t s, int n_seq = 1);
+bool attn_prefill_prefix_ok(const AttnParams& p, int hd, int n_seq);
 bool attn_prefill_small_ok(const AttnParams& p, int hd, int n_seq);
 hipError_t launch_attn_decode(const AttnParams& p, int hd, int max_seq, hipStream_t s, int n_seq = 1);
 bool attn_wo_supported(const AttnParams& p, const Q4W& wo, int hd, int max_seq);
diff --git a/voxtral-mini-realtime-rs_amd/csrc/vox_kernels.hip b/voxtral-mini-realtime-rs_amd/csrc/vox_kernels.hip
--- a/voxtral-mini-realtime-rs_amd/csrc/vox_kernels.hip
+++ b/voxtral-mini-realtime-rs_amd/csrc/vox_kernels.hip
@@ -2503,7 +2503,7 @@
             *reinterpret_cast<float4*>(op + e) = make_float4(o[e] * inv, o[e + 1] * inv, o[e + 2] * inv, o[e + 3] * inv);
     }
 }
-template <int HD>
+template <int HD, bool PFX>
 __global__ __launch_bounds__(256) __attribute__((amdgpu_waves_per_eu(2))) void attn_prefill_mfma_kernel(const AttnParams p) {
     constexpr int KS = HD / 32, DT = HD / 16, KROW = HD + 8, VROW = 72;
     extern __shared__ __attribute__((aligned(16))) uint16_t smh[];
@@ -2552,6 +2552,11 @@
     const size_t kvso = p.seq_row_off ? (size_t)p.seq_row_off[sq] * p.kv_row_stride : (size_t)sq * p.kv_seq_stride;
     const float* kbase = p.k + kvso + (size_t)kvh * p.kv_head_stride;
     const float* vbase = p.v + kvso + (size_t)kvh * p.kv_head_stride;
+    const int n_pfx = PFX ? p.prefix_len : 0;
+    const float* pkbase = PFX ? p.prefix_k + (size_t)kvh * p.prefix_head_stride : nullptr;
+    const float* pvbase = PFX ? p.prefix_v + (size_t)kvh * p.prefix_head_stride : nullptr;
+#define VOX_ATT_ROW(BASE_, PBASE_, J_) \
+    ((PFX && (J_) < n_pfx) ? (PBASE_) + (size_t)(J_) * p.prefix_row_stride : (BASE_) + (size_t)((J_) - n_pfx) * p.kv_row_stride)
 
     constexpr int NK = (64 * (HD / 4)) / 256, NV = (32 * (HD / 4)) / 256;
     float4 kreg[NK], vra[NV], vrb[NV];
@@ -2559,13 +2564,13 @@
     _Pragma("unroll") for (int u = 0; u < NK; u++) {                                                                \
         const int i = tid + 256 * u, key = i / (HD / 4), d4 = i % (HD / 4);                                         \
         const int jc = min((J0_) + key, kv_len - 1);      \
-        kreg[u] = *reinterpret_cast<const float4*>(kbase + (size_t)jc * p.kv_row_stride + d4 * 4);                  \
+        kreg[u] = *reinterpret_cast<const float4*>(VOX_ATT_ROW(kbase, pkbase, jc) + d4 * 4);                        \
     }                                                                                                               \
     _Pragma("unroll") for (int u = 0; u < NV; u++) {                                                                \
         const int i = tid + 256 * u, kp = i / (HD / 4), d4 = i % (HD / 4);                                          \
         const int ja = min((J0_) + 2 * kp, kv_len - 1), jb = min((J0_) + 2 * kp + 1, kv_len - 1);               \
-        vra[u] = *reinterpret_cast<const float4*>(vbase + (size_t)ja * p.kv_row_stride + d4 * 4);                   \
-        vrb[u] = *reinterpret_cast<const float4*>(vbase + (size_t)jb * p.kv_row_stride + d4 * 4);                   \
+        vra[u] = *reinterpret_cast<const float4*>(VOX_ATT_ROW(vbase, pvbase, ja) + d4 * 4);                         \
+        vrb[u] = *reinterpret_cast<const float4*>(VOX_ATT_ROW(vbase, pvbase, jb) + d4 * 4);                         \
     }
     const int j_first = (j_lo / 64) * 64, j_last = (j_hi / 64) * 64;
     VOX_ATT_LOAD(j_first)
@@ -2653,6 +2658,7 @@
         }
     }
 #undef VOX_ATT_LOAD
+#undef VOX_ATT_ROW
     lsum += __shfl_xor(lsum, 16, 64); lsum += __shfl_xor(lsum, 32, 64);
     if (m < M) {
         const float inv = 1.0f / lsum;
@@ -2662,10 +2668,10 @@
             *reinterpret_cast<float4*>(op + dt * 16) = make_float4(o[dt][0] * inv, o[dt][1] * inv, o[dt][2] * inv, o[dt][3] * inv);
     }
 }
-template <int HD>
+template <int HD, bool PFX>
 static hipError_t attn_prefill_mfma_launch(const AttnParams& p, hipStream_t s, int n_seq) {
     constexpr size_t lds = ((size_t)2 * 64 * (HD + 8) + (size_t)2 * HD * 72) * sizeof(uint16_t);
-    auto kern = attn_prefill_mfma_kernel<HD>;
+    auto kern = attn_prefill_mfma_kernel<HD, PFX>;
     static DevOnce attr_done;
     hipError_t e = ensure_dyn_lds(kern, lds, &attr_done);
     if (e != hipSuccess) return e;
@@ -2742,13 +2748,22 @@
     attn_form_note(ATTN_FORM_PREFILL_SMALL);
     return hipGetLastError();
 }
+bool attn_prefill_prefix_ok(const AttnParams& p, int hd, int n_seq) {
+    return (hd == 64 || hd == 128) && n_seq == 1 && !p.seq_len && !p.seq_row_off && !p.out_xf_tiles && p.prefix_k && p.prefix_v && p.prefix_len > 0 && p.offset == p.prefix_len &&
+           p.M >= 1 && p.kv_len == p.prefix_len + p.M && (p.q_stride % 4) == 0 && (p.kv_row_stride % 4) == 0 && (p.prefix_row_stride % 4) == 0 && (p.prefix_head_stride % 4) == 0 &&
+           !env_int("VOX_ATTN_F32");
+}
 hipError_t launch_attn_prefill(const AttnParams& p, int hd, hipStream_t s, int n_seq) {
     if (attn_prefill_small_ok(p, hd, n_seq)) return attn_prefill_small_launch(p, s, n_seq);
     if (p.out_xf_tiles) return hipErrorInvalidValue;
     const int f32_only = env_int("VOX_ATTN_F32");
+    if (p.prefix_len > 0) {
+        if (!attn_prefill_prefix_ok(p, hd, n_seq)) return hipErrorInvalidValue;
+        return hd == 64 ? attn_prefill_mfma_launch<64, true>(p, s, 1) : attn_prefill_mfma_launch<128, true>(p, s, 1);
+    }
     if (!f32_only && (p.q_stride % 4) == 0 && (p.kv_row_stride % 4) == 0) {
-        if (hd == 64) return attn_prefill_mfma_launch<64>(p, s, n_seq);
-        if (hd == 128) return attn_prefill_mfma_launch<128>(p, s, n_seq);
+        if (hd == 64) return attn_prefill_mfma_launch<64, false>(p, s, n_seq);
+        if (hd == 128) return attn_prefill_mfma_launch<128, false>(p, s, n_seq);
     }
     if (n_seq != 1 || p.seq_len) return hipErrorInvalidValue;
     dim3 grid((p.M + 63) / 64, p.n_heads);
diff --git a/voxtral-mini-realtime-rs_amd/gguf.py b/voxtral-mini-realtime-rs_amd/gguf.py
--- a/voxtral-mini-realtime-rs_amd/gguf.py
+++ b/voxtral-mini-realtime-rs_amd/gguf.py
@@ -412,6 +412,12 @@
 
     def set_decode_engine(self, on: bool) -> bool:
         a = C.c_int32(); check(lib().vox_model_set_decode_engine(self.h, 1 if on else 0, C.byref(a))); return bool(a.value)
+
+    def set_prefix_cache(self, on=None) -> bool:
+        a = C.c_int32(); check(lib().vox_model_set_prefix_cache(self.h, -1 if on is None else (1 if on else 0), C.byref(a))); return bool(a.value)
+
+    def prefix_info(self):
+        v = (C.c_int32 * 4)(); check(lib().vox_model_prefix_info(self.h, v)); return {"built": bool(v[0]), "encoder_rows": v[1], "decoder_positions": v[2], "bytes": v[3]}
 
     def memory(self):
         v = (C.c_uint64 * 4)(); check(lib().vox_model_memory(self.h, v)); return {"arena": v[0], "arena_primary": v[1], "engine_stream": v[2], "engine_state": v[3]}
```

Result: faster. 1498, median of 6 (+3.5%).
